# vlongle/pixie

Hardware: AMD Instinct MI355X
Metric: voxels/s (128^3 U-Net fwd) + MPM particle-steps/s (higher is better)
Workload: dtype f32 (operands split fp16 hi+lo, 3 f16 MFMAs/product, fp32 accumulate); 1 GPU; 128^3x64 feature grid -> SegmentationUNet+RegressionUNet forward (+argmax/one-hot combine), 1 scene per GPU per step; grid=128, feature_channels=64, parallelism=scene-parallel x1, executor=c+hip_graph

## Files before the change

include/pixie_hip.h:

```cpp
#ifndef PIXIE_HIP_H
#define PIXIE_HIP_H

#include <stdint.h>

#ifdef __cplusplus
extern "C" {
#endif

const char* pixie_last_error(void);
const char* pixie_build_arch(void);

typedef struct pixie_mpm pixie_mpm;

int pixie_mpm_create(pixie_mpm** out, int n_particles, int n_grid, double grid_lim);
int pixie_mpm_destroy(pixie_mpm* h);
int pixie_mpm_regrid(pixie_mpm* h, int n_grid, double grid_lim, void* stream);

int pixie_mpm_set_field(pixie_mpm* h, const char* name, const void* d_src, int64_t count, void* stream);
int pixie_mpm_get_field(pixie_mpm* h, const char* name, void* d_dst, int64_t count, void* stream);
int pixie_mpm_fill_field(pixie_mpm* h, const char* name, double value, void* stream);

int pixie_mpm_set_scalar(pixie_mpm* h, const char* key, double value);
int pixie_mpm_get_scalar(pixie_mpm* h, const char* key, double* value);

int pixie_mpm_update_mass(pixie_mpm* h, void* stream);
int pixie_mpm_finalize_mu_lam(pixie_mpm* h, int with_bulk, void* stream);
int pixie_mpm_apply_additional_params(pixie_mpm* h, const double point[3], const double size[3], double E,
                                      double nu, double density, int material, void* stream);
int pixie_mpm_apply_additional_params_batch(pixie_mpm* h, int64_t n_boxes, const float* d_boxes, const float* d_params,
                                            const int32_t* d_material, void* stream);

enum { PIXIE_BC_SURFACE = 0, PIXIE_BC_CUBOID = 1, PIXIE_BC_BBOX = 2 };
typedef struct pixie_bc_desc {
    int32_t type;
    int32_t surface_type;
    int32_t reset;
    int32_t pad_;
    double point[3], size[3], velocity[3], normal[3];
    double start_time, end_time, friction;
} pixie_bc_desc;
int pixie_mpm_add_bc(pixie_mpm* h, const pixie_bc_desc* bc);

enum { PIXIE_PM_IMPULSE = 0, PIXIE_PM_TRANSLATION = 1, PIXIE_PM_ROTATION = 2 };
typedef struct pixie_pmod_desc {
    int32_t type;
    int32_t pad_;
    double point[3], size[3];
    double force[3];
    double velocity[3];
    double normal[3], h1[3], h2[3];
    double half_height, radius, rotation_scale, translation_scale;
    double start_time, end_time;
} pixie_pmod_desc;
int pixie_mpm_add_particle_modifier(pixie_mpm* h, const pixie_pmod_desc* pm, void* stream);

int pixie_mpm_step(pixie_mpm* h, double dt, int n_substeps, void* stream);

typedef struct pixie_mpm_batch pixie_mpm_batch;
typedef struct pixie_batch_sched {
    double dt;
    int32_t steps_per_chunk;
    int32_t n_chunks;
    int32_t n_out;
    int32_t pad_;
    double shift[3], scale, mean[3];
    double inv_rotation[9];
    float* d_pos;
    float* d_cov;
} pixie_batch_sched;
int pixie_mpm_batch_create(pixie_mpm_batch** out, pixie_mpm* const* handles, int n_handles);
int pixie_mpm_batch_step(pixie_mpm_batch* b, double dt, int n_substeps, void* stream);
int pixie_mpm_batch_run(pixie_mpm_batch* b, const pixie_batch_sched* per_scene, int n_scenes, void* stream);
typedef struct pixie_batch_splat_out {
    float* d_log_scale;
    float* d_quat;
} pixie_batch_splat_out;
int pixie_mpm_batch_run_splats(pixie_mpm_batch* b, const pixie_batch_sched* per_scene, const pixie_batch_splat_out* splats ,
                               int n_scenes, void* stream);
int pixie_mpm_batch_destroy(pixie_mpm_batch* b);

int pixie_mpm_export_cov(pixie_mpm* h, float* d_cov , void* stream);
int pixie_mpm_export_R(pixie_mpm* h, float* d_R , void* stream);
int pixie_mpm_export_frame(pixie_mpm* h, int n_out, const double shift[3], double scale, const double mean[3],
                           const double inv_rotation[9], float* d_pos , float* d_cov ,
                           void* stream);
int pixie_splat_from_cov(const float* d_cov , int64_t n, float* d_log_scale , float* d_quat ,
                         void* stream);
int pixie_mpm_export_frame_splats(pixie_mpm* h, int n_out, const double shift[3], double scale, const double mean[3],
                                  const double inv_rotation[9], float* d_pos , float* d_cov ,
                                  float* d_log_scale , float* d_quat , void* stream);
int pixie_mpm_out_of_bounds(pixie_mpm* h, int64_t* count, void* stream);


typedef struct pixie_conv_desc {
    const float* d_in0; int32_t c0;
    const float* d_in1; int32_t c1;
    int32_t in_d, in_h, in_w;
    int32_t upsample;
    int32_t stride;
    int32_t ksize;
    const float* d_pro_a; const float* d_pro_b;
    const float* d_gamma; const float* d_beta;
    int32_t act;
    const float* d_w; const float* d_bias;
    int32_t c_out;
    const float* d_residual;
    float* d_out;
    const void* d_w16;
    const uint32_t* d_in_amax0; const uint32_t* d_in_amax1;
    float in_bound;
    float* d_out_stats;
    uint32_t* d_out_amax;
    void* d_workspace;
    int32_t out_d, out_h, out_w;
    const float* d_skip_in0; int32_t skip_c0;
    const float* d_skip_in1; int32_t skip_c1;
    const void* d_skip_w16; const float* d_skip_bias;
    const uint32_t* d_skip_amax0; const uint32_t* d_skip_amax1;
    int32_t w16_subpixel;
} pixie_conv_desc;

int pixie_conv_cout_padded(int c_out);
int pixie_conv_pack_weights(const float* d_w_oidhw, float* d_w_packed, int c_out, int c_in, int ksize, void* stream);
int64_t pixie_conv_packed16_bytes(int c_out, int c_in, int ksize);
int pixie_conv_pack_weights_f16x2(const float* d_w_oidhw, void* d_packed, int c_out, int c_in, int ksize, void* stream);
int64_t pixie_conv_subpixel_bytes(int c_out, int c_in);
int pixie_conv_pack_weights_subpixel(const float* d_w_oidhw, void* d_packed, int c_out, int c_in, void* stream);
int pixie_conv3d_forward(const pixie_conv_desc* desc, void* stream);
int64_t pixie_conv_stats_floats(const pixie_conv_desc* desc);
int64_t pixie_conv_workspace_bytes(const pixie_conv_desc* desc);
int pixie_stats_finalize(const float* d_stats, const pixie_conv_desc* desc, double* d_sums, void* stream);
int pixie_conv_skip_foldable(const pixie_conv_desc* desc);

int pixie_channel_sums(const float* d_x, int channels, int64_t spatial, double* d_sums, void* stream);
int pixie_channel_stats(const float* d_x, int channels, int64_t spatial, double* d_sums, uint32_t* d_amax, void* stream);
int pixie_tensor_amax(const float* d_x, int64_t count, uint32_t* d_slot, void* stream);
int pixie_norm_finalize(const double* d_sums, int channels, int64_t spatial, int mode, int groups, double eps,
                        const float* d_weight, const float* d_bias, float* d_a, float* d_b, void* stream);

int pixie_attention_forward(const float* d_qkv, float* d_out, int channels, int tokens, void* stream);

int pixie_channel_affine(const float* d_x, const float* d_a, const float* d_b, float* d_y, int channels,
                         int64_t spatial, void* stream);

int pixie_voxel_grid_to_ncdhw(const void* d_feat_dhwc_f16, int d, int h, int w, int channels, float* d_out_cdhw, void* stream);

int pixie_projector_conv0(const void* d_feat_dhwc_f16, int64_t voxels, int channels, int n_networks, const void* const* d_w16,
                          const float* const* d_bias, float* const* d_out, int c_out, void* stream);

int pixie_pack_fields(const float* d_cont, const int32_t* d_seg_pred, int64_t n_scenes, int64_t spatial, void* d_wire, int64_t wire_bytes,
                      void* stream);

int pixie_combine_predictions(const float* d_logits, int num_classes, const float* d_cont, int64_t spatial,
                              float* d_combined, int32_t* d_argmax , void* stream);

int pixie_combine_class_ids(const int32_t* d_seg_pred, int num_classes, const float* d_cont, int64_t spatial, float* d_combined,
                            void* stream);

typedef struct pixie_unet pixie_unet;
typedef struct pixie_unet_config {
    int32_t feature_channels, cond_dim, model_channels, num_res_blocks;
    int32_t n_channel_mult; int32_t channel_mult[8];
    int32_t n_attention_resolutions; int32_t attention_resolutions[8];
    int32_t grid_size;
    int32_t out_channels;
    int32_t precision;
} pixie_unet_config;

int pixie_unet_create(pixie_unet** out, const pixie_unet_config* cfg);
int pixie_unet_destroy(pixie_unet* h);
int pixie_unet_param_count(const pixie_unet* h);
int pixie_unet_param_info(const pixie_unet* h, int index, const char** key, int64_t* numel, int32_t* ndim, int64_t shape[5]);
int pixie_unet_set_param(pixie_unet* h, const char* key, const float* d_values, int64_t numel);
int64_t pixie_unet_workspace_bytes(pixie_unet* h, int d, int hh, int w);
int pixie_unet_forward(pixie_unet* h, const float* d_feat, const float* d_proj0, int d, int hh, int w, float* d_out,
                       void* d_workspace, int64_t workspace_bytes, void* stream);
int pixie_unet_set_option(pixie_unet* h, const char* key, int value);

typedef struct pixie_field_desc {
    const float* d_pred;
    const uint8_t* d_mask;
    const float* d_axis_x; const float* d_axis_y; const float* d_axis_z;
    int32_t n_classes, d, h, w;
    double min_spacing;
    double density_min, density_max, E_min, E_max, nu_min, nu_max;
} pixie_field_desc;
int pixie_field_to_particles(const pixie_field_desc* field, const float* d_pos, int n, int k, double nn_distance_threshold,
                             int weighted, int default_material, int default_part_label, float* d_density, float* d_E,
                             float* d_nu, int32_t* d_material, int32_t* d_part_label, float* d_conf, float* d_nearest,
                             void* d_scratch, void* stream);

int pixie_unscale_prediction(const float* d_pred, int channels, int64_t spatial, double density_min, double density_max,
                             double E_min, double E_max, double nu_min, double nu_max, float* d_out, void* stream);
int64_t pixie_field_points_scratch_bytes(const pixie_field_desc* field);
int pixie_field_points(const pixie_field_desc* field, int64_t capacity, float* d_xyz , float* d_density, float* d_E,
                       float* d_nu, int32_t* d_material, float* d_conf, int64_t* d_count, void* d_scratch, void* stream);

int pixie_dbscan_roots(const float* d_pos_sorted, const int32_t* d_orig_index, const int32_t* d_cell_start, int n, int nx, int ny, int nz,
                       const double lo[3], double cell_size, double eps, int min_samples, int32_t* d_core_scratch,
                       int32_t* d_parent_scratch, int32_t* d_root, void* stream);

int pixie_fill_densify(const float* d_pos, const float* d_opacity, const float* d_cov6, int n, int grid_n, double grid_dx,
                       int32_t* d_grid_count, float* d_grid_density, void* stream);
int pixie_fill_dense_cells(int32_t* d_grid_count, const float* d_grid_density, int grid_n, double grid_dx, double density_thres,
                           int max_particles_per_cell, float* d_new_particles , int64_t max_samples,
                           uint64_t* d_counter, uint32_t seed, void* stream);
int pixie_fill_internal_cells(int32_t* d_grid_count, const float* d_grid_density, int grid_n, double grid_dx, int max_particles_per_cell,
                              int exclude_dir, int ray_cast_dir, double threshold, float* d_new_particles, int64_t max_samples,
                              uint64_t* d_counter, uint32_t seed, void* stream);
int pixie_particle_volume(const float* d_pos, int n, int grid_n, double grid_dx, int32_t* d_grid_count_scratch, float* d_vol, void* stream);
int pixie_nearest_particle(const float* d_pos, int n, const float* d_new_pos, int n_new, int32_t* d_nearest, void* stream);

#ifdef PIXIE_DIAG
int pixie_mpm_phase(pixie_mpm* h, int phase, double dt, void* stream);

int pixie_mpm_kernel_times(pixie_mpm* h, double* particle_ms, double* grid_ms, int64_t* n_launches);

int pixie_conv_kernel_variant(const pixie_conv_desc* desc, int* slices);

int pixie_conv_tile_geometry(const pixie_conv_desc* desc, int32_t out[10]);
#endif

#ifdef __cplusplus
}
#endif
#endif
```

pixie_amd/_lib.py:

```python
from __future__ import annotations

import ctypes as C
import os

_HERE = os.path.dirname(os.path.abspath(__file__))
LIB_PATH = os.path.join(_HERE, "libpixie_hip.so")
DIAG_LIB_PATH = os.path.join(_HERE, "libpixie_hip_diag.so")


class PixieHipError(RuntimeError):
    pass


class BCDesc(C.Structure):
    _fields_ = [("type", C.c_int32), ("surface_type", C.c_int32), ("reset", C.c_int32), ("pad_", C.c_int32),
                ("point", C.c_double * 3), ("size", C.c_double * 3), ("velocity", C.c_double * 3),
                ("normal", C.c_double * 3), ("start_time", C.c_double), ("end_time", C.c_double),
                ("friction", C.c_double)]


class PModDesc(C.Structure):
    _fields_ = [("type", C.c_int32), ("pad_", C.c_int32),
                ("point", C.c_double * 3), ("size", C.c_double * 3), ("force", C.c_double * 3),
                ("velocity", C.c_double * 3), ("normal", C.c_double * 3), ("h1", C.c_double * 3),
                ("h2", C.c_double * 3), ("half_height", C.c_double), ("radius", C.c_double),
                ("rotation_scale", C.c_double), ("translation_scale", C.c_double),
                ("start_time", C.c_double), ("end_time", C.c_double)]


class ConvDesc(C.Structure):
    _fields_ = [("d_in0", C.c_void_p), ("c0", C.c_int32),
                ("d_in1", C.c_void_p), ("c1", C.c_int32),
                ("in_d", C.c_int32), ("in_h", C.c_int32), ("in_w", C.c_int32),
                ("upsample", C.c_int32), ("stride", C.c_int32), ("ksize", C.c_int32),
                ("d_pro_a", C.c_void_p), ("d_pro_b", C.c_void_p),
                ("d_gamma", C.c_void_p), ("d_beta", C.c_void_p),
                ("act", C.c_int32),
                ("d_w", C.c_void_p), ("d_bias", C.c_void_p),
                ("c_out", C.c_int32),
                ("d_residual", C.c_void_p), ("d_out", C.c_void_p),
                ("d_w16", C.c_void_p), ("d_in_amax0", C.c_void_p), ("d_in_amax1", C.c_void_p),
                ("in_bound", C.c_float),
                ("d_out_stats", C.c_void_p), ("d_out_amax", C.c_void_p),
                ("d_workspace", C.c_void_p),
                ("out_d", C.c_int32), ("out_h", C.c_int32), ("out_w", C.c_int32),
                ("d_skip_in0", C.c_void_p), ("skip_c0", C.c_int32),
                ("d_skip_in1", C.c_void_p), ("skip_c1", C.c_int32),
                ("d_skip_w16", C.c_void_p), ("d_skip_bias", C.c_void_p),
                ("d_skip_amax0", C.c_void_p), ("d_skip_amax1", C.c_void_p),
                ("w16_subpixel", C.c_int32)]


class UNetConfigC(C.Structure):
    _fields_ = [("feature_channels", C.c_int32), ("cond_dim", C.c_int32), ("model_channels", C.c_int32), ("num_res_blocks", C.c_int32),
                ("n_channel_mult", C.c_int32), ("channel_mult", C.c_int32 * 8),
                ("n_attention_resolutions", C.c_int32), ("attention_resolutions", C.c_int32 * 8),
                ("grid_size", C.c_int32), ("out_channels", C.c_int32), ("precision", C.c_int32)]


class BatchSched(C.Structure):
    _fields_ = [("dt", C.c_double), ("steps_per_chunk", C.c_int32), ("n_chunks", C.c_int32), ("n_out", C.c_int32), ("pad_", C.c_int32),
                ("shift", C.c_double * 3), ("scale", C.c_double), ("mean", C.c_double * 3), ("inv_rotation", C.c_double * 9),
                ("d_pos", C.c_void_p), ("d_cov", C.c_void_p)]


class BatchSplatOut(C.Structure):
    _fields_ = [("d_log_scale", C.c_void_p), ("d_quat", C.c_void_p)]


class FieldDesc(C.Structure):
    _fields_ = [("d_pred", C.c_void_p), ("d_mask", C.c_void_p),
                ("d_axis_x", C.c_void_p), ("d_axis_y", C.c_void_p), ("d_axis_z", C.c_void_p),
                ("n_classes", C.c_int32), ("d", C.c_int32), ("h", C.c_int32), ("w", C.c_int32),
                ("min_spacing", C.c_double),
                ("density_min", C.c_double), ("density_max", C.c_double), ("E_min", C.c_double), ("E_max", C.c_double),
                ("nu_min", C.c_double), ("nu_max", C.c_double)]


_VP, _I, _I64, _D, _S = C.c_void_p, C.c_int, C.c_int64, C.c_double, C.c_char_p
_D3 = C.POINTER(C.c_double)
SIGNATURES = {
    "pixie_last_error": (C.c_char_p, []),
    "pixie_build_arch": (C.c_char_p, []),
    "pixie_mpm_create": (_I, [C.POINTER(_VP), _I, _I, _D]),
    "pixie_mpm_destroy": (_I, [_VP]),
    "pixie_mpm_regrid": (_I, [_VP, _I, _D, _VP]),
    "pixie_mpm_set_field": (_I, [_VP, _S, _VP, _I64, _VP]),
    "pixie_mpm_get_field": (_I, [_VP, _S, _VP, _I64, _VP]),
    "pixie_mpm_fill_field": (_I, [_VP, _S, _D, _VP]),
    "pixie_mpm_set_scalar": (_I, [_VP, _S, _D]),
    "pixie_mpm_get_scalar": (_I, [_VP, _S, C.POINTER(_D)]),
    "pixie_mpm_update_mass": (_I, [_VP, _VP]),
    "pixie_mpm_finalize_mu_lam": (_I, [_VP, _I, _VP]),
    "pixie_mpm_apply_additional_params": (_I, [_VP, _D3, _D3, _D, _D, _D, _I, _VP]),
    "pixie_mpm_apply_additional_params_batch": (_I, [_VP, _I64, _VP, _VP, _VP, _VP]),
    "pixie_mpm_add_bc": (_I, [_VP, C.POINTER(BCDesc)]),
    "pixie_mpm_add_particle_modifier": (_I, [_VP, C.POINTER(PModDesc), _VP]),
    "pixie_mpm_step": (_I, [_VP, _D, _I, _VP]),
    "pixie_mpm_export_cov": (_I, [_VP, _VP, _VP]),
    "pixie_mpm_export_R": (_I, [_VP, _VP, _VP]),
    "pixie_mpm_export_frame": (_I, [_VP, _I, _D3, _D, _D3, C.POINTER(C.c_double), _VP, _VP, _VP]),
    "pixie_mpm_out_of_bounds": (_I, [_VP, C.POINTER(_I64), _VP]),
    "pixie_mpm_batch_create": (_I, [C.POINTER(_VP), C.POINTER(_VP), _I]),
    "pixie_mpm_batch_step": (_I, [_VP, _D, _I, _VP]),
    "pixie_mpm_batch_run": (_I, [_VP, C.POINTER(BatchSched), _I, _VP]),
    "pixie_mpm_batch_run_splats": (_I, [_VP, C.POINTER(BatchSched), C.POINTER(BatchSplatOut), _I, _VP]),
    "pixie_splat_from_cov": (_I, [_VP, _I64, _VP, _VP, _VP]),
    "pixie_mpm_export_frame_splats": (_I, [_VP, _I, _D3, _D, _D3, C.POINTER(C.c_double), _VP, _VP, _VP, _VP, _VP]),
    "pixie_mpm_batch_destroy": (_I, [_VP]),
    "pixie_pack_fields": (_I, [_VP, _VP, _I64, _I64, _VP, _I64, _VP]),
    "pixie_conv_cout_padded": (_I, [_I]),
    "pixie_conv_pack_weights": (_I, [_VP, _VP, _I, _I, _I, _VP]),
    "pixie_conv_packed16_bytes": (_I64, [_I, _I, _I]),
    "pixie_conv_pack_weights_f16x2": (_I, [_VP, _VP, _I, _I, _I, _VP]),
    "pixie_conv_subpixel_bytes": (_I64, [_I, _I]),
    "pixie_conv_pack_weights_subpixel": (_I, [_VP, _VP, _I, _I, _VP]),
    "pixie_conv3d_forward": (_I, [C.POINTER(ConvDesc), _VP]),
    "pixie_conv_stats_floats": (_I64, [C.POINTER(ConvDesc)]),
    "pixie_conv_workspace_bytes": (_I64, [C.POINTER(ConvDesc)]),
    "pixie_stats_finalize": (_I, [_VP, C.POINTER(ConvDesc), _VP, _VP]),
    "pixie_channel_stats": (_I, [_VP, _I, _I64, _VP, _VP, _VP]),
    "pixie_tensor_amax": (_I, [_VP, _I64, _VP, _VP]),
    "pixie_channel_sums": (_I, [_VP, _I, _I64, _VP, _VP]),
    "pixie_norm_finalize": (_I, [_VP, _I, _I64, _I, _I, _D, _VP, _VP, _VP, _VP, _VP]),
    "pixie_attention_forward": (_I, [_VP, _VP, _I, _I, _VP]),
    "pixie_channel_affine": (_I, [_VP, _VP, _VP, _VP, _I, _I64, _VP]),
    "pixie_projector_conv0": (_I, [_VP, _I64, _I, _I, C.POINTER(_VP), C.POINTER(_VP), C.POINTER(_VP), _I, _VP]),
    "pixie_conv_skip_foldable": (_I, [C.POINTER(ConvDesc)]),
    "pixie_unet_create": (_I, [C.POINTER(_VP), C.POINTER(UNetConfigC)]),
    "pixie_unet_destroy": (_I, [_VP]),
    "pixie_unet_param_count": (_I, [_VP]),
    "pixie_unet_param_info": (_I, [_VP, _I, C.POINTER(_S), C.POINTER(_I64), C.POINTER(C.c_int32), C.POINTER(_I64)]),
    "pixie_unet_set_param": (_I, [_VP, _S, _VP, _I64]),
    "pixie_unet_workspace_bytes": (_I64, [_VP, _I, _I, _I]),
    "pixie_unet_set_option": (_I, [_VP, _S, _I]),
    "pixie_unet_forward": (_I, [_VP, _VP, _VP, _I, _I, _I, _VP, _VP, _I64, _VP]),
    "pixie_combine_class_ids": (_I, [_VP, _I, _VP, _I64, _VP, _VP]),
    "pixie_combine_predictions": (_I, [_VP, _I, _VP, _I64, _VP, _VP, _VP]),
    "pixie_voxel_grid_to_ncdhw": (_I, [_VP, _I, _I, _I, _I, _VP, _VP]),
    "pixie_unscale_prediction": (_I, [_VP, _I, _I64, _D, _D, _D, _D, _D, _D, _VP, _VP]),
    "pixie_field_points_scratch_bytes": (_I64, [C.POINTER(FieldDesc)]),
    "pixie_field_points": (_I, [C.POINTER(FieldDesc), _I64, _VP, _VP, _VP, _VP, _VP, _VP, _VP, _VP, _VP]),
    "pixie_fill_densify": (_I, [_VP, _VP, _VP, _I, _I, _D, _VP, _VP, _VP]),
    "pixie_fill_dense_cells": (_I, [_VP, _VP, _I, _D, _D, _I, _VP, _I64, _VP, C.c_uint32, _VP]),
    "pixie_fill_internal_cells": (_I, [_VP, _VP, _I, _D, _I, _I, _I, _D, _VP, _I64, _VP, C.c_uint32, _VP]),
    "pixie_particle_volume": (_I, [_VP, _I, _I, _D, _VP, _VP, _VP]),
    "pixie_nearest_particle": (_I, [_VP, _I, _VP, _I, _VP, _VP]),
    "pixie_dbscan_roots": (_I, [_VP, _VP, _VP, _I, _I, _I, _I, C.POINTER(_D), _D, _D, _I, _VP, _VP, _VP, _VP]),
    "pixie_field_to_particles": (_I, [C.POINTER(FieldDesc), _VP, _I, _I, _D, _I, _I, _I, _VP, _VP, _VP, _VP, _VP, _VP, _VP, _VP, _VP]),
}

DIAG_SIGNATURES = {
    "pixie_mpm_phase": (_I, [_VP, _I, _D, _VP]),
    "pixie_mpm_kernel_times": (_I, [_VP, C.POINTER(_D), C.POINTER(_D), C.POINTER(_I64)]),
    "pixie_conv_kernel_variant": (C.c_int, [C.POINTER(ConvDesc), C.POINTER(C.c_int)]),
    "pixie_conv_tile_geometry": (C.c_int, [C.POINTER(ConvDesc), C.POINTER(C.c_int32)]),
}

_libs = {}


def load(diag: bool = False):
    if diag in _libs:
        return _libs[diag]
    path = DIAG_LIB_PATH if diag else LIB_PATH
    if not os.path.exists(path):
        raise PixieHipError(
            f"{path} not found: build it with `python -m pixie_amd.build` (hipcc, gfx950). "
            "pixie_amd has no CPU fallback.")
    import torch
    lib = C.CDLL(path)
    for name, (res, args) in list(SIGNATURES.items()) + (list(DIAG_SIGNATURES.items()) if diag else []):
        fn = getattr(lib, name)
        fn.restype = res
        fn.argtypes = args
    _libs[diag] = lib
    return lib


def check(rc: int, what: str = "", lib=None):
    if rc != 0:
        msg = (lib or load()).pixie_last_error()
        raise PixieHipError(f"{what}: {msg.decode() if msg else 'unknown error'}")


def current_stream_ptr():
    import torch
    try:
        return C.c_void_p(torch._C._cuda_getCurrentRawStream(torch.cuda.current_device()))
    except AttributeError:
        return C.c_void_p(torch.cuda.current_stream().cuda_stream)


def d3(v):
    return (C.c_double * 3)(*[float(x) for x in v])
```

pixie_amd/csrc/conv3d_f16x3.hip:

```cpp
#include <hip/hip_runtime.h>

#include <cstdlib>
#include <map>
#include <string>
#include <type_traits>

#include "../../include/pixie_hip.h"
#include "common.h"

namespace pixie {

typedef float f32x16 __attribute__((ext_vector_type(16)));
typedef _Float16 f16x8 __attribute__((ext_vector_type(8)));

constexpr int kW16HeaderU4 = 4;

struct Conv16Args {
    const float* in0; const float* in1;
    int c0, cin;
    int ID, IH, IW;
    int LD, LH, LW;
    int ups;
    int stride;
    int OD, OH, OW;
    const float* pro_a; const float* pro_b; const float* gamma; const float* beta;
    int act;
    const uint4* w16;
    const float* wf;
    const float* bias;
    int cout, coutp;
    const float* residual; float* out;
    const unsigned* amax0; const unsigned* amax1;
    float in_bound;
    int TX, TY, TZ, lTX, lTY;
    int tiles_x, tiles_y, tiles_z, n_tiles;
    int HX, HY, HZ, HYX, CS;
    unsigned mHX, mHYX;
    float* stats; unsigned* out_amax;
    float* partial; int chunks_per_slice;
    int epi_lds;
    const float* sk_in0; const float* sk_in1;
    int sk_c0, sk_cin;
    const uint4* sk_w16; const float* sk_bias;
    const unsigned* sk_amax0; const unsigned* sk_amax1;
};

__device__ __forceinline__ int fast_div16(int n, int d, unsigned magic) {
    return (d == 1) ? n : (int)__umulhi((unsigned)n, magic);
}
__device__ __forceinline__ float act16(float t, int act) {
    if (act == 1) return t > 0.0f ? t : 0.02f * t;
    if (act == 2) return t / (1.0f + __expf(-t));
    return t;
}
__device__ __forceinline__ int scale_exponent(float bound) {
    const unsigned bits = __float_as_uint(bound);
    const int eb = (int)((bits >> 23) & 0xffu) - 127;
    if (!(bound > 0.0f) || eb > 100) return 0;
    int e = 14 - eb;
    return e > 100 ? 100 : (e < -100 ? -100 : e);
}
__device__ __forceinline__ float pow2i(int e) { return __uint_as_float((unsigned)(e + 127) << 23); }

template <int KS, int MB, int NB, bool EX = false, bool SP = false>
__device__ __forceinline__ void conv3d_f16x3_body(const Conv16Args& A) {
    static_assert(!SP || (KS == 3 && NB == 4 && !EX), "sub-pixel path: 3^3, two x parities x two voxel blocks per wave");
    extern __shared__ uint4 smem16[];
    constexpr int PAD = (KS == 3) ? 1 : 0;
    constexpr int NW = 4, NT = 64 * NW;
    const int bufsz = 4 * A.CS;

    const int tid = threadIdx.x;
    const int lane = tid & 63;
    const int wave = tid >> 6;
    const int kh = lane >> 5;
    const int l31 = lane & 31;

    int t = blockIdx.x;
    {
        const int per = (A.n_tiles + 7) >> 3;
        const int cand = (t & 7) * per + (t >> 3);
        if ((A.n_tiles & 7) == 0) t = cand;
    }
    int par = 0;
    if constexpr (SP) { par = t & 3; t >>= 2; }
    const int py = par & 1, pz = par >> 1;
    const int tx = t % A.tiles_x; t /= A.tiles_x;
    const int ty = t % A.tiles_y;
    const int tz = t / A.tiles_y;
    const int ox0 = tx * A.TX, oy0 = ty * A.TY, oz0 = tz * A.TZ;
    const int cout0 = blockIdx.y * (MB * 32);
    const int lx0 = SP ? ox0 - 1 : ox0 * A.stride - PAD;
    const int ly0 = SP ? oy0 - 1 + py : oy0 * A.stride - PAD;
    const int lz0 = SP ? oz0 - 1 + pz : oz0 * A.stride - PAD;
    const size_t ISP = (size_t)A.ID * A.IH * A.IW;
    const size_t OSP = (size_t)A.OD * A.OH * A.OW;

    int voff[NB];
    int ovox[NB];
    bool valid[NB];
#pragma unroll
    for (int nb = 0; nb < NB; ++nb) {
        if constexpr (SP) {
            const int px = nb >> 1;
            const int j = (wave * 2 + (nb & 1)) * 32 + l31;
            int x = j & (A.TX - 1);
            int y = (j >> A.lTX) & (A.TY - 1);
            int z = j >> (A.lTX + A.lTY);
            const int gx = 2 * (ox0 + x) + px, gy = 2 * (oy0 + y) + py, gz = 2 * (oz0 + z) + pz;
            const bool v = (z < A.TZ) && (gx < A.OW) && (gy < A.OH) && (gz < A.OD);
            if (!v) { x = 0; y = 0; z = 0; }
            voff[nb] = (z * A.HY + y) * A.HX + x + px + kh * A.CS;
            ovox[nb] = v ? (gz * A.OH + gy) * A.OW + gx : 0;
            valid[nb] = v;
            continue;
        }
        const int j = (wave * NB + nb) * 32 + l31;
        int x = j & (A.TX - 1);
        int y = (j >> A.lTX) & (A.TY - 1);
        int z = j >> (A.lTX + A.lTY);
        const bool v = (z < A.TZ) && (ox0 + x < A.OW) && (oy0 + y < A.OH) && (oz0 + z < A.OD);
        if (!v) { x = 0; y = 0; z = 0; }
        voff[nb] = ((z * A.HY + y) * A.HX + x) * A.stride + kh * A.CS;
        ovox[nb] = ((oz0 + z) * A.OH + (oy0 + y)) * A.OW + ox0 + x;
        valid[nb] = v;
    }

    float bound = A.in_bound;
    if (A.amax0) {
        bound = __uint_as_float(*A.amax0);
        if (A.amax1) bound = fmaxf(bound, __uint_as_float(*A.amax1));
    }
    const int ex = EX ? 0 : scale_exponent(bound);
    const float sx = pow2i(ex);

    f32x16 acc[MB][NB];
#pragma unroll
    for (int mb = 0; mb < MB; ++mb)
#pragma unroll
        for (int nb = 0; nb < NB; ++nb)
#pragma unroll
            for (int r = 0; r < 16; ++r) acc[mb][nb][r] = 0.0f;

    const int KG = A.cin >> 3;
    const size_t tap_stride = (size_t)KG * A.coutp;
    const size_t plane = (size_t)(SP ? 64 : KS * KS * KS) * tap_stride;
    const uint4* wHi = A.w16 + kW16HeaderU4 + (size_t)kh * A.coutp + cout0 + l31 + (size_t)(par * 16) * tap_stride;
    const uint4* wLo = wHi + plane;
    const float* wF = A.wf + (size_t)kh * A.coutp + cout0 + l31;

    constexpr int TAPS = KS * KS * KS;
    auto stage_chunk = [&](int c_base, uint4* buf, int stid, int nthr) {
        uint4* bHi = buf;
        uint4* bLo = buf + 2 * A.CS;
        float pa[16], pb[16];
        {
            float pv = 0.0f;
            if (A.pro_a) pv = (lane & 16) ? A.pro_b[c_base + (lane & 15)] : A.pro_a[c_base + (lane & 15)];
#pragma unroll
            for (int j = 0; j < 16; ++j) {
                pa[j] = __int_as_float(__builtin_amdgcn_readlane(__float_as_int(pv), j));
                pb[j] = __int_as_float(__builtin_amdgcn_readlane(__float_as_int(pv), 16 + j));
            }
        }
        const bool has_aff = A.gamma != nullptr;
        for (int v0 = stid; v0 < A.CS; v0 += 2 * nthr) {
            float val[2][16];
            float gm[2], bt[2];
            int sidx[2];
            bool ok[2];
#pragma unroll
            for (int u = 0; u < 2; ++u) {
                const int vox = v0 + u * nthr;
                int rem = vox;
                const int hz = fast_div16(rem, A.HYX, A.mHYX);
                rem -= hz * A.HYX;
                const int hy = fast_div16(rem, A.HX, A.mHX);
                const int hx = rem - hy * A.HX;
                const int lz = lz0 + hz, ly = ly0 + hy, lx = lx0 + hx;
                ok[u] = vox < A.CS && (unsigned)lz < (unsigned)A.LD && (unsigned)ly < (unsigned)A.LH && (unsigned)lx < (unsigned)A.LW;
                sidx[u] = ok[u] ? ((lz >> A.ups) * A.IH + (ly >> A.ups)) * A.IW + (lx >> A.ups) : 0;
            }
#pragma unroll
            for (int u = 0; u < 2; ++u) {
#pragma unroll
                for (int j = 0; j < 16; ++j) {
                    const int cg = c_base + j;
                    const float* src = (cg < A.c0) ? (A.in0 + (size_t)cg * ISP) : (A.in1 + (size_t)(cg - A.c0) * ISP);
                    val[u][j] = src[sidx[u]];
                }
                gm[u] = 1.0f; bt[u] = 0.0f;
                if (has_aff) { gm[u] = A.gamma[sidx[u]]; bt[u] = A.beta[sidx[u]]; }
            }
            auto convert = [&](auto has_pro, auto act_c) {
#pragma unroll
                for (int u = 0; u < 2; ++u) {
                    const int vox = v0 + u * nthr;
                    if (EX) {
                        float* bF = reinterpret_cast<float*>(buf);
#pragma unroll
                        for (int j = 0; j < 16; ++j) {
                            float t = val[u][j];
                            if (decltype(has_pro)::value) t = t * pa[j] + pb[j];
                            t = t * gm[u] + bt[u];
                            const float sc = ok[u] ? act16(t, decltype(act_c)::value) : 0.0f;
                            if (vox < A.CS) bF[j * A.CS + vox] = sc;
                        }
                        continue;
                    }
                    f16x8 vh[2], vl[2];
#pragma unroll
                    for (int j = 0; j < 16; ++j) {
                        float t = val[u][j];
                        if (decltype(has_pro)::value) t = t * pa[j] + pb[j];
                        t = t * gm[u] + bt[u];
                        const float sc = ok[u] ? act16(t, decltype(act_c)::value) * sx : 0.0f;
                        const _Float16 h = (_Float16)sc;
                        vh[j >> 3][j & 7] = h;
                        vl[j >> 3][j & 7] = (_Float16)(sc - (float)h);
                    }
                    if (vox < A.CS) {
                        bHi[vox] = __builtin_bit_cast(uint4, vh[0]);
                        bHi[A.CS + vox] = __builtin_bit_cast(uint4, vh[1]);
                        bLo[vox] = __builtin_bit_cast(uint4, vl[0]);
                        bLo[A.CS + vox] = __builtin_bit_cast(uint4, vl[1]);
                    }
                }
            };
            using T = std::true_type; using F = std::false_type;
            if (A.pro_a) {
                if (A.act == 1) convert(T{}, std::integral_constant<int, 1>{});
                else if (A.act == 2) convert(T{}, std::integral_constant<int, 2>{});
                else convert(T{}, std::integral_constant<int, 0>{});
            } else {
                if (A.act == 1) convert(F{}, std::integral_constant<int, 1>{});
                else if (A.act == 2) convert(F{}, std::integral_constant<int, 2>{});
                else convert(F{}, std::integral_constant<int, 0>{});
            }
        }
    };
    auto mfma_chunk = [&](int c_base, const uint4* buf) {
        __builtin_amdgcn_s_setprio(3);
        if constexpr (EX) {
            const float* ldsF = reinterpret_cast<const float*>(buf);
            const size_t tapw = (size_t)A.cin * A.coutp;
            const float* wc = wF + (size_t)c_base * A.coutp;
            float a[8][MB], an[8][MB];
#pragma unroll
            for (int kp = 0; kp < 8; ++kp)
#pragma unroll
                for (int mb = 0; mb < MB; ++mb) a[kp][mb] = wc[(size_t)(2 * kp) * A.coutp + mb * 32];
#pragma unroll 1
            for (int zy = 0; zy < KS * KS; ++zy) {
                const int dz = zy / KS, dy = zy - dz * KS;
                const int rowoff = (dz * A.HY + dy) * A.HX;
#pragma unroll
                for (int dx = 0; dx < KS; ++dx) {
                    const int tap = zy * KS + dx;
                    const int nxt = (tap + 1 < TAPS) ? tap + 1 : tap;
#pragma unroll
                    for (int kp = 0; kp < 8; ++kp)
#pragma unroll
                        for (int mb = 0; mb < MB; ++mb) an[kp][mb] = wc[(size_t)nxt * tapw + (size_t)(2 * kp) * A.coutp + mb * 32];
                    __builtin_amdgcn_sched_barrier(0);
#pragma unroll
                    for (int kp = 0; kp < 8; ++kp) {
                        float b[NB];
#pragma unroll
                        for (int nb = 0; nb < NB; ++nb) b[nb] = ldsF[voff[nb] + rowoff + dx + 2 * kp * A.CS];
#pragma unroll
                        for (int mb = 0; mb < MB; ++mb)
#pragma unroll
                            for (int nb = 0; nb < NB; ++nb)
                                acc[mb][nb] = __builtin_amdgcn_mfma_f32_32x32x2f32(a[kp][mb], b[nb], acc[mb][nb], 0, 0, 0);
                    }
#pragma unroll
                    for (int kp = 0; kp < 8; ++kp)
#pragma unroll
                        for (int mb = 0; mb < MB; ++mb) a[kp][mb] = an[kp][mb];
                }
            }
            __builtin_amdgcn_s_setprio(0);
            return;
        }
        const uint4* ldsHi = buf;
        const uint4* ldsLo = buf + 2 * A.CS;
        const uint4* wh = wHi + (size_t)(c_base >> 3) * A.coutp;
        const uint4* wl = wLo + (size_t)(c_base >> 3) * A.coutp;
        if constexpr (SP) {
            f16x8 ah[MB], al[MB];
#pragma unroll
            for (int mb = 0; mb < MB; ++mb) {
                ah[mb] = __builtin_bit_cast(f16x8, wh[mb * 32]);
                al[mb] = __builtin_bit_cast(f16x8, wl[mb * 32]);
            }
#pragma unroll 1
            for (int zy = 0; zy < 4; ++zy) {
                const int rowoff = ((zy >> 1) * A.HY + (zy & 1)) * A.HX;
                const int zyn = zy < 3 ? zy + 1 : 3;
#pragma unroll
                for (int q = 0; q < 4; ++q) {
                    const int ex = q >> 1, px = q & 1;
                    const size_t nxt = (q < 3) ? (size_t)(((q + 1) & 1) * 8 + zy * 2 + ((q + 1) >> 1)) * tap_stride : (size_t)(zyn * 2) * tap_stride;
                    f16x8 ahn[MB], aln[MB];
#pragma unroll
                    for (int mb = 0; mb < MB; ++mb) {
                        ahn[mb] = __builtin_bit_cast(f16x8, wh[nxt + mb * 32]);
                        aln[mb] = __builtin_bit_cast(f16x8, wl[nxt + mb * 32]);
                    }
                    __builtin_amdgcn_sched_barrier(0);
                    f16x8 bh[2], bl[2];
#pragma unroll
                    for (int s = 0; s < 2; ++s) {
                        bh[s] = __builtin_bit_cast(f16x8, ldsHi[voff[px * 2 + s] + rowoff + ex]);
                        bl[s] = __builtin_bit_cast(f16x8, ldsLo[voff[px * 2 + s] + rowoff + ex]);
                    }
#pragma unroll
                    for (int mb = 0; mb < MB; ++mb)
#pragma unroll
                        for (int s = 0; s < 2; ++s)
                            acc[mb][px * 2 + s] = __builtin_amdgcn_mfma_f32_32x32x16_f16(al[mb], bh[s], acc[mb][px * 2 + s], 0, 0, 0);
#pragma unroll
                    for (int mb = 0; mb < MB; ++mb)
#pragma unroll
                        for (int s = 0; s < 2; ++s)
                            acc[mb][px * 2 + s] = __builtin_amdgcn_mfma_f32_32x32x16_f16(ah[mb], bl[s], acc[mb][px * 2 + s], 0, 0, 0);
#pragma unroll
                    for (int mb = 0; mb < MB; ++mb)
#pragma unroll
                        for (int s = 0; s < 2; ++s)
                            acc[mb][px * 2 + s] = __builtin_amdgcn_mfma_f32_32x32x16_f16(ah[mb], bh[s], acc[mb][px * 2 + s], 0, 0, 0);
#pragma unroll
                    for (int mb = 0; mb < MB; ++mb) { ah[mb] = ahn[mb]; al[mb] = aln[mb]; }
                }
            }
            __builtin_amdgcn_s_setprio(0);
            return;
        }
        f16x8 ah[MB], al[MB];
#pragma unroll
        for (int mb = 0; mb < MB; ++mb) {
            ah[mb] = __builtin_bit_cast(f16x8, wh[mb * 32]);
            al[mb] = __builtin_bit_cast(f16x8, wl[mb * 32]);
        }
#pragma unroll 1
        for (int zy = 0; zy < KS * KS; ++zy) {
            const int dz = zy / KS, dy = zy - dz * KS;
            const int rowoff = (dz * A.HY + dy) * A.HX;
#pragma unroll
            for (int dx = 0; dx < KS; ++dx) {
                const int tap = zy * KS + dx;
                const int nxt = (tap + 1 < TAPS) ? tap + 1 : tap;
                f16x8 ahn[MB], aln[MB];
#pragma unroll
                for (int mb = 0; mb < MB; ++mb) {
                    ahn[mb] = __builtin_bit_cast(f16x8, wh[(size_t)nxt * tap_stride + mb * 32]);
                    aln[mb] = __builtin_bit_cast(f16x8, wl[(size_t)nxt * tap_stride + mb * 32]);
                }
                __builtin_amdgcn_sched_barrier(0);
                f16x8 bh[NB], bl[NB];
#pragma unroll
                for (int nb = 0; nb < NB; ++nb) {
                    bh[nb] = __builtin_bit_cast(f16x8, ldsHi[voff[nb] + rowoff + dx]);
                    bl[nb] = __builtin_bit_cast(f16x8, ldsLo[voff[nb] + rowoff + dx]);
                }
#pragma unroll
                for (int mb = 0; mb < MB; ++mb)
#pragma unroll
                    for (int nb = 0; nb < NB; ++nb)
                        acc[mb][nb] = __builtin_amdgcn_mfma_f32_32x32x16_f16(al[mb], bh[nb], acc[mb][nb], 0, 0, 0);
#pragma unroll
                for (int mb = 0; mb < MB; ++mb)
#pragma unroll
                    for (int nb = 0; nb < NB; ++nb)
                        acc[mb][nb] = __builtin_amdgcn_mfma_f32_32x32x16_f16(ah[mb], bl[nb], acc[mb][nb], 0, 0, 0);
#pragma unroll
                for (int mb = 0; mb < MB; ++mb)
#pragma unroll
                    for (int nb = 0; nb < NB; ++nb)
                        acc[mb][nb] = __builtin_amdgcn_mfma_f32_32x32x16_f16(ah[mb], bh[nb], acc[mb][nb], 0, 0, 0);
#pragma unroll
                for (int mb = 0; mb < MB; ++mb) { ah[mb] = ahn[mb]; al[mb] = aln[mb]; }
            }
        }
        __builtin_amdgcn_s_setprio(0);
    };

    float inv2 = 0.0f;
    {
        const int c_begin = A.partial ? (int)blockIdx.z * A.chunks_per_slice * 16 : 0;
        const int c_end = A.partial ? min(A.cin, c_begin + A.chunks_per_slice * 16) : A.cin;
        for (int c_base = c_begin; c_base < c_end; c_base += 16) {
            __syncthreads();
            stage_chunk(c_base, smem16, tid, NT);
            __syncthreads();
            mfma_chunk(c_base, smem16);
        }
        if (!EX && !SP && A.sk_w16) {
            float sb = __uint_as_float(*A.sk_amax0);
            if (A.sk_amax1) sb = fmaxf(sb, __uint_as_float(*A.sk_amax1));
            const int ex2 = scale_exponent(sb);
            const float sx2 = pow2i(ex2);
            const float inv_main = __uint_as_float(A.w16[0].x) * pow2i(-ex);
            inv2 = __uint_as_float(A.sk_w16[0].x) * pow2i(-ex2);
            const float ratio = inv_main / inv2;
#pragma unroll
            for (int mb = 0; mb < MB; ++mb)
#pragma unroll
                for (int nb = 0; nb < NB; ++nb)
#pragma unroll
                    for (int r = 0; r < 16; ++r) acc[mb][nb][r] *= ratio;
            const int KG2 = A.sk_cin >> 3;
            const uint4* w2Hi = A.sk_w16 + kW16HeaderU4 + (size_t)kh * A.coutp + cout0 + l31;
            const uint4* w2Lo = w2Hi + (size_t)KG2 * A.coutp;
            const int centre = (KS == 3) ? (A.HY + 1) * A.HX + 1 : 0;
            const int tvox = A.TX * A.TY * A.TZ;
            for (int c2 = 0; c2 < A.sk_cin; c2 += 16) {
                f16x8 ah[MB], al[MB];
#pragma unroll
                for (int mb = 0; mb < MB; ++mb) {
                    ah[mb] = __builtin_bit_cast(f16x8, w2Hi[(size_t)(c2 >> 3) * A.coutp + mb * 32]);
                    al[mb] = __builtin_bit_cast(f16x8, w2Lo[(size_t)(c2 >> 3) * A.coutp + mb * 32]);
                }
                __syncthreads();
                uint4* bHi = smem16;
                uint4* bLo = smem16 + 2 * A.CS;
                for (int j = tid; j < tvox; j += NT) {
                    const int x = j & (A.TX - 1), y = (j >> A.lTX) & (A.TY - 1), z = j >> (A.lTX + A.lTY);
                    const bool okv = (ox0 + x < A.OW) && (oy0 + y < A.OH) && (oz0 + z < A.OD);
                    const size_t sidx = okv ? ((size_t)(oz0 + z) * A.IH + (oy0 + y)) * A.IW + ox0 + x : 0;
                    float val[16];
#pragma unroll
                    for (int q = 0; q < 16; ++q) {
                        const int cg = c2 + q;
                        const float* src = (cg < A.sk_c0) ? (A.sk_in0 + (size_t)cg * ISP) : (A.sk_in1 + (size_t)(cg - A.sk_c0) * ISP);
                        val[q] = src[sidx];
                    }
                    f16x8 vh[2], vl[2];
#pragma unroll
                    for (int q = 0; q < 16; ++q) {
                        const float sc = okv ? val[q] * sx2 : 0.0f;
                        const _Float16 hq = (_Float16)sc;
                        vh[q >> 3][q & 7] = hq;
                        vl[q >> 3][q & 7] = (_Float16)(sc - (float)hq);
                    }
                    const int slot = (z * A.HY + y) * A.HX + x + centre;
                    bHi[slot] = __builtin_bit_cast(uint4, vh[0]);
                    bHi[A.CS + slot] = __builtin_bit_cast(uint4, vh[1]);
                    bLo[slot] = __builtin_bit_cast(uint4, vl[0]);
                    bLo[A.CS + slot] = __builtin_bit_cast(uint4, vl[1]);
                }
                __syncthreads();
                f16x8 bh[NB], bl[NB];
#pragma unroll
                for (int nb = 0; nb < NB; ++nb) {
                    bh[nb] = __builtin_bit_cast(f16x8, bHi[voff[nb] + centre]);
                    bl[nb] = __builtin_bit_cast(f16x8, bLo[voff[nb] + centre]);
                }
#pragma unroll
                for (int mb = 0; mb < MB; ++mb)
#pragma unroll
                    for (int nb = 0; nb < NB; ++nb)
                        acc[mb][nb] = __builtin_amdgcn_mfma_f32_32x32x16_f16(al[mb], bh[nb], acc[mb][nb], 0, 0, 0);
#pragma unroll
                for (int mb = 0; mb < MB; ++mb)
#pragma unroll
                    for (int nb = 0; nb < NB; ++nb)
                        acc[mb][nb] = __builtin_amdgcn_mfma_f32_32x32x16_f16(ah[mb], bl[nb], acc[mb][nb], 0, 0, 0);
#pragma unroll
                for (int mb = 0; mb < MB; ++mb)
#pragma unroll
                    for (int nb = 0; nb < NB; ++nb)
                        acc[mb][nb] = __builtin_amdgcn_mfma_f32_32x32x16_f16(ah[mb], bh[nb], acc[mb][nb], 0, 0, 0);
            }
        }
    }

    const float inv = EX ? 1.0f : (A.sk_w16 ? inv2 : __uint_as_float(A.w16[0].x) * pow2i(-ex));
    if (A.partial) {
        float* dst = A.partial + (size_t)blockIdx.z * A.cout * OSP;
#pragma unroll
        for (int mb = 0; mb < MB; ++mb)
#pragma unroll
            for (int r = 0; r < 16; ++r) {
                const int co = cout0 + mb * 32 + (r & 3) + 8 * (r >> 2) + 4 * kh;
                if (co < A.cout) {
#pragma unroll
                    for (int nb = 0; nb < NB; ++nb)
                        if (valid[nb]) dst[(size_t)co * OSP + ovox[nb]] = acc[mb][nb][r] * inv;
                }
            }
        return;
    }
    float* red = reinterpret_cast<float*>(smem16);
    float wmax = 0.0f;
    const bool full = SP ? (A.epi_lds && cout0 + MB * 32 <= A.cout && (A.TX & 1) == 0 && (A.OW & 3) == 0 && NW * 64 <= A.TX * A.TY * A.TZ &&
                            2 * (ox0 + A.TX) <= A.OW && 2 * (oy0 + A.TY) <= A.OH && 2 * (oz0 + A.TZ) <= A.OD)
                         : (A.epi_lds && cout0 + MB * 32 <= A.cout && (A.TX & 3) == 0 && (A.OW & 3) == 0 && NW * NB * 32 <= A.TX * A.TY * A.TZ &&
                            ox0 + A.TX <= A.OW && oy0 + A.TY <= A.OH && oz0 + A.TZ <= A.OD);
    if (full) {
        __syncthreads();
        constexpr int LDO = NB * 32 + 4;
        float* ldsO = reinterpret_cast<float*>(smem16) + wave * (32 * LDO);
        red = reinterpret_cast<float*>(smem16) + NW * 32 * LDO;
        constexpr int LPR = NB * 8;
        constexpr int RPI = 32 / LPR;
        const int rsub = l31 / LPR, colq = 4 * (l31 % LPR), nbq = colq >> 5;
        const int jq = SP ? wave * 64 + (colq >> 1) : (wave * NB + nbq) * 32 + (colq & 31);
        const int xq = jq & (A.TX - 1), yq = (jq >> A.lTX) & (A.TY - 1), zq = jq >> (A.lTX + A.lTY);
        const size_t ovq = SP ? ((size_t)(2 * (oz0 + zq) + pz) * A.OH + (2 * (oy0 + yq) + py)) * A.OW + 2 * (ox0 + xq)
                              : ((size_t)(oz0 + zq) * A.OH + (oy0 + yq)) * A.OW + ox0 + xq;
        const bool has_res = A.residual != nullptr, has_stats = A.stats != nullptr;
#pragma unroll
        for (int mb = 0; mb < MB; ++mb) {
#pragma unroll
            for (int r = 0; r < 16; ++r)
#pragma unroll
                for (int nb = 0; nb < NB; ++nb)
                    ldsO[((r & 3) + 8 * (r >> 2) + 4 * kh) * LDO + (SP ? 2 * ((nb & 1) * 32 + l31) + (nb >> 1) : nb * 32 + l31)] = acc[mb][nb][r];
#pragma unroll 4
            for (int it = 0; it < 16 / RPI; ++it) {
                const int rowl = (2 * it + kh) * RPI + rsub;
                const int co = cout0 + mb * 32 + rowl;
                const float4 a4 = *reinterpret_cast<const float4*>(ldsO + rowl * LDO + colq);
                const float bv = (A.bias ? A.bias[co] : 0.0f) + (A.sk_bias ? A.sk_bias[co] : 0.0f);
                const size_t o = (size_t)co * OSP + ovq;
                float4 v4;
                v4.x = a4.x * inv + bv; v4.y = a4.y * inv + bv; v4.z = a4.z * inv + bv; v4.w = a4.w * inv + bv;
                if (has_res) {
                    const float4 r4 = *reinterpret_cast<const float4*>(A.residual + o);
                    v4.x += r4.x; v4.y += r4.y; v4.z += r4.z; v4.w += r4.w;
                }
                *reinterpret_cast<float4*>(A.out + o) = v4;
                if (has_stats) {
                    float s1 = (v4.x + v4.y) + (v4.z + v4.w);
                    float s2 = (v4.x * v4.x + v4.y * v4.y) + (v4.z * v4.z + v4.w * v4.w);
                    wmax = fmaxf(fmaxf(wmax, fmaxf(fabsf(v4.x), fabsf(v4.y))), fmaxf(fabsf(v4.z), fabsf(v4.w)));
#pragma unroll
                    for (int off = LPR / 2; off > 0; off >>= 1) { s1 += __shfl_xor(s1, off, 64); s2 += __shfl_xor(s2, off, 64); }
                    if ((l31 % LPR) == 0) { red[(wave * MB * 32 + mb * 32 + rowl) * 2] = s1; red[(wave * MB * 32 + mb * 32 + rowl) * 2 + 1] = s2; }
                }
            }
        }
    } else {
    if (A.stats) __syncthreads();
#pragma unroll
    for (int mb = 0; mb < MB; ++mb) {
#pragma unroll
        for (int r = 0; r < 16; ++r) {
            const int row = mb * 32 + (r & 3) + 8 * (r >> 2) + 4 * kh;
            const int co = cout0 + row;
            float s1 = 0.0f, s2 = 0.0f;
            if (co < A.cout) {
                const float bv = (A.bias ? A.bias[co] : 0.0f) + (A.sk_bias ? A.sk_bias[co] : 0.0f);
#pragma unroll
                for (int nb = 0; nb < NB; ++nb) {
                    if (valid[nb]) {
                        const size_t o = (size_t)co * OSP + ovox[nb];
                        float val = acc[mb][nb][r] * inv + bv;
                        if (A.residual) val += A.residual[o];
                        A.out[o] = val;
                        s1 += val; s2 += val * val; wmax = fmaxf(wmax, fabsf(val));
                    }
                }
            }
            if (A.stats) {
#pragma unroll
                for (int off = 16; off > 0; off >>= 1) { s1 += __shfl_xor(s1, off, 64); s2 += __shfl_xor(s2, off, 64); }
                if (l31 == 0) { red[(wave * MB * 32 + row) * 2] = s1; red[(wave * MB * 32 + row) * 2 + 1] = s2; }
            }
        }
    }
    }
    if (A.stats) {
        __syncthreads();
        if (tid < MB * 32 * 2) {
            float t = red[tid];
#pragma unroll
            for (int w = 1; w < NW; ++w) t += red[w * MB * 64 + tid];
            A.stats[((size_t)blockIdx.x * A.coutp + cout0) * 2 + tid] = t;
        }
        if (A.out_amax) {
#pragma unroll
            for (int off = 32; off > 0; off >>= 1) wmax = fmaxf(wmax, __shfl_xor(wmax, off, 64));
            if (lane == 0 && wmax > 0.0f) atomicMax(A.out_amax, __float_as_uint(wmax));
        }
    }
}

template <int KS, int MB, int NB>
__global__ __launch_bounds__(256, 2) void conv3d_f16x3_kernel(Conv16Args A) {
    conv3d_f16x3_body<KS, MB, NB>(A);
}
template <int KS, int MB, int NB>
__global__ __launch_bounds__(256, 2) void conv3d_exact_kernel(Conv16Args A) {
    conv3d_f16x3_body<KS, MB, NB, true>(A);
}
template <int MB>
__global__ __launch_bounds__(256, 2) void conv3d_f16x3_subpixel_kernel(Conv16Args A) {
    conv3d_f16x3_body<3, MB, 4, false, true>(A);
}
__global__ __launch_bounds__(256, 2) void conv3d_f16x3_c64_fullres_kernel(Conv16Args A) {
    conv3d_f16x3_body<3, 2, 4>(A);
}

__global__ __launch_bounds__(256) void stats_finalize_kernel(const float* __restrict__ stats, int n_tiles, int coutp, double* __restrict__ sums) {
    const int c = blockIdx.x;
    double s1 = 0.0, s2 = 0.0;
    for (int t = threadIdx.x; t < n_tiles; t += 256) {
        const float2 v = *reinterpret_cast<const float2*>(stats + ((size_t)t * coutp + c) * 2);
        s1 += v.x; s2 += v.y;
    }
    for (int off = 32; off > 0; off >>= 1) { s1 += __shfl_down(s1, off, 64); s2 += __shfl_down(s2, off, 64); }
    __shared__ double r[8];
    if ((threadIdx.x & 63) == 0) { r[2 * (threadIdx.x >> 6)] = s1; r[2 * (threadIdx.x >> 6) + 1] = s2; }
    __syncthreads();
    if (threadIdx.x == 0) { sums[2 * c] = r[0] + r[2] + r[4] + r[6]; sums[2 * c + 1] = r[1] + r[3] + r[5] + r[7]; }
}

__global__ __launch_bounds__(256) void splitk_reduce_kernel(const float* __restrict__ partial, int slices, long n_elems, long osp,
                                                            const float* __restrict__ bias, const float* residual, float* out) {
    const long i = (long)blockIdx.x * 256 + threadIdx.x;
    if (i >= n_elems) return;
    float v = partial[i];
    for (int s = 1; s < slices; ++s) v += partial[(size_t)s * n_elems + i];
    if (bias) v += bias[i / osp];
    if (residual) v += residual[i];
    out[i] = v;
}

__global__ __launch_bounds__(256) void amax_kernel(const float* __restrict__ x, long n, unsigned* __restrict__ slot) {
    float m = 0.0f;
    const long stride = (long)gridDim.x * 256 * 4;
    long i = ((long)blockIdx.x * 256 + threadIdx.x) * 4;
    if ((reinterpret_cast<size_t>(x) & 15) == 0) {
        for (; i + 3 < n; i += stride) {
            const float4 v = *reinterpret_cast<const float4*>(x + i);
            m = fmaxf(fmaxf(m, fabsf(v.x)), fmaxf(fabsf(v.y), fmaxf(fabsf(v.z), fabsf(v.w))));
        }
        for (long k = i; k < n && k < i + 4; ++k) m = fmaxf(m, fabsf(x[k]));
    } else {
        for (long k = (long)blockIdx.x * 256 + threadIdx.x; k < n; k += (long)gridDim.x * 256) m = fmaxf(m, fabsf(x[k]));
    }
    for (int off = 32; off > 0; off >>= 1) m = fmaxf(m, __shfl_down(m, off, 64));
    if ((threadIdx.x & 63) == 0 && m > 0.0f) atomicMax(slot, __float_as_uint(m));
}

__global__ void pack_weights_f16x2_kernel(const float* __restrict__ src, uint4* __restrict__ dst, int cout, int cin, int taps,
                                          int coutp, const unsigned* __restrict__ amax_bits) {
    const int KG = cin >> 3;
    const long total = (long)taps * KG * coutp;
    const long i = (long)blockIdx.x * blockDim.x + threadIdx.x;
    const int e = scale_exponent(__uint_as_float(*amax_bits));
    if (i == 0) dst[0] = make_uint4(__float_as_uint(pow2i(-e)), (unsigned)cout, (unsigned)cin, (unsigned)taps);
    if (i >= total) return;
    const float s = pow2i(e);
    const int co = (int)(i % coutp);
    const long row = i / coutp;
    const int kg = (int)(row % KG);
    const int tap = (int)(row / KG);
    f16x8 vh, vl;
#pragma unroll
    for (int j = 0; j < 8; ++j) {
        float w = 0.0f;
        if (co < cout) w = src[((long)co * cin + kg * 8 + j) * taps + tap] * s;
        const _Float16 h = (_Float16)w;
        vh[j] = h;
        vl[j] = (_Float16)(w - (float)h);
    }
    dst[kW16HeaderU4 + i] = __builtin_bit_cast(uint4, vh);
    dst[kW16HeaderU4 + total + i] = __builtin_bit_cast(uint4, vl);
}

__device__ __forceinline__ float subpixel_weight(const float* __restrict__ w27, int par, int tap) {
    int lo[3], hi[3];
#pragma unroll
    for (int ax = 0; ax < 3; ++ax) {
        const int p = (par >> (2 - ax)) & 1, e = (tap >> (2 - ax)) & 1;
        lo[ax] = e ? (p ? 2 : 1) : 0;
        hi[ax] = e ? 2 : (p ? 1 : 0);
    }
    float sum = 0.0f;
    for (int dz = lo[0]; dz <= hi[0]; ++dz)
        for (int dy = lo[1]; dy <= hi[1]; ++dy)
            for (int dx = lo[2]; dx <= hi[2]; ++dx) sum += w27[(dz * 3 + dy) * 3 + dx];
    return sum;
}
__global__ __launch_bounds__(256) void subpixel_amax_kernel(const float* __restrict__ src, long pairs, unsigned* __restrict__ slot) {
    const long i = (long)blockIdx.x * 256 + threadIdx.x;
    float m = 0.0f;
    if (i < pairs)
        for (int pt = 0; pt < 64; ++pt) m = fmaxf(m, fabsf(subpixel_weight(src + i * 27, pt >> 3, pt & 7)));
    for (int off = 32; off > 0; off >>= 1) m = fmaxf(m, __shfl_down(m, off, 64));
    if ((threadIdx.x & 63) == 0 && m > 0.0f) atomicMax(slot, __float_as_uint(m));
}
__global__ void pack_weights_subpixel_kernel(const float* __restrict__ src, uint4* __restrict__ dst, int cout, int cin, int coutp,
                                             const unsigned* __restrict__ amax_bits) {
    const int KG = cin >> 3;
    const long total = 64L * KG * coutp;
    const long i = (long)blockIdx.x * blockDim.x + threadIdx.x;
    const int e = scale_exponent(__uint_as_float(*amax_bits));
    if (i == 0) dst[0] = make_uint4(__float_as_uint(pow2i(-e)), (unsigned)cout, (unsigned)cin, 64u);
    if (i >= total) return;
    const float s = pow2i(e);
    const int co = (int)(i % coutp);
    const long row = i / coutp;
    const int kg = (int)(row % KG);
    const int pt = (int)(row / KG);
    f16x8 vh, vl;
#pragma unroll
    for (int j = 0; j < 8; ++j) {
        float w = 0.0f;
        if (co < cout) w = subpixel_weight(src + ((long)co * cin + kg * 8 + j) * 27, pt >> 3, pt & 7) * s;
        const _Float16 h = (_Float16)w;
        vh[j] = h;
        vl[j] = (_Float16)(w - (float)h);
    }
    dst[kW16HeaderU4 + i] = __builtin_bit_cast(uint4, vh);
    dst[kW16HeaderU4 + total + i] = __builtin_bit_cast(uint4, vl);
}

static unsigned magic_of16(int d) { return d <= 1 ? 0u : (unsigned)((0x100000000ull + (unsigned long long)d - 1) / (unsigned long long)d); }
static int ilog2_16(int v) { int l = 0; while ((1 << l) < v) ++l; return l; }
static int pow2_le16(int v, int cap) { int p = 1; while (p * 2 <= v && p * 2 <= cap) p *= 2; return p; }

template <int MB>
static int launch_subpixel(const Conv16Args& a, size_t lds_bytes, dim3 grid, hipStream_t st) {
    auto kern = conv3d_f16x3_subpixel_kernel<MB>;
    PX_CHECK_HIP(allow_max_dynamic_lds(reinterpret_cast<const void*>(kern)));
    hipLaunchKernelGGL(kern, grid, dim3(256), lds_bytes, st, a);
    PX_CHECK_HIP(hipGetLastError());
    return 0;
}

static bool conv16_subpixel(const pixie_conv_desc* d) {
    return d->d_w16 && d->w16_subpixel && d->upsample == 1 && d->ksize == 3 && d->stride == 1;
}

template <int KS, int MB, int NB>
static int launch_f16x3(const Conv16Args& a, size_t lds_bytes, dim3 grid, hipStream_t st) {
    auto kern = conv3d_f16x3_kernel<KS, MB, NB>;
    PX_CHECK_HIP(allow_max_dynamic_lds(reinterpret_cast<const void*>(kern)));
    hipLaunchKernelGGL(kern, grid, dim3(256), lds_bytes, st, a);
    PX_CHECK_HIP(hipGetLastError());
    return 0;
}

static void conv16_tiling(const pixie_conv_desc* d, Conv16Args& a, int& MB_out, int& NB_out, int* slices_out = nullptr) {
    a.ID = d->in_d; a.IH = d->in_h; a.IW = d->in_w;
    a.ups = d->upsample;
    a.LD = a.ID << a.ups; a.LH = a.IH << a.ups; a.LW = a.IW << a.ups;
    const int pad = d->ksize == 3 ? 1 : 0;
    a.stride = d->stride;
    a.OD = (a.LD + 2 * pad - d->ksize) / a.stride + 1; a.OH = (a.LH + 2 * pad - d->ksize) / a.stride + 1; a.OW = (a.LW + 2 * pad - d->ksize) / a.stride + 1;
    if (d->out_d > 0) a.OD = std::min(a.OD, (int)d->out_d);
    if (d->out_h > 0) a.OH = std::min(a.OH, (int)d->out_h);
    if (d->out_w > 0) a.OW = std::min(a.OW, (int)d->out_w);
    a.cout = d->c_out; a.coutp = pixie_conv_cout_padded(d->c_out);
    const int chunks = (d->c0 + d->c1) / 16;
    const int smax = d->d_workspace ? std::min(8, chunks / 2) : 1;
    if (conv16_subpixel(d)) {
        a.ups = 0; a.LD = a.ID; a.LH = a.IH; a.LW = a.IW;
        const int SD = (a.OD + 1) / 2, SH = (a.OH + 1) / 2, SW = (a.OW + 1) / 2;
        a.TX = pow2_le16(SW, 32);
        a.TY = pow2_le16(SH, std::max(1, std::min(4, 256 / a.TX)));
        a.TZ = std::max(1, std::min(SD, 256 / (a.TX * a.TY)));
        a.lTX = ilog2_16(a.TX); a.lTY = ilog2_16(a.TY);
        a.tiles_x = (SW + a.TX - 1) / a.TX; a.tiles_y = (SH + a.TY - 1) / a.TY; a.tiles_z = (SD + a.TZ - 1) / a.TZ;
        a.n_tiles = 4 * a.tiles_x * a.tiles_y * a.tiles_z;
        a.HX = a.TX + 2; a.HY = a.TY + 1; a.HZ = a.TZ + 1;
        a.HYX = a.HY * a.HX; a.CS = a.HZ * a.HYX;
        a.mHX = magic_of16(a.HX); a.mHYX = magic_of16(a.HYX);
        MB_out = (a.coutp >= 64) ? 2 : 1; NB_out = 4;
        int sl = 1;
        const long wgs = (long)a.n_tiles * ((a.coutp + MB_out * 32 - 1) / (MB_out * 32));
        while (sl * 2 <= smax && wgs * sl < 512) sl *= 2;
        if (slices_out) *slices_out = sl;
        return;
    }
    const long ovol = (long)a.OD * a.OH * a.OW;
    int MB = (a.coutp >= 64) ? 2 : 1;
    int NB = (a.stride == 2) ? 1 : 4;
    auto n_wg = [&](int mb, int nb) {
        const long tiles = (ovol + 128L * nb - 1) / (128L * nb);
        return tiles * ((a.coutp + mb * 32 - 1) / (mb * 32));
    };
    int slices = 1;
    if (smax >= 2 && n_wg(MB, NB) < 512) {
        bool found = false;
        for (int nb = NB; nb >= 1 && !found; nb /= 2) {
            for (int sl = 1; sl <= smax; sl *= 2)
                if (n_wg(MB, nb) * sl >= 512) { NB = nb; slices = sl; found = true; break; }
        }
        if (!found) { NB = 1; slices = 1; while (slices * 2 <= smax) slices *= 2; }
    } else {
        while (n_wg(MB, NB) < 512 && NB > 1) NB /= 2;
        if (n_wg(MB, NB) < 512 && MB > 1) MB = 1;
    }
    if (slices_out) *slices_out = slices;
    const int tile_vox = 128 * NB;
    a.TX = pow2_le16(a.OW, 32);
    a.TY = pow2_le16(a.OH, std::max(1, std::min(4, tile_vox / a.TX)));
    a.TZ = std::max(1, std::min(a.OD, tile_vox / (a.TX * a.TY)));
    a.lTX = ilog2_16(a.TX); a.lTY = ilog2_16(a.TY);
    a.tiles_x = (a.OW + a.TX - 1) / a.TX; a.tiles_y = (a.OH + a.TY - 1) / a.TY; a.tiles_z = (a.OD + a.TZ - 1) / a.TZ;
    a.n_tiles = a.tiles_x * a.tiles_y * a.tiles_z;
    a.HX = (a.TX - 1) * a.stride + d->ksize; a.HY = (a.TY - 1) * a.stride + d->ksize; a.HZ = (a.TZ - 1) * a.stride + d->ksize;
    a.HYX = a.HY * a.HX; a.CS = a.HZ * a.HYX;
    a.mHX = magic_of16(a.HX); a.mHYX = magic_of16(a.HYX);

    MB_out = MB; NB_out = NB;
}

static size_t conv16_epi_bytes(int MB, int NB) { return ((size_t)4 * 32 * (NB * 32 + 4) + (size_t)4 * MB * 32 * 2) * sizeof(float); }
static bool conv16_epi_lds(int MB, int NB, int slices) { return slices == 1 && conv16_epi_bytes(MB, NB) <= 80 * 1024; }

static void conv16_exact_tiling(const pixie_conv_desc* d, Conv16Args& a, int& MB_out, int& NB_out) {
    pixie_conv_desc probe = *d;
    probe.d_workspace = nullptr;
    probe.w16_subpixel = 0;
    int slices = 1;
    conv16_tiling(&probe, a, MB_out, NB_out, &slices);
}

int conv3d_f16x3_forward(const pixie_conv_desc* d, hipStream_t st) {
    PX_REQUIRE(d->stride == 1 || (d->stride == 2 && d->ksize == 3 && !d->upsample), "f16x3 conv: stride must be 1, or 2 for a 3^3 kernel");
    const int cin = d->c0 + d->c1;
    PX_REQUIRE(cin % 16 == 0 && d->c0 % 8 == 0, "f16x3 conv: c_in must be a multiple of 16 (got %d+%d)", d->c0, d->c1);
    PX_REQUIRE(d->d_in_amax0 != nullptr || d->in_bound > 0.0f, "f16x3 conv: needs d_in_amax0 or a positive in_bound");
    PX_REQUIRE(d->c1 == 0 || d->d_in_amax0 == nullptr || d->d_in_amax1 != nullptr, "f16x3 conv: second input needs its own amax slot");
    Conv16Args a{};
    a.in0 = d->d_in0; a.in1 = d->d_in1; a.c0 = d->c0; a.cin = cin;
    a.ID = d->in_d; a.IH = d->in_h; a.IW = d->in_w;
    a.ups = d->upsample;
    a.LD = a.ID << a.ups; a.LH = a.IH << a.ups; a.LW = a.IW << a.ups;
    const int pad = d->ksize == 3 ? 1 : 0;
    a.stride = d->stride;
    a.OD = (a.LD + 2 * pad - d->ksize) / a.stride + 1; a.OH = (a.LH + 2 * pad - d->ksize) / a.stride + 1; a.OW = (a.LW + 2 * pad - d->ksize) / a.stride + 1;
    if (d->out_d > 0) a.OD = std::min(a.OD, (int)d->out_d);
    if (d->out_h > 0) a.OH = std::min(a.OH, (int)d->out_h);
    if (d->out_w > 0) a.OW = std::min(a.OW, (int)d->out_w);
    a.pro_a = d->d_pro_a; a.pro_b = d->d_pro_b; a.gamma = d->d_gamma; a.beta = d->d_beta; a.act = d->act;
    a.w16 = reinterpret_cast<const uint4*>(d->d_w16); a.bias = d->d_bias; a.cout = d->c_out; a.coutp = pixie_conv_cout_padded(d->c_out);
    a.residual = d->d_residual; a.out = d->d_out;
    a.amax0 = d->d_in_amax0; a.amax1 = (d->c1 > 0) ? d->d_in_amax1 : nullptr; a.in_bound = d->in_bound;
    a.stats = d->d_out_stats; a.out_amax = d->d_out_amax;

    int MB = 0, NB = 0, slices = 1;
    const bool sp = d->w16_subpixel != 0;
    PX_REQUIRE(!sp || (conv16_subpixel(d) && !d->d_skip_w16), "f16x3 conv: sub-pixel weights need upsample = 1, ksize = 3, stride = 1 and no folded skip");
    conv16_tiling(d, a, MB, NB, &slices);
    if (d->d_skip_w16) {
        const int scin = d->skip_c0 + d->skip_c1;
        PX_REQUIRE(pixie_conv_skip_foldable(d), "f16x3 conv: this launch cannot fold a skip convolution (pixie_conv_skip_foldable)");
        PX_REQUIRE(d->d_skip_in0 && d->d_skip_amax0 && (d->skip_c1 == 0 || (d->d_skip_in1 && d->d_skip_amax1)), "f16x3 conv: folded skip needs its inputs and their amax slots");
        a.sk_in0 = d->d_skip_in0; a.sk_in1 = d->d_skip_in1; a.sk_c0 = d->skip_c0; a.sk_cin = scin;
        a.sk_w16 = reinterpret_cast<const uint4*>(d->d_skip_w16); a.sk_bias = d->d_skip_bias;
        a.sk_amax0 = d->d_skip_amax0; a.sk_amax1 = d->skip_c1 > 0 ? d->d_skip_amax1 : nullptr;
    }
    if (slices > 1) {
        a.partial = static_cast<float*>(d->d_workspace);
        a.chunks_per_slice = (cin / 16 + slices - 1) / slices;
        a.stats = nullptr; a.out_amax = nullptr;
    }

    size_t lds = (size_t)4 * a.CS * sizeof(uint4);
    PX_REQUIRE(lds <= 160 * 1024, "f16x3 conv: tile needs %zu B of LDS", lds);
    if (conv16_epi_lds(MB, NB, slices)) { a.epi_lds = 1; lds = std::max(lds, conv16_epi_bytes(MB, NB)); }
    const dim3 grid((unsigned)a.n_tiles, (unsigned)((a.coutp + MB * 32 - 1) / (MB * 32)), (unsigned)slices);
    if (slices > 1) {
        int rc = 1;
        if (sp) {
            rc = (MB == 2) ? launch_subpixel<2>(a, lds, grid, st) : launch_subpixel<1>(a, lds, grid, st);
        } else {
#define PX_CONV16_SK(KS_, MB_, NB_) \
            if (d->ksize == KS_ && MB == MB_ && NB == NB_) rc = launch_f16x3<KS_, MB_, NB_>(a, lds, grid, st);
            PX_CONV16_SK(3, 2, 4) PX_CONV16_SK(3, 2, 2) PX_CONV16_SK(3, 2, 1) PX_CONV16_SK(3, 1, 4) PX_CONV16_SK(3, 1, 2) PX_CONV16_SK(3, 1, 1)
            PX_CONV16_SK(1, 2, 4) PX_CONV16_SK(1, 2, 2) PX_CONV16_SK(1, 2, 1) PX_CONV16_SK(1, 1, 4) PX_CONV16_SK(1, 1, 2) PX_CONV16_SK(1, 1, 1)
#undef PX_CONV16_SK
        }
        if (rc) return rc;
        const long osp = (long)a.OD * a.OH * a.OW, n_elems = (long)a.cout * osp;
        hipLaunchKernelGGL(splitk_reduce_kernel, dim3((unsigned)((n_elems + 255) / 256)), dim3(256), 0, st, a.partial, slices, n_elems, osp,
                           a.bias, a.residual, a.out);
        PX_CHECK_HIP(hipGetLastError());
        return 0;
    }
    if (sp) return (MB == 2) ? launch_subpixel<2>(a, lds, grid, st) : launch_subpixel<1>(a, lds, grid, st);
    if (d->ksize == 3 && MB == 2 && NB == 4 && cin == 64 && d->c_out == 64 && d->stride == 1 && !d->upsample && d->c1 == 0 && !a.sk_w16 &&
        (long)a.OD * a.OH * a.OW >= 128L * 128 * 128) {
        auto kern = conv3d_f16x3_c64_fullres_kernel;
        PX_CHECK_HIP(allow_max_dynamic_lds(reinterpret_cast<const void*>(kern)));
        hipLaunchKernelGGL(kern, grid, dim3(256), lds, st, a);
        PX_CHECK_HIP(hipGetLastError());
        return 0;
    }
#define PX_CONV16_CASE(KS_, MB_, NB_) \
    if (d->ksize == KS_ && MB == MB_ && NB == NB_) return launch_f16x3<KS_, MB_, NB_>(a, lds, grid, st);
    PX_CONV16_CASE(3, 2, 4) PX_CONV16_CASE(3, 2, 2) PX_CONV16_CASE(3, 2, 1)
    PX_CONV16_CASE(3, 1, 4) PX_CONV16_CASE(3, 1, 2) PX_CONV16_CASE(3, 1, 1)
    PX_CONV16_CASE(1, 2, 4) PX_CONV16_CASE(1, 2, 2) PX_CONV16_CASE(1, 2, 1)
    PX_CONV16_CASE(1, 1, 4) PX_CONV16_CASE(1, 1, 2) PX_CONV16_CASE(1, 1, 1)
#undef PX_CONV16_CASE
    return set_error("f16x3 conv: no kernel variant for ksize=%d MB=%d NB=%d", d->ksize, MB, NB);
}

template <int KS, int MB, int NB>
static int launch_exact(const Conv16Args& a, size_t lds_bytes, dim3 grid, hipStream_t st) {
    auto kern = conv3d_exact_kernel<KS, MB, NB>;
    PX_CHECK_HIP(allow_max_dynamic_lds(reinterpret_cast<const void*>(kern)));
    hipLaunchKernelGGL(kern, grid, dim3(256), lds_bytes, st, a);
    PX_CHECK_HIP(hipGetLastError());
    return 0;
}

bool conv3d_exact_tiled_ok(const pixie_conv_desc* d) {
    const int cin = d->c0 + d->c1;
    return cin % 16 == 0 && (d->stride == 1 || (d->stride == 2 && d->ksize == 3 && !d->upsample)) && getenv("PIXIE_CONV_EXACT_V1") == nullptr;
}

int conv3d_exact_forward(const pixie_conv_desc* d, hipStream_t st) {
    Conv16Args a{};
    a.in0 = d->d_in0; a.in1 = d->d_in1; a.c0 = d->c0; a.cin = d->c0 + d->c1;
    a.pro_a = d->d_pro_a; a.pro_b = d->d_pro_b; a.gamma = d->d_gamma; a.beta = d->d_beta; a.act = d->act;
    a.wf = d->d_w; a.bias = d->d_bias;
    a.residual = d->d_residual; a.out = d->d_out;
    a.in_bound = 1.0f;
    int MB = 0, NB = 0;
    conv16_exact_tiling(d, a, MB, NB);
    size_t lds = (size_t)4 * a.CS * sizeof(uint4);
    PX_REQUIRE(lds <= 160 * 1024, "exact conv: tile needs %zu B of LDS", lds);
    if (conv16_epi_lds(MB, NB, 1)) { a.epi_lds = 1; lds = std::max(lds, conv16_epi_bytes(MB, NB)); }
    const dim3 grid((unsigned)a.n_tiles, (unsigned)((a.coutp + MB * 32 - 1) / (MB * 32)), 1u);
#define PX_CONVEX_CASE(KS_, MB_, NB_) \
    if (d->ksize == KS_ && MB == MB_ && NB == NB_) return launch_exact<KS_, MB_, NB_>(a, lds, grid, st);
    PX_CONVEX_CASE(3, 2, 4) PX_CONVEX_CASE(3, 2, 2) PX_CONVEX_CASE(3, 2, 1)
    PX_CONVEX_CASE(3, 1, 4) PX_CONVEX_CASE(3, 1, 2) PX_CONVEX_CASE(3, 1, 1)
    PX_CONVEX_CASE(1, 2, 4) PX_CONVEX_CASE(1, 2, 2) PX_CONVEX_CASE(1, 2, 1)
    PX_CONVEX_CASE(1, 1, 4) PX_CONVEX_CASE(1, 1, 2) PX_CONVEX_CASE(1, 1, 1)
#undef PX_CONVEX_CASE
    return set_error("exact conv: no kernel variant for ksize=%d MB=%d NB=%d", d->ksize, MB, NB);
}

}

using namespace pixie;

extern "C" int64_t pixie_conv_stats_floats(const pixie_conv_desc* d) {
    if (!d || !d->d_w16 || !(d->stride == 1 || (d->stride == 2 && d->ksize == 3)) || (d->ksize != 1 && d->ksize != 3)) return 0;
    Conv16Args a{};
    int MB = 0, NB = 0, slices = 1;
    conv16_tiling(d, a, MB, NB, &slices);
    return slices > 1 ? 0 : (int64_t)a.n_tiles * a.coutp * 2;
}

extern "C" int64_t pixie_conv_workspace_bytes(const pixie_conv_desc* d) {
    if (!d || !d->d_w16 || !(d->stride == 1 || (d->stride == 2 && d->ksize == 3)) || (d->ksize != 1 && d->ksize != 3)) return 0;
    pixie_conv_desc probe = *d;
    probe.d_workspace = reinterpret_cast<void*>(1);
    Conv16Args a{};
    int MB = 0, NB = 0, slices = 1;
    conv16_tiling(&probe, a, MB, NB, &slices);
    return slices > 1 ? (int64_t)slices * a.cout * a.OD * a.OH * a.OW * (int64_t)sizeof(float) : 0;
}

#ifdef PIXIE_DIAG
extern "C" int pixie_conv_kernel_variant(const pixie_conv_desc* d, int* slices_out) {
    if (slices_out) *slices_out = 1;
    if (!d || !d->d_w16 || !(d->stride == 1 || (d->stride == 2 && d->ksize == 3)) || (d->ksize != 1 && d->ksize != 3)) return 0;
    Conv16Args a{};
    int MB = 0, NB = 0, slices = 1;
    conv16_tiling(d, a, MB, NB, &slices);
    if (slices_out) *slices_out = slices;
    if (conv16_subpixel(d)) return 8300 + MB * 10 + NB;
    if (d->ksize == 3 && MB == 2 && NB == 4 && d->c0 + d->c1 == 64 && d->c_out == 64 && d->stride == 1 && !d->upsample && d->c1 == 0 && !d->d_skip_w16 &&
        (long)a.OD * a.OH * a.OW >= 128L * 128 * 128)
        return 9324;
    return d->ksize * 100 + MB * 10 + NB;
}

extern "C" int pixie_conv_tile_geometry(const pixie_conv_desc* d, int32_t out[10]) {
    if (!d || !out || (d->ksize != 1 && d->ksize != 3) || !(d->stride == 1 || (d->stride == 2 && d->ksize == 3 && !d->upsample))) return 1;
    if ((d->c0 + d->c1) % 16 != 0 || (d->d_w16 && d->c0 % 8 != 0)) return 1;
    if (!d->d_w16 && !conv3d_exact_tiled_ok(d)) return 1;
    Conv16Args a{};
    int MB = 0, NB = 0, slices = 1;
    if (d->d_w16) conv16_tiling(d, a, MB, NB, &slices);
    else conv16_exact_tiling(d, a, MB, NB);
    const int32_t v[10] = {a.TX, a.TY, a.TZ, a.tiles_x, a.tiles_y, a.tiles_z, conv16_epi_lds(MB, NB, slices) ? 1 : 0, slices, MB, NB};
    for (int i = 0; i < 10; ++i) out[i] = v[i];
    return 0;
}
#endif

extern "C" int pixie_conv_skip_foldable(const pixie_conv_desc* d) {
    if (!d || !d->d_w16 || d->stride != 1 || d->upsample || (d->ksize != 1 && d->ksize != 3)) return 0;
    const int scin = d->skip_c0 + d->skip_c1;
    if (scin <= 0 || scin % 16 != 0 || d->skip_c0 % 8 != 0 || (d->c0 + d->c1) % 16 != 0 || d->c0 % 8 != 0) return 0;
    Conv16Args a{};
    int MB = 0, NB = 0, slices = 1;
    conv16_tiling(d, a, MB, NB, &slices);
    return slices == 1 ? 1 : 0;
}

extern "C" int pixie_stats_finalize(const float* d_stats, const pixie_conv_desc* d, double* d_sums, void* stream) {
    PX_REQUIRE(d_stats && d && d_sums, "pixie_stats_finalize: null argument");
    Conv16Args a{};
    int MB = 0, NB = 0;
    conv16_tiling(d, a, MB, NB);
    hipLaunchKernelGGL(stats_finalize_kernel, dim3((unsigned)d->c_out), dim3(256), 0, as_stream(stream), d_stats, a.n_tiles, a.coutp, d_sums);
    PX_CHECK_HIP(hipGetLastError());
    return 0;
}

extern "C" int64_t pixie_conv_packed16_bytes(int c_out, int c_in, int ksize) {
    if (c_out <= 0 || c_in <= 0 || c_in % 8 != 0 || (ksize != 1 && ksize != 3)) return 0;
    const int64_t taps = (int64_t)ksize * ksize * ksize;
    return ((int64_t)kW16HeaderU4 + 2 * taps * (c_in / 8) * pixie_conv_cout_padded(c_out)) * (int64_t)sizeof(uint4);
}

extern "C" int pixie_tensor_amax(const float* d_x, int64_t count, uint32_t* d_slot, void* stream) {
    PX_REQUIRE(d_x && d_slot && count > 0, "pixie_tensor_amax: bad arguments");
    const int blocks = (int)std::min<int64_t>(2048, (count + 1023) / 1024);
    hipLaunchKernelGGL(amax_kernel, dim3(blocks), dim3(256), 0, as_stream(stream), d_x, (long)count, d_slot);
    PX_CHECK_HIP(hipGetLastError());
    return 0;
}

extern "C" int pixie_conv_pack_weights_f16x2(const float* d_w, void* d_packed, int c_out, int c_in, int ksize, void* stream) {
    PX_REQUIRE(d_w && d_packed && c_out > 0 && c_in > 0 && c_in % 8 == 0 && (ksize == 1 || ksize == 3),
               "pixie_conv_pack_weights_f16x2: bad arguments (c_in must be a multiple of 8)");
    hipStream_t st = as_stream(stream);
    const int taps = ksize * ksize * ksize;
    const int coutp = pixie_conv_cout_padded(c_out);
    unsigned* slot = reinterpret_cast<unsigned*>(d_packed) + 15;
    PX_CHECK_HIP(hipMemsetAsync(d_packed, 0, kW16HeaderU4 * sizeof(uint4), st));
    if (pixie_tensor_amax(d_w, (int64_t)c_out * c_in * taps, slot, stream)) return 1;
    const long total = (long)taps * (c_in / 8) * coutp;
    hipLaunchKernelGGL(pack_weights_f16x2_kernel, dim3(cdiv(total, 256)), dim3(256), 0, st, d_w, reinterpret_cast<uint4*>(d_packed), c_out,
                       c_in, taps, coutp, slot);
    PX_CHECK_HIP(hipGetLastError());
    return 0;
}

extern "C" int64_t pixie_conv_subpixel_bytes(int c_out, int c_in) {
    if (c_out <= 0 || c_in <= 0 || c_in % 16 != 0) return 0;
    return ((int64_t)kW16HeaderU4 + 2 * 64 * (int64_t)(c_in / 8) * pixie_conv_cout_padded(c_out)) * (int64_t)sizeof(uint4);
}

extern "C" int pixie_conv_pack_weights_subpixel(const float* d_w, void* d_packed, int c_out, int c_in, void* stream) {
    PX_REQUIRE(d_w && d_packed && c_out > 0 && c_in > 0 && c_in % 16 == 0,
               "pixie_conv_pack_weights_subpixel: bad arguments (c_in must be a multiple of 16)");
    hipStream_t st = as_stream(stream);
    const int coutp = pixie_conv_cout_padded(c_out);
    unsigned* slot = reinterpret_cast<unsigned*>(d_packed) + 15;
    PX_CHECK_HIP(hipMemsetAsync(d_packed, 0, kW16HeaderU4 * sizeof(uint4), st));
    const long pairs = (long)c_out * c_in;
    hipLaunchKernelGGL(subpixel_amax_kernel, dim3(cdiv(pairs, 256)), dim3(256), 0, st, d_w, pairs, slot);
    PX_CHECK_HIP(hipGetLastError());
    const long total = 64L * (c_in / 8) * coutp;
    hipLaunchKernelGGL(pack_weights_subpixel_kernel, dim3(cdiv(total, 256)), dim3(256), 0, st, d_w, reinterpret_cast<uint4*>(d_packed), c_out,
                       c_in, coutp, slot);
    PX_CHECK_HIP(hipGetLastError());
    return 0;
}
```

pixie_amd/csrc/unet_exec.hip:

```cpp
#include <hip/hip_runtime.h>

#include <algorithm>
#include <cmath>
#include <cstdlib>
#include <cstring>
#include <map>
#include <memory>
#include <stdexcept>
#include <string>
#include <tuple>
#include <unordered_map>
#include <vector>

#include "../../include/pixie_hip.h"
#include "common.h"

namespace pixie {
int channel_stats_prezeroed(const float* d_x, int channels, int64_t spatial, double* d_sums, uint32_t* d_amax, hipStream_t st);
int norm_finalize_cat(const double* d_sums0, int c0, const double* d_sums1, int c1, int64_t spatial, int mode, int groups, double eps,
                      const float* d_weight, const float* d_bias, float* d_a, float* d_b, hipStream_t st);
namespace {

enum { ACT_NONE = 0, ACT_LEAKY = 1, ACT_SILU = 2 };
enum Kind { CONV_IN, RES, DOWN, ATTN, UP };

struct Blk { Kind kind; std::string prefix; int cin, cout, sp; };
struct Plan {
    std::vector<std::vector<Blk>> in_blocks, out_blocks;
    std::vector<Blk> middle;
    int out_sp = 0;
};

struct Err : std::runtime_error { using std::runtime_error::runtime_error; };
[[noreturn]] void fail(const char* fmt, ...) {
    char buf[512];
    va_list ap; va_start(ap, fmt); vsnprintf(buf, sizeof buf, fmt, ap); va_end(ap);
    throw Err(buf);
}
void ok(int rc, const char* what) { if (rc != 0) fail("%s: %s", what, pixie_last_error()); }

bool has(const std::vector<int>& v, int x) { for (int e : v) if (e == x) return true; return false; }

struct Cfg {
    int feature_channels, cond_dim, model_channels, num_res_blocks;
    std::vector<int> mult, attn;
    int grid_size, out_channels, precision;
    bool has_projector() const { return feature_channels != cond_dim; }
    int projector_hidden() const { return feature_channels > cond_dim ? 128 : 0; }
};

Plan build_plan(const Cfg& c) {
    Plan p;
    const int mc = c.model_channels, nrb = c.num_res_blocks;
    auto name = [](const char* part, int idx, int sub) { return std::string("unet.") + part + "." + std::to_string(idx) + "." + std::to_string(sub); };
    p.in_blocks.push_back({Blk{CONV_IN, "unet.input_blocks.0.0", c.cond_dim, mc, c.grid_size}});
    std::vector<int> chans{mc}, sizes{c.grid_size};
    int ch = mc, ds = 1, sp = c.grid_size;
    for (size_t level = 0; level < c.mult.size(); ++level) {
        const int m = c.mult[level];
        for (int r = 0; r < nrb; ++r) {
            const int idx = (int)p.in_blocks.size();
            std::vector<Blk> seq{Blk{RES, name("input_blocks", idx, 0), ch, m * mc, sp}};
            ch = m * mc;
            if (has(c.attn, ds)) seq.push_back(Blk{ATTN, name("input_blocks", idx, 1), ch, ch, sp});
            p.in_blocks.push_back(seq);
            chans.push_back(ch);
        }
        if (level + 1 != c.mult.size()) {
            const int idx = (int)p.in_blocks.size();
            p.in_blocks.push_back({Blk{DOWN, name("input_blocks", idx, 0), ch, ch, sp}});
            chans.push_back(ch);
            sizes.push_back(sp);
            ds *= 2;
            sp = (sp + 1) / 2;
        }
    }
    p.middle = {Blk{RES, "unet.middle_block.0", ch, ch, sp}, Blk{ATTN, "unet.middle_block.1", ch, ch, sp}, Blk{RES, "unet.middle_block.2", ch, ch, sp}};
    for (int level = (int)c.mult.size() - 1; level >= 0; --level) {
        const int m = c.mult[level];
        for (int i = 0; i <= nrb; ++i) {
            const int idx = (int)p.out_blocks.size();
            const int ich = chans.back(); chans.pop_back();
            std::vector<Blk> seq{Blk{RES, name("output_blocks", idx, 0), ch + ich, mc * m, sp}};
            ch = mc * m;
            if (has(c.attn, ds)) seq.push_back(Blk{ATTN, name("output_blocks", idx, (int)seq.size()), ch, ch, sp});
            if (level && i == nrb) {
                seq.push_back(Blk{UP, name("output_blocks", idx, (int)seq.size()), ch, ch, sp});
                ds /= 2;
                sp = sizes.back(); sizes.pop_back();
            }
            p.out_blocks.push_back(seq);
        }
    }
    p.out_sp = sp;
    return p;
}

struct Param {
    std::string key;
    std::vector<int64_t> shape;
    int64_t numel = 1;
    bool norm = false;
    const float* d = nullptr;
    uint64_t version = 0;
};

std::vector<Param> param_table(const Cfg& c, const Plan& plan) {
    std::vector<Param> out;
    auto add = [&](const std::string& key, std::vector<int64_t> shape, bool norm) {
        Param p; p.key = key; p.shape = shape; p.norm = norm;
        for (int64_t s : shape) p.numel *= s;
        out.push_back(p);
    };
    auto conv = [&](const std::string& prefix, int cout, int cin, int k, int dims = 3) {
        std::vector<int64_t> s{cout, cin};
        for (int i = 0; i < dims; ++i) s.push_back(k);
        add(prefix + ".weight", s, false);
        add(prefix + ".bias", {cout}, false);
    };
    auto norm = [&](const std::string& prefix, std::vector<int64_t> shape) {
        add(prefix + ".weight", shape, true);
        add(prefix + ".bias", shape, true);
    };
    if (c.has_projector()) {
        const int hid = c.projector_hidden();
        if (!hid) {
            conv("projector.net.0", c.cond_dim, c.feature_channels, 1);
            norm("projector.net.1", {c.cond_dim});
        } else {
            conv("projector.net.0", hid, c.feature_channels, 1);
            norm("projector.net.1", {hid});
            conv("projector.net.3", hid, hid, 3);
            norm("projector.net.4", {hid});
            conv("projector.net.6", c.cond_dim, hid, 1);
            norm("projector.net.7", {c.cond_dim});
        }
    }
    auto emit = [&](const Blk& b) {
        const std::vector<int64_t> vol{b.sp, b.sp, b.sp};
        switch (b.kind) {
            case CONV_IN: conv(b.prefix, b.cout, b.cin, 3); break;
            case RES:
                norm(b.prefix + ".in_layers.0", vol);
                conv(b.prefix + ".in_layers.2", b.cout, b.cin, 3);
                norm(b.prefix + ".out_layers.0", vol);
                conv(b.prefix + ".out_layers.3", b.cout, b.cout, 3);
                if (b.cin != b.cout) conv(b.prefix + ".skip_connection", b.cout, b.cin, 1);
                break;
            case DOWN: conv(b.prefix + ".op", b.cout, b.cin, 3); break;
            case UP:   conv(b.prefix + ".conv", b.cout, b.cin, 3); break;
            case ATTN:
                norm(b.prefix + ".norm", {b.cin});
                conv(b.prefix + ".qkv", 3 * b.cin, b.cin, 1, 1);
                conv(b.prefix + ".proj_out", b.cin, b.cin, 1, 1);
                break;
        }
    };
    for (auto& seq : plan.in_blocks) for (auto& b : seq) emit(b);
    for (auto& b : plan.middle) emit(b);
    for (auto& seq : plan.out_blocks) for (auto& b : seq) emit(b);
    norm("unet.out.0", {plan.out_sp, plan.out_sp, plan.out_sp});
    conv("unet.out.2", c.out_channels, c.model_channels, 3);
    return out;
}

struct Arena {
    static constexpr int64_t kAlign = 256;
    char* base = nullptr;
    int64_t capacity = 0, peak = 0;
    std::map<int64_t, int64_t> free_;
    std::map<int64_t, int64_t> used_;

    void reset(char* b, int64_t cap) {
        base = b; capacity = cap; peak = 0;
        free_.clear(); used_.clear();
        free_[0] = cap;
    }
    int64_t alloc(int64_t bytes) {
        bytes = (bytes + kAlign - 1) / kAlign * kAlign;
        if (bytes == 0) bytes = kAlign;
        for (auto it = free_.begin(); it != free_.end(); ++it) {
            if (it->second < bytes) continue;
            const int64_t off = it->first, rest = it->second - bytes;
            free_.erase(it);
            if (rest > 0) free_[off + bytes] = rest;
            used_[off] = bytes;
            if (off + bytes > peak) peak = off + bytes;
            return off;
        }
        fail("pixie_unet_forward: the workspace is too small (%lld bytes; ask pixie_unet_workspace_bytes for this grid size)", (long long)capacity);
    }
    void release(int64_t off) {
        auto u = used_.find(off);
        if (u == used_.end()) return;
        int64_t size = u->second;
        used_.erase(u);
        auto next = free_.lower_bound(off);
        if (next != free_.end() && off + size == next->first) { size += next->second; next = free_.erase(next); }
        if (next != free_.begin()) {
            auto prev = std::prev(next);
            if (prev->first + prev->second == off) { prev->second += size; return; }
        }
        free_[off] = size;
    }
    template <class T> T* ptr(int64_t off) const { return reinterpret_cast<T*>(base + off); }
};

struct Exec;
struct Tens {
    Exec* ex = nullptr;
    float* p = nullptr;
    int64_t off = -1;
    int c = 0, d = 0, h = 0, w = 0;
    int64_t sums_off = -1;
    bool has_sums = false;
    double* sums = nullptr;
    uint32_t* slot = nullptr;
    int64_t spatial() const { return (int64_t)d * h * w; }
    ~Tens();
};
using TP = std::shared_ptr<Tens>;

struct Packed { void* d = nullptr; uint64_t version = ~0ull; };
struct Sized { int64_t bytes; int slots; int64_t zsum_doubles; };
struct Bound { float wmax = 0, bmax = 0; uint64_t wver = ~0ull, bver = ~0ull; };

}
}

using namespace pixie;

struct pixie_unet {
    Cfg cfg;
    Plan plan;
    std::vector<Param> params;
    std::unordered_map<std::string, int> index;
    std::unordered_map<std::string, Packed> packed32, packed16;
    std::unordered_map<std::string, Bound> bounds;
    uint32_t* d_bound_slots = nullptr;
    std::vector<uint32_t> h_bound_slots;
    std::map<std::tuple<int, int, int, bool>, Sized> sized;
    bool fuse_stats = true, split_k = true, fold_skip = true, subpixel = true;
    struct Replay { const float* feat; const float* proj0; float* out; void* ws; int d; uint64_t epoch; hipGraph_t graph; hipGraphExec_t exec; };
    bool use_graph = false;
    uint64_t epoch = 0;
    std::vector<Replay> replays;
    static constexpr size_t kMaxReplays = 4;
    void drop_replay(size_t i) {
        (void)hipGraphExecDestroy(replays[i].exec);
        (void)hipGraphDestroy(replays[i].graph);
        replays.erase(replays.begin() + (long)i);
    }

    const Param& param(const std::string& key) const {
        auto it = index.find(key);
        if (it == index.end()) fail("pixie_unet: no parameter named '%s'", key.c_str());
        return params[it->second];
    }
};

namespace pixie {
namespace {

struct Exec {
    pixie_unet* net = nullptr;
    Arena arena;
    bool dry = false;
    void* stream = nullptr;
    uint32_t* slots = nullptr;
    int slot_next = 0, slot_cap = 0;
    double* zsums = nullptr;
    int64_t zsum_next = 0, zsum_cap = 0;

    TP make(int c, int d, int h, int w) {
        auto t = std::make_shared<Tens>();
        t->ex = this; t->c = c; t->d = d; t->h = h; t->w = w;
        t->off = arena.alloc((int64_t)c * d * h * w * sizeof(float));
        t->p = arena.ptr<float>(t->off);
        return t;
    }
    TP external(const float* p, int c, int d, int h, int w) {
        auto t = std::make_shared<Tens>();
        t->ex = this; t->p = const_cast<float*>(p); t->c = c; t->d = d; t->h = h; t->w = w;
        return t;
    }
    uint32_t* new_slot() {
        if (!dry && slot_next >= slot_cap) fail("pixie_unet_forward: out of |x|max slots (internal sizing error)");
        return dry ? (slot_next++, nullptr) : slots + slot_next++;
    }
    struct Scratch {
        Exec* ex; int64_t off;
        Scratch(Exec* e, int64_t bytes) : ex(e), off(e->arena.alloc(bytes)) {}
        ~Scratch() { ex->arena.release(off); }
        template <class T> T* as() const { return ex->arena.ptr<T>(off); }
    };

    const float* P(const std::string& key) {
        const Param& p = net->param(key);
        if (!dry && !p.d) fail("pixie_unet_forward: parameter '%s' was never set", key.c_str());
        return p.d;
    }
    const void* w16(const std::string& key, bool subpixel = false) {
        const Param& p = net->param(key + ".weight");
        if (dry) return nullptr;
        Packed& e = net->packed16[subpixel ? key + "#subpixel" : key];
        if (e.version != p.version) {
            const int cout = (int)p.shape[0], cin = (int)p.shape[1], k = (int)p.shape[2];
            const int64_t nb = subpixel ? (k == 3 ? pixie_conv_subpixel_bytes(cout, cin) : 0) : pixie_conv_packed16_bytes(cout, cin, k);
            if (nb <= 0) fail("pixie_unet: '%s' cannot take the f16x3 packing (c_in %d)", key.c_str(), cin);
            if (!e.d && hipMalloc(&e.d, (size_t)nb) != hipSuccess) fail("pixie_unet: hipMalloc of %lld bytes failed", (long long)nb);
            if (!p.d) fail("pixie_unet_forward: parameter '%s.weight' was never set", key.c_str());
            if (subpixel) ok(pixie_conv_pack_weights_subpixel(p.d, e.d, cout, cin, stream), "pixie_conv_pack_weights_subpixel");
            else ok(pixie_conv_pack_weights_f16x2(p.d, e.d, cout, cin, k, stream), "pixie_conv_pack_weights_f16x2");
            e.version = p.version;
        }
        return e.d;
    }
    const float* w32(const std::string& key) {
        const Param& p = net->param(key + ".weight");
        if (dry) return nullptr;
        Packed& e = net->packed32[key];
        if (e.version != p.version) {
            const int cout = (int)p.shape[0], cin = (int)p.shape[1], k = (int)p.shape[2];
            int64_t taps = 1;
            for (size_t i = 2; i < p.shape.size(); ++i) taps *= p.shape[i];
            const int64_t nb = taps * cin * pixie_conv_cout_padded(cout) * (int64_t)sizeof(float);
            if (!e.d && hipMalloc(&e.d, (size_t)nb) != hipSuccess) fail("pixie_unet: hipMalloc of %lld bytes failed", (long long)nb);
            if (!p.d) fail("pixie_unet_forward: parameter '%s.weight' was never set", key.c_str());
            ok(pixie_conv_pack_weights(p.d, static_cast<float*>(e.d), cout, cin, k, stream), "pixie_conv_pack_weights");
            e.version = p.version;
        }
        return static_cast<const float*>(e.d);
    }
    float norm_bound(const std::string& key, int64_t count) {
        if (dry) return 1.0f;
        const Bound& b = net->bounds[key];
        return (float)(std::sqrt((double)count) * (double)b.wmax + (double)b.bmax + 1e-30);
    }

    void stats(const TP& t) {
        if (t->has_sums) return;
        t->has_sums = true;
        if (!dry && zsum_next + 2 * t->c > zsum_cap) fail("pixie_unet_forward: out of statistics space (internal sizing error)");
        t->sums = dry ? nullptr : zsums + zsum_next;
        zsum_next += 2 * t->c;
        t->slot = new_slot();
        if (!dry) ok(channel_stats_prezeroed(t->p, t->c, t->spatial(), t->sums, t->slot, as_stream(stream)), "pixie_channel_stats");
    }
    struct AB { std::shared_ptr<Scratch> mem; float* a; float* b; };
    AB norm_finalize(const double* sums, int c, int64_t spatial, int mode, int groups, const float* w, const float* b) {
        AB r;
        const int cpad = (c + 63) / 64 * 64;
        r.mem = std::make_shared<Scratch>(this, (int64_t)(cpad + c) * sizeof(float));
        r.a = r.mem->as<float>();
        r.b = r.a + cpad;
        if (!dry) ok(pixie_norm_finalize(sums, c, spatial, mode, groups, 1e-5, w, b, r.a, r.b, stream), "pixie_norm_finalize");
        return r;
    }

    bool f16_ok(const std::vector<TP>& parts, int stride) const {
        int cin = 0;
        for (auto& t : parts) cin += t->c;
        return net->cfg.precision == 0 && (stride == 1 || stride == 2) && cin % 16 == 0 && parts[0]->c % 8 == 0;
    }
    bool skip_foldable(const TP& x, int cout, int ksize, const std::vector<TP>& sp) const {
        pixie_conv_desc d;
        std::memset(&d, 0, sizeof d);
        d.c0 = x->c; d.in_d = x->d; d.in_h = x->h; d.in_w = x->w;
        d.stride = 1; d.ksize = ksize; d.c_out = cout;
        d.d_w16 = reinterpret_cast<const void*>(0x100);
        d.d_workspace = net->split_k ? reinterpret_cast<void*>(0x100) : nullptr;
        d.skip_c0 = sp[0]->c; d.skip_c1 = sp.size() > 1 ? sp[1]->c : 0;
        return pixie_conv_skip_foldable(&d) != 0;
    }

    struct ConvOpt {
        int stride = 1; bool upsample = false;
        const AB* pro = nullptr; std::string affine_store;
        int act = ACT_NONE; TP residual; float bound = 0.0f;
        int out_d = 0, out_h = 0, out_w = 0;
        float* out_ptr = nullptr;
        const std::vector<TP>* skip_parts = nullptr; std::string skip_key;
    };
    TP conv(const std::vector<TP>& parts, const std::string& wkey, int cout, int ksize, const ConvOpt& o) {
        const TP& x0 = parts[0];
        const Tens* x1 = parts.size() > 1 ? parts[1].get() : nullptr;
        const int up = o.upsample ? 2 : 1, pad = ksize == 3 ? 1 : 0;
        int od = (x0->d * up + 2 * pad - ksize) / o.stride + 1;
        int oh = (x0->h * up + 2 * pad - ksize) / o.stride + 1;
        int ow = (x0->w * up + 2 * pad - ksize) / o.stride + 1;
        pixie_conv_desc desc;
        std::memset(&desc, 0, sizeof desc);
        if (o.out_d) {
            od = std::min(od, o.out_d); oh = std::min(oh, o.out_h); ow = std::min(ow, o.out_w);
            desc.out_d = od; desc.out_h = oh; desc.out_w = ow;
        }
        const bool f16 = f16_ok(parts, o.stride);
        const bool raw = !o.pro && o.affine_store.empty();
        if (f16 && raw) for (auto& t : parts) stats(t);

        TP out = o.out_ptr ? external(o.out_ptr, cout, od, oh, ow) : make(cout, od, oh, ow);
        desc.d_in0 = x0->p; desc.c0 = x0->c;
        desc.d_in1 = x1 ? x1->p : nullptr; desc.c1 = x1 ? x1->c : 0;
        desc.in_d = x0->d; desc.in_h = x0->h; desc.in_w = x0->w;
        desc.upsample = o.upsample ? 1 : 0;
        desc.stride = o.stride;
        desc.ksize = ksize;
        if (o.pro) { desc.d_pro_a = o.pro->a; desc.d_pro_b = o.pro->b; }
        if (!o.affine_store.empty()) { desc.d_gamma = P(o.affine_store + ".weight"); desc.d_beta = P(o.affine_store + ".bias"); }
        desc.act = o.act;
        desc.d_bias = P(wkey + ".bias");
        desc.c_out = cout;
        desc.d_residual = o.residual ? o.residual->p : nullptr;
        desc.d_out = out->p;
        if (!f16) {
            desc.d_w = w32(wkey);
            if (!dry) ok(pixie_conv3d_forward(&desc, stream), "pixie_conv3d_forward");
            return out;
        }
        const bool sub = net->subpixel && o.upsample && ksize == 3 && o.stride == 1;
        desc.d_w16 = w16(wkey, sub);
        desc.w16_subpixel = sub ? 1 : 0;
        if (o.skip_parts) {
            const std::vector<TP>& sp = *o.skip_parts;
            desc.d_skip_in0 = sp[0]->p; desc.skip_c0 = sp[0]->c;
            desc.d_skip_in1 = sp.size() > 1 ? sp[1]->p : nullptr; desc.skip_c1 = sp.size() > 1 ? sp[1]->c : 0;
            desc.d_skip_w16 = w16(o.skip_key);
            desc.d_skip_bias = P(o.skip_key + ".bias");
            desc.d_skip_amax0 = sp[0]->slot; desc.d_skip_amax1 = sp.size() > 1 ? sp[1]->slot : nullptr;
            if (dry) desc.d_skip_w16 = reinterpret_cast<const void*>(0x100);
        }
        if (raw) {
            desc.d_in_amax0 = parts[0]->slot;
            desc.d_in_amax1 = x1 ? parts[1]->slot : nullptr;
        } else {
            desc.in_bound = o.bound;
        }
        std::unique_ptr<Scratch> workspace, tile_stats;
        if (dry) { desc.d_w16 = reinterpret_cast<const void*>(0x100); }
        if (net->split_k) {
            const int64_t wsb = pixie_conv_workspace_bytes(&desc);
            if (wsb > 0) { workspace.reset(new Scratch(this, wsb)); desc.d_workspace = workspace->as<void>(); if (dry) desc.d_workspace = reinterpret_cast<void*>(0x100); }
        }
        bool have_stats = false;
        if (net->fuse_stats) {
            uint32_t* slot = new_slot();
            const int64_t nfl = pixie_conv_stats_floats(&desc);
            if (nfl > 0) {
                tile_stats.reset(new Scratch(this, nfl * (int64_t)sizeof(float)));
                desc.d_out_stats = tile_stats->as<float>();
                desc.d_out_amax = slot;
                have_stats = true;
                out->slot = slot;
            }
        }
        if (!dry) ok(pixie_conv3d_forward(&desc, stream), "pixie_conv3d_forward");
        if (have_stats) {
            out->sums_off = arena.alloc((int64_t)cout * 2 * sizeof(double));
            out->sums = arena.ptr<double>(out->sums_off);
            out->has_sums = true;
            if (!dry) ok(pixie_stats_finalize(desc.d_out_stats, &desc, out->sums, stream), "pixie_stats_finalize");
        }
        return out;
    }

    AB norm_finalize_parts(const std::vector<TP>& parts, int64_t spatial) {
        for (auto& t : parts) stats(t);
        if (parts.size() == 1) return norm_finalize(parts[0]->sums, parts[0]->c, spatial, 0, 1, nullptr, nullptr);
        const int c0 = parts[0]->c, c1 = parts[1]->c, c = c0 + c1;
        AB r;
        const int cpad = (c + 63) / 64 * 64;
        r.mem = std::make_shared<Scratch>(this, (int64_t)(cpad + c) * sizeof(float));
        r.a = r.mem->as<float>();
        r.b = r.a + cpad;
        if (!dry) ok(norm_finalize_cat(parts[0]->sums, c0, parts[1]->sums, c1, spatial, 0, 1, 1e-5, nullptr, nullptr, r.a, r.b, as_stream(stream)),
                     "pixie_norm_finalize");
        return r;
    }
    TP res(const Blk& b, const std::vector<TP>& parts) {
        const std::string& p = b.prefix;
        const int64_t spatial = parts[0]->spatial();
        AB pro = norm_finalize_parts(parts, spatial);
        ConvOpt o1; o1.pro = &pro; o1.affine_store = p + ".in_layers.0"; o1.act = ACT_LEAKY; o1.bound = norm_bound(p + ".in_layers.0", spatial);
        TP h = conv(parts, p + ".in_layers.2", b.cout, 3, o1);
        stats(h);
        AB pro2 = norm_finalize(h->sums, b.cout, spatial, 0, 1, nullptr, nullptr);
        TP skip = parts[0];
        ConvOpt o2; o2.pro = &pro2; o2.affine_store = p + ".out_layers.0"; o2.act = ACT_LEAKY; o2.bound = norm_bound(p + ".out_layers.0", spatial);
        if (b.cin != b.cout) {
            if (net->fold_skip && f16_ok({h}, 1) && f16_ok(parts, 1) && skip_foldable(h, b.cout, 3, parts)) {
                skip.reset();
                for (auto& t : parts) stats(t);
                o2.skip_parts = &parts; o2.skip_key = p + ".skip_connection";
            } else {
                skip = conv(parts, p + ".skip_connection", b.cout, 1, ConvOpt{});
            }
        }
        o2.residual = skip;
        return conv({h}, p + ".out_layers.3", b.cout, 3, o2);
    }
    TP attn(const Blk& b, const TP& x) {
        const std::string& p = b.prefix;
        const int c = x->c;
        const int64_t spatial = x->spatial();
        stats(x);
        AB pro = norm_finalize(x->sums, c, spatial, 1, 32, P(p + ".norm.weight"), P(p + ".norm.bias"));
        ConvOpt o; o.pro = &pro; o.bound = norm_bound(p + ".norm", spatial * (c / 32));
        TP qkv = conv({x}, p + ".qkv", 3 * c, 1, o);
        TP att = make(c, x->d, x->h, x->w);
        if (!dry) ok(pixie_attention_forward(qkv->p, att->p, c, (int)spatial, stream), "pixie_attention_forward");
        qkv.reset();
        ConvOpt o2; o2.residual = x;
        return conv({att}, p + ".proj_out", c, 1, o2);
    }
    TP block(const Blk& b, const std::vector<TP>& parts, const Tens* up_to) {
        if (b.kind == RES) return res(b, parts);
        const TP& x = parts[0];
        if (b.kind == ATTN) return attn(b, x);
        if (b.kind == DOWN) { ConvOpt o; o.stride = 2; return conv({x}, b.prefix + ".op", b.cout, 3, o); }
        if (b.kind == UP) {
            ConvOpt o; o.upsample = true;
            if (up_to) { o.out_d = up_to->d; o.out_h = up_to->h; o.out_w = up_to->w; }
            return conv({x}, b.prefix + ".conv", b.cout, 3, o);
        }
        fail("pixie_unet: unexpected block kind");
    }

    TP forward(const float* d_feat, const float* d_proj0, int D, int H, int W, float* d_out) {
        const Cfg& c = net->cfg;
        const int64_t spatial = (int64_t)D * H * W;
        TP x;
        AB pro_in; const AB* pro_in_p = nullptr;
        int act_in = ACT_NONE; float bound_in = 0.0f;
        if (c.has_projector()) {
            const std::string q = "projector.net.";
            const int hid = c.projector_hidden();
            if (!hid) {
                const int g = std::max(c.cond_dim / 2, 1);
                x = conv({external(d_feat, c.feature_channels, D, H, W)}, q + "0", c.cond_dim, 1, ConvOpt{});
                stats(x);
                pro_in = norm_finalize(x->sums, c.cond_dim, spatial, 1, g, P(q + "1.weight"), P(q + "1.bias"));
                act_in = ACT_SILU;
                bound_in = norm_bound(q + "1", spatial * (c.cond_dim / g));
            } else {
                if (d_proj0) x = external(d_proj0, hid, D, H, W);
                else x = conv({external(d_feat, c.feature_channels, D, H, W)}, q + "0", hid, 1, ConvOpt{});
                stats(x);
                AB pro = norm_finalize(x->sums, hid, spatial, 1, 32, P(q + "1.weight"), P(q + "1.bias"));
                ConvOpt o; o.pro = &pro; o.act = ACT_SILU; o.bound = norm_bound(q + "1", spatial * (hid / 32));
                x = conv({x}, q + "3", hid, 3, o);
                stats(x);
                AB pro2 = norm_finalize(x->sums, hid, spatial, 1, 32, P(q + "4.weight"), P(q + "4.bias"));
                ConvOpt o2; o2.pro = &pro2; o2.act = ACT_SILU; o2.bound = norm_bound(q + "4", spatial * (hid / 32));
                x = conv({x}, q + "6", c.cond_dim, 1, o2);
                stats(x);
                pro_in = norm_finalize(x->sums, c.cond_dim, spatial, 1, 32, P(q + "7.weight"), P(q + "7.bias"));
                bound_in = norm_bound(q + "7", spatial * std::max(c.cond_dim / 32, 1));
            }
            pro_in_p = &pro_in;
        } else {
            x = external(d_feat, c.feature_channels, D, H, W);
        }
        const Plan& plan = net->plan;
        std::vector<TP> hs;
        const Blk& first = plan.in_blocks[0][0];
        ConvOpt of; of.pro = pro_in_p; of.act = act_in; of.bound = bound_in;
        TP h = conv({x}, first.prefix, first.cout, 3, of);
        x.reset();
        pro_in = AB{};
        hs.push_back(h);
        for (size_t i = 1; i < plan.in_blocks.size(); ++i) {
            for (const Blk& b : plan.in_blocks[i]) h = block(b, {h}, nullptr);
            hs.push_back(h);
        }
        for (const Blk& b : plan.middle) h = block(b, {h}, nullptr);
        for (auto& seq : plan.out_blocks) {
            TP skip = hs.back(); hs.pop_back();
            if (skip->d != h->d || skip->h != h->h || skip->w != h->w) fail("pixie_unet_forward: skip tensor and decoder tensor differ in size");
            std::vector<TP> parts{h, skip};
            h.reset(); skip.reset();
            for (const Blk& b : seq) {
                TP nh = block(b, parts, (b.kind == UP && !hs.empty()) ? hs.back().get() : nullptr);
                parts.clear();
                parts.push_back(nh);
            }
            h = parts[0];
        }
        stats(h);
        AB pro = norm_finalize(h->sums, h->c, h->spatial(), 0, 1, nullptr, nullptr);
        ConvOpt oo; oo.pro = &pro; oo.affine_store = "unet.out.0"; oo.act = ACT_LEAKY; oo.bound = norm_bound("unet.out.0", h->spatial());
        oo.out_ptr = d_out;
        return conv({h}, "unet.out.2", c.out_channels, 3, oo);
    }
};

Tens::~Tens() {
    if (!ex) return;
    if (off >= 0) ex->arena.release(off);
    if (sums_off >= 0) ex->arena.release(sums_off);
}

void refresh_bounds(pixie_unet* net, void* stream) {
    std::vector<std::pair<std::string, int>> todo;
    int n_norm = 0;
    for (const Param& p : net->params) {
        if (!p.norm || p.key.size() < 7 || p.key.compare(p.key.size() - 7, 7, ".weight") != 0) continue;
        const std::string key = p.key.substr(0, p.key.size() - 7);
        const Param& pb = net->param(key + ".bias");
        Bound& b = net->bounds[key];
        if (b.wver != p.version || b.bver != pb.version) todo.push_back({key, 2 * n_norm});
        ++n_norm;
    }
    if (todo.empty()) return;
    const size_t bytes = (size_t)2 * n_norm * sizeof(uint32_t);
    if (!net->d_bound_slots && hipMalloc(&net->d_bound_slots, bytes) != hipSuccess) fail("pixie_unet: hipMalloc failed");
    net->h_bound_slots.assign((size_t)2 * n_norm, 0u);
    hipStream_t s = as_stream(stream);
    if (hipMemsetAsync(net->d_bound_slots, 0, bytes, s) != hipSuccess) fail("pixie_unet: hipMemsetAsync failed");
    for (auto& t : todo) {
        const Param& pw = net->param(t.first + ".weight");
        const Param& pb = net->param(t.first + ".bias");
        if (!pw.d || !pb.d) fail("pixie_unet_forward: parameter '%s' was never set", t.first.c_str());
        ok(pixie_tensor_amax(pw.d, pw.numel, net->d_bound_slots + t.second, stream), "pixie_tensor_amax");
        ok(pixie_tensor_amax(pb.d, pb.numel, net->d_bound_slots + t.second + 1, stream), "pixie_tensor_amax");
    }
    if (hipMemcpyAsync(net->h_bound_slots.data(), net->d_bound_slots, bytes, hipMemcpyDeviceToHost, s) != hipSuccess ||
        hipStreamSynchronize(s) != hipSuccess)
        fail("pixie_unet: reading the normalisation bounds back failed: %s", hipGetErrorString(hipGetLastError()));
    for (auto& t : todo) {
        Bound& b = net->bounds[t.first];
        std::memcpy(&b.wmax, &net->h_bound_slots[t.second], 4);
        std::memcpy(&b.bmax, &net->h_bound_slots[t.second + 1], 4);
        b.wver = net->param(t.first + ".weight").version;
        b.bver = net->param(t.first + ".bias").version;
    }
}

__global__ void zero_head_kernel(uint4* p, int64_t n16) {
    const int64_t i = (int64_t)blockIdx.x * 256 + threadIdx.x;
    if (i < n16) p[i] = make_uint4(0u, 0u, 0u, 0u);
}

constexpr int64_t kSlotAlign = 256;
int64_t slot_region_bytes(int n_slots) { return ((int64_t)n_slots * 4 + kSlotAlign - 1) / kSlotAlign * kSlotAlign; }
int64_t zsum_region_bytes(int64_t n_doubles) { return (n_doubles * 8 + kSlotAlign - 1) / kSlotAlign * kSlotAlign; }

Sized size_pass(pixie_unet* net, int D, int H, int W, bool from_proj0) {
    auto key = std::make_tuple(D, H, W, from_proj0);
    auto it = net->sized.find(key);
    if (it != net->sized.end()) return it->second;
    Exec ex;
    ex.net = net; ex.dry = true; ex.stream = nullptr;
    ex.arena.reset(reinterpret_cast<char*>(0x10000000), (int64_t)1 << 50);
    {
        const float* fake = reinterpret_cast<const float*>(0x100);
        TP out = ex.forward(from_proj0 ? nullptr : fake, from_proj0 ? fake : nullptr, D, H, W, reinterpret_cast<float*>(0x100));
    }
    Sized r{ex.arena.peak + slot_region_bytes(ex.slot_next) + zsum_region_bytes(ex.zsum_next), ex.slot_next, ex.zsum_next};
    net->sized[key] = r;
    return r;
}

template <class F> int guarded(F f) {
    try { return f(); }
    catch (const std::exception& e) { return set_error("%s", e.what()); }
}

}
}

extern "C" int pixie_unet_create(pixie_unet** out, const pixie_unet_config* c) {
    PX_REQUIRE(out && c, "pixie_unet_create: null argument");
    PX_REQUIRE(c->n_channel_mult >= 1 && c->n_channel_mult <= 8 && c->n_attention_resolutions >= 0 && c->n_attention_resolutions <= 8,
               "pixie_unet_create: channel_mult needs 1..8 entries, attention_resolutions 0..8");
    PX_REQUIRE(c->feature_channels > 0 && c->cond_dim > 0 && c->model_channels > 0 && c->num_res_blocks > 0 && c->grid_size > 0 && c->out_channels > 0,
               "pixie_unet_create: non-positive size");
    PX_REQUIRE(c->precision == 0 || c->precision == 1, "pixie_unet_create: precision is 0 (f16x3) or 1 (exact fp32)");
    return guarded([&] {
        std::unique_ptr<pixie_unet> n(new pixie_unet);
        n->cfg.feature_channels = c->feature_channels; n->cfg.cond_dim = c->cond_dim; n->cfg.model_channels = c->model_channels;
        n->cfg.num_res_blocks = c->num_res_blocks; n->cfg.grid_size = c->grid_size; n->cfg.out_channels = c->out_channels;
        n->cfg.precision = c->precision;
        n->cfg.mult.assign(c->channel_mult, c->channel_mult + c->n_channel_mult);
        n->cfg.attn.assign(c->attention_resolutions, c->attention_resolutions + c->n_attention_resolutions);
        n->plan = build_plan(n->cfg);
        n->params = param_table(n->cfg, n->plan);
        for (size_t i = 0; i < n->params.size(); ++i) n->index[n->params[i].key] = (int)i;
        const char* fs = getenv("PIXIE_FUSE_STATS"); n->fuse_stats = !(fs && fs[0] == '0');
        const char* sk = getenv("PIXIE_CONV_SPLIT_K"); n->split_k = !(sk && sk[0] == '0');
        const char* fk = getenv("PIXIE_FOLD_SKIP"); n->fold_skip = !(fk && fk[0] == '0');
        const char* sx = getenv("PIXIE_CONV_SUBPIXEL"); n->subpixel = !(sx && sx[0] == '0');
        *out = n.release();
        return 0;
    });
}

extern "C" int pixie_unet_destroy(pixie_unet* h) {
    if (!h) return 0;
    for (auto& kv : h->packed16) if (kv.second.d) (void)hipFree(kv.second.d);
    for (auto& kv : h->packed32) if (kv.second.d) (void)hipFree(kv.second.d);
    if (h->d_bound_slots) (void)hipFree(h->d_bound_slots);
    while (!h->replays.empty()) h->drop_replay(0);
    delete h;
    return 0;
}

extern "C" int pixie_unet_param_count(const pixie_unet* h) { return h ? (int)h->params.size() : 0; }

extern "C" int pixie_unet_param_info(const pixie_unet* h, int i, const char** key, int64_t* numel, int32_t* ndim, int64_t shape[5]) {
    PX_REQUIRE(h && i >= 0 && i < (int)h->params.size(), "pixie_unet_param_info: index out of range");
    const Param& p = h->params[i];
    if (key) *key = p.key.c_str();
    if (numel) *numel = p.numel;
    if (ndim) *ndim = (int32_t)p.shape.size();
    if (shape) for (size_t k = 0; k < p.shape.size() && k < 5; ++k) shape[k] = p.shape[k];
    return 0;
}

extern "C" int pixie_unet_set_param(pixie_unet* h, const char* key, const float* d_values, int64_t numel) {
    PX_REQUIRE(h && key && d_values, "pixie_unet_set_param: null argument");
    auto it = h->index.find(key);
    PX_REQUIRE(it != h->index.end(), "pixie_unet_set_param: unexpected key '%s' (the reference's load_state_dict(strict=True) raises here too)", key);
    Param& p = h->params[it->second];
    PX_REQUIRE(numel == p.numel, "pixie_unet_set_param: '%s' has %lld elements, got %lld", key, (long long)p.numel, (long long)numel);
    p.d = d_values;
    ++p.version;
    ++h->epoch;
    return 0;
}

extern "C" int64_t pixie_unet_workspace_bytes(pixie_unet* h, int d, int hh, int w) {
    if (!h || d <= 0 || hh <= 0 || w <= 0) { set_error("pixie_unet_workspace_bytes: bad argument"); return -1; }
    int64_t bytes = -1;
    const int rc = guarded([&] {
        bytes = size_pass(h, d, hh, w, false).bytes;
        if (h->cfg.projector_hidden() > 0) bytes = std::max(bytes, size_pass(h, d, hh, w, true).bytes);
        return 0;
    });
    return rc == 0 ? bytes : -1;
}

extern "C" int pixie_unet_forward(pixie_unet* h, const float* d_feat, const float* d_proj0, int d, int hh, int w, float* d_out,
                                  void* d_workspace, int64_t workspace_bytes, void* stream) {
    PX_REQUIRE(h && d_out && d_workspace && (d_feat || d_proj0), "pixie_unet_forward: null argument");
    PX_REQUIRE(d == h->cfg.grid_size && hh == d && w == d,
               "pixie_unet_forward: the network was built for a %d^3 grid (its LayerNorm parameters have that shape), got %d x %d x %d", h->cfg.grid_size, d, hh, w);
    PX_REQUIRE(!d_proj0 || h->cfg.projector_hidden() > 0, "pixie_unet_forward: d_proj0 needs the hidden-128 projector (feature_channels > cond_dim)");
    PX_REQUIRE(d_feat || (d_proj0 && h->cfg.has_projector()), "pixie_unet_forward: d_feat is null");
    return guarded([&] {
        const auto sized = size_pass(h, d, hh, w, d_proj0 != nullptr);
        if (workspace_bytes < sized.bytes)
            fail("pixie_unet_forward: workspace of %lld bytes, this grid needs %lld (pixie_unet_workspace_bytes)", (long long)workspace_bytes, (long long)sized.bytes);
        auto launch_all = [&] {
            Exec ex;
            ex.net = h; ex.dry = false; ex.stream = stream;
            const int64_t slot_bytes = slot_region_bytes(sized.slots), head_bytes = slot_bytes + zsum_region_bytes(sized.zsum_doubles);
            ex.slots = static_cast<uint32_t*>(d_workspace);
            ex.slot_cap = sized.slots;
            ex.zsums = reinterpret_cast<double*>(static_cast<char*>(d_workspace) + slot_bytes);
            ex.zsum_cap = sized.zsum_doubles;
            hipLaunchKernelGGL(zero_head_kernel, dim3((unsigned)((head_bytes / 16 + 255) / 256)), dim3(256), 0, as_stream(stream),
                               static_cast<uint4*>(d_workspace), head_bytes / 16);
            if (hipGetLastError() != hipSuccess) fail("pixie_unet_forward: clearing the workspace head failed");
            ex.arena.reset(static_cast<char*>(d_workspace) + head_bytes, workspace_bytes - head_bytes);
            TP out = ex.forward(d_feat, d_proj0, d, hh, w, d_out);
        };
        if (h->use_graph) {
            for (size_t i = 0; i < h->replays.size(); ++i) {
                const pixie_unet::Replay& r = h->replays[i];
                if (r.feat != d_feat || r.proj0 != d_proj0 || r.out != d_out || r.ws != d_workspace || r.d != d) continue;
                if (r.epoch != h->epoch) { h->drop_replay(i); break; }
                if (hipGraphLaunch(r.exec, as_stream(stream)) != hipSuccess) fail("pixie_unet_forward: hipGraphLaunch failed: %s", hipGetErrorString(hipGetLastError()));
                if (i + 1 != h->replays.size()) std::rotate(h->replays.begin() + (long)i, h->replays.begin() + (long)i + 1, h->replays.end());
                return 0;
            }
        }
        if (h->use_graph && as_stream(stream) == nullptr)
            fail("pixie_unet_forward: option \"graph\" needs a non-default stream (the legacy stream cannot be captured); pass a created stream or set graph = 0");
        refresh_bounds(h, stream);
        launch_all();
        if (h->use_graph) {
            hipStream_t st = as_stream(stream);
            if (hipStreamBeginCapture(st, hipStreamCaptureModeThreadLocal) != hipSuccess)
                fail("pixie_unet_forward: cannot capture on this stream (graph replay needs a non-default stream): %s", hipGetErrorString(hipGetLastError()));
            hipGraph_t graph = nullptr;
            try { launch_all(); }
            catch (...) { (void)hipStreamEndCapture(st, &graph); if (graph) (void)hipGraphDestroy(graph); throw; }
            if (hipStreamEndCapture(st, &graph) != hipSuccess || !graph) fail("pixie_unet_forward: hipStreamEndCapture failed: %s", hipGetErrorString(hipGetLastError()));
            hipGraphExec_t exec = nullptr;
            if (hipGraphInstantiate(&exec, graph, nullptr, nullptr, 0) != hipSuccess) { (void)hipGraphDestroy(graph); fail("pixie_unet_forward: hipGraphInstantiate failed"); }
            if (h->replays.size() >= pixie_unet::kMaxReplays) h->drop_replay(0);
            h->replays.push_back(pixie_unet::Replay{d_feat, d_proj0, d_out, d_workspace, d, h->epoch, graph, exec});
        }
        return 0;
    });
}

extern "C" int pixie_unet_set_option(pixie_unet* h, const char* key, int value) {
    PX_REQUIRE(h && key, "pixie_unet_set_option: null argument");
    const std::string k(key);
    if (k == "graph") {
        h->use_graph = value != 0;
        if (!h->use_graph) while (!h->replays.empty()) h->drop_replay(0);
        return 0;
    }
    return set_error("pixie_unet_set_option: unknown key '%s' (known: graph)", key);
}
```

pixie_amd/unet.py:

```python
from __future__ import annotations

import ctypes as C
import math
import os
import warnings
import weakref
from typing import Dict, List, Optional, Sequence, Tuple

import torch
import torch.nn as nn

from . import _lib
from ._lib import ConvDesc, check
from .unet_plan import Block, UNetConfig, UNetPlan, build_plan, param_shapes, is_norm_key

ACT_NONE, ACT_LEAKY, ACT_SILU = 0, 1, 2
DEFAULT_PRECISION = os.environ.get("PIXIE_CONV_PRECISION", "f16x3")
_ZERO_INIT_SUFFIXES = (".out_layers.3.weight", ".out_layers.3.bias", ".proj_out.weight", ".proj_out.bias",
                       "unet.out.2.weight", "unet.out.2.bias")


def _ptr(t: Optional[torch.Tensor]):
    return C.c_void_p(t.data_ptr()) if t is not None else C.c_void_p(0)


def _addr(t: Optional[torch.Tensor]):
    return t.data_ptr() if t is not None else None


def fill_conv_desc(lib, alloc, parts: Sequence[torch.Tensor], packed_w, bias, cout: int, ksize: int, *, stride: int = 1,
                   upsample: bool = False, pro=None, affine=None, act: int = 0, residual=None, w16=None, in_amax=None,
                   in_bound: float = 0.0, out_amax=None, out_size=None, skip=None, subpixel: bool = False, split_k: bool = True,
                   addr=_addr):
    x0 = parts[0]
    x1 = parts[1] if len(parts) > 1 else None
    cin0, d, h, w = x0.shape
    up = 2 if upsample else 1
    pad = 1 if ksize == 3 else 0
    od = (d * up + 2 * pad - ksize) // stride + 1
    oh = (h * up + 2 * pad - ksize) // stride + 1
    ow = (w * up + 2 * pad - ksize) // stride + 1
    desc = ConvDesc()
    if out_size is not None:
        od, oh, ow = min(od, int(out_size[0])), min(oh, int(out_size[1])), min(ow, int(out_size[2]))
        desc.out_d, desc.out_h, desc.out_w = od, oh, ow
    out = alloc((cout, od, oh, ow), torch.float32)
    desc.d_in0 = addr(x0); desc.c0 = cin0
    desc.d_in1 = addr(x1)
    desc.c1 = x1.shape[0] if x1 is not None else 0
    desc.in_d, desc.in_h, desc.in_w = d, h, w
    desc.upsample = 1 if upsample else 0
    desc.stride = stride
    desc.ksize = ksize
    desc.d_pro_a = addr(pro[0]) if pro is not None else None
    desc.d_pro_b = addr(pro[1]) if pro is not None else None
    desc.d_gamma = addr(affine[0]) if affine is not None else None
    desc.d_beta = addr(affine[1]) if affine is not None else None
    desc.act = act
    desc.d_w = addr(packed_w)
    desc.d_w16 = addr(w16)
    desc.w16_subpixel = 1 if subpixel else 0
    desc.d_in_amax0 = addr(in_amax[0]) if in_amax else None
    desc.d_in_amax1 = addr(in_amax[1]) if in_amax and len(in_amax) > 1 else None
    desc.in_bound = float(in_bound)
    desc.d_bias = addr(bias)
    desc.c_out = cout
    desc.d_residual = addr(residual)
    desc.d_out = addr(out)
    if skip is not None:
        sp = skip["parts"]
        desc.d_skip_in0 = addr(sp[0]); desc.skip_c0 = sp[0].shape[0]
        desc.d_skip_in1 = addr(sp[1]) if len(sp) > 1 else None
        desc.skip_c1 = sp[1].shape[0] if len(sp) > 1 else 0
        desc.d_skip_w16 = addr(skip["w16"])
        desc.d_skip_bias = addr(skip["bias"])
        desc.d_skip_amax0 = addr(skip["amax"][0])
        desc.d_skip_amax1 = addr(skip["amax"][1]) if len(sp) > 1 else None
    stats = workspace = None
    if w16 is not None and split_k:
        wsb = lib.pixie_conv_workspace_bytes(C.byref(desc))
        if wsb > 0:
            workspace = alloc((wsb,), torch.uint8)
            desc.d_workspace = addr(workspace)
    if out_amax is not None and w16 is not None:
        nfl = lib.pixie_conv_stats_floats(C.byref(desc))
        if nfl > 0:
            stats = alloc((nfl,), torch.float32)
            desc.d_out_stats = addr(stats)
            desc.d_out_amax = addr(out_amax)
    return desc, out, stats, workspace


class HipOps:

    def __init__(self, device: torch.device):
        if device.type != "cuda":
            raise _lib.PixieHipError("pixie_amd U-Net operators run on a HIP device only (no CPU fallback)")
        self.device = device
        self.lib = _lib.load()
        self.split_k = os.environ.get("PIXIE_CONV_SPLIT_K", "1") != "0"
        self.record_variant = False
        self.last_variant = (0, 1)

    @property
    def stream(self):
        return _lib.current_stream_ptr()

    def pack_conv(self, weight: torch.Tensor) -> torch.Tensor:
        cout, cin = weight.shape[0], weight.shape[1]
        k = weight.shape[2]
        coutp = self.lib.pixie_conv_cout_padded(cout)
        w = weight.detach().to(self.device, torch.float32).contiguous()
        taps = 1
        for s in weight.shape[2:]:
            taps *= int(s)
        packed = torch.empty((taps, cin, coutp), device=self.device, dtype=torch.float32)
        check(self.lib.pixie_conv_pack_weights(_ptr(w), _ptr(packed), cout, cin, k, self.stream), "pixie_conv_pack_weights")
        return packed

    def pack_conv16(self, weight: torch.Tensor) -> torch.Tensor:
        cout, cin, k = weight.shape[0], weight.shape[1], weight.shape[2]
        nbytes = self.lib.pixie_conv_packed16_bytes(cout, cin, k)
        if nbytes <= 0:
            raise _lib.PixieHipError(f"f16x3 packing needs c_in % 8 == 0 (got {cin})")
        w = weight.detach().to(self.device, torch.float32).contiguous()
        packed = torch.empty(nbytes, device=self.device, dtype=torch.uint8)
        check(self.lib.pixie_conv_pack_weights_f16x2(_ptr(w), _ptr(packed), cout, cin, k, self.stream), "pixie_conv_pack_weights_f16x2")
        return packed

    def pack_conv_subpixel(self, weight: torch.Tensor) -> torch.Tensor:
        cout, cin = weight.shape[0], weight.shape[1]
        nbytes = self.lib.pixie_conv_subpixel_bytes(cout, cin) if tuple(weight.shape[2:]) == (3, 3, 3) else 0
        if nbytes <= 0:
            raise _lib.PixieHipError(f"sub-pixel packing needs a 3x3x3 weight with c_in % 16 == 0 (got {tuple(weight.shape)})")
        w = weight.detach().to(self.device, torch.float32).contiguous()
        packed = torch.empty(nbytes, device=self.device, dtype=torch.uint8)
        check(self.lib.pixie_conv_pack_weights_subpixel(_ptr(w), _ptr(packed), cout, cin, self.stream), "pixie_conv_pack_weights_subpixel")
        return packed

    @staticmethod
    def f16x3_ok(parts: Sequence[torch.Tensor], stride: int) -> bool:
        cin = sum(int(p.shape[0]) for p in parts)
        return stride in (1, 2) and cin % 16 == 0 and int(parts[0].shape[0]) % 8 == 0

    def conv(self, parts: Sequence[torch.Tensor], packed_w: Optional[torch.Tensor], bias: Optional[torch.Tensor], cout: int, ksize: int,
             stride: int = 1, upsample: bool = False, pro: Optional[Tuple[torch.Tensor, torch.Tensor]] = None,
             affine: Optional[Tuple[torch.Tensor, torch.Tensor]] = None, act: int = ACT_NONE,
             residual: Optional[torch.Tensor] = None, w16: Optional[torch.Tensor] = None,
             in_amax: Optional[Sequence[torch.Tensor]] = None, in_bound: float = 0.0,
             out_amax: Optional[torch.Tensor] = None, out_size: Optional[Tuple[int, int, int]] = None,
             skip: Optional[dict] = None, subpixel: bool = False):
        desc, out, stats, _ = fill_conv_desc(
            self.lib, lambda shape, dtype: torch.empty(shape, device=self.device, dtype=dtype), parts, packed_w, bias, cout, ksize,
            stride=stride, upsample=upsample, pro=pro, affine=affine, act=act, residual=residual, w16=w16, in_amax=in_amax,
            in_bound=in_bound, out_amax=out_amax, out_size=out_size, skip=skip, subpixel=subpixel, split_k=self.split_k)
        sums = None
        if self.record_variant:
            sl = C.c_int(1)
            self.last_variant = (int(_lib.load(diag=True).pixie_conv_kernel_variant(C.byref(desc), C.byref(sl))), int(sl.value))
        check(self.lib.pixie_conv3d_forward(C.byref(desc), self.stream), "pixie_conv3d_forward")
        if desc.d_out_stats:
            sums = torch.empty((cout, 2), device=self.device, dtype=torch.float64)
            check(self.lib.pixie_stats_finalize(_ptr(stats), C.byref(desc), _ptr(sums), self.stream), "pixie_stats_finalize")
        if out_amax is not None:
            return out, sums
        return out

    def skip_foldable(self, x: torch.Tensor, cout: int, ksize: int, skip_parts: Sequence[torch.Tensor]) -> bool:
        desc = ConvDesc()
        desc.c0 = x.shape[0]
        desc.in_d, desc.in_h, desc.in_w = (int(v) for v in x.shape[1:])
        desc.stride, desc.ksize, desc.c_out = 1, ksize, cout
        desc.d_w16 = 1
        desc.d_workspace = 1 if self.split_k else None
        desc.skip_c0 = skip_parts[0].shape[0]
        desc.skip_c1 = skip_parts[1].shape[0] if len(skip_parts) > 1 else 0
        return bool(self.lib.pixie_conv_skip_foldable(C.byref(desc)))

    def channel_sums(self, x: torch.Tensor) -> torch.Tensor:
        c = x.shape[0]
        spatial = x.numel() // c
        sums = torch.empty((c, 2), device=self.device, dtype=torch.float64)
        check(self.lib.pixie_channel_sums(_ptr(x), c, spatial, _ptr(sums), self.stream), "pixie_channel_sums")
        return sums

    def channel_stats(self, x: torch.Tensor, amax_slot: torch.Tensor) -> torch.Tensor:
        c = x.shape[0]
        spatial = x.numel() // c
        sums = torch.empty((c, 2), device=self.device, dtype=torch.float64)
        check(self.lib.pixie_channel_stats(_ptr(x), c, spatial, _ptr(sums), _ptr(amax_slot), self.stream), "pixie_channel_stats")
        return sums

    def norm_finalize(self, sums: torch.Tensor, spatial: int, mode: int, groups: int = 1, eps: float = 1e-5,
                      weight: Optional[torch.Tensor] = None, bias: Optional[torch.Tensor] = None):
        c = sums.shape[0]
        a = torch.empty(c, device=self.device, dtype=torch.float32)
        b = torch.empty(c, device=self.device, dtype=torch.float32)
        check(self.lib.pixie_norm_finalize(_ptr(sums), c, spatial, mode, groups, eps, _ptr(weight), _ptr(bias), _ptr(a), _ptr(b),
                                           self.stream), "pixie_norm_finalize")
        return a, b

    def attention(self, qkv: torch.Tensor, channels: int, tokens: int) -> torch.Tensor:
        out = torch.empty((channels, tokens), device=self.device, dtype=torch.float32)
        check(self.lib.pixie_attention_forward(_ptr(qkv), _ptr(out), channels, tokens, self.stream), "pixie_attention_forward")
        return out

    def projector_conv0(self, grid_dhwc_f16: torch.Tensor, nets: Sequence[Tuple[torch.Tensor, Optional[torch.Tensor]]], cout: int):
        d, h, w, c = (int(v) for v in grid_dhwc_f16.shape)
        g = grid_dhwc_f16.contiguous()
        outs = [torch.empty((cout, d, h, w), device=self.device, dtype=torch.float32) for _ in nets]
        n = len(nets)
        w_arr = (C.c_void_p * n)(*[t[0].data_ptr() for t in nets])
        b_arr = (C.c_void_p * n)(*[(t[1].data_ptr() if t[1] is not None else None) for t in nets])
        o_arr = (C.c_void_p * n)(*[o.data_ptr() for o in outs])
        check(self.lib.pixie_projector_conv0(_ptr(g), d * h * w, c, n, w_arr, b_arr, o_arr, cout, self.stream), "pixie_projector_conv0")
        return outs

    def combine(self, logits: torch.Tensor, cont: torch.Tensor):
        ncls = logits.shape[0]
        spatial = logits.numel() // ncls
        combined = torch.empty((3 + ncls,) + tuple(logits.shape[1:]), device=self.device, dtype=torch.float32)
        amax = torch.empty(tuple(logits.shape[1:]), device=self.device, dtype=torch.int32)
        check(self.lib.pixie_combine_predictions(_ptr(logits), ncls, _ptr(cont), spatial, _ptr(combined), _ptr(amax), self.stream),
              "pixie_combine_predictions")
        return combined, amax


class UNetRunner:

    def __init__(self, cfg: UNetConfig, params: Dict[str, torch.Tensor], ops, precision: Optional[str] = None):
        self.cfg = cfg
        self.plan: UNetPlan = build_plan(cfg)
        self.p = params
        self.ops = ops
        self.precision = precision or DEFAULT_PRECISION
        if self.precision not in ("f16x3", "f32"):
            raise ValueError(f"unknown conv precision {self.precision!r}")
        self._packed: Dict[str, Tuple[int, int, torch.Tensor]] = {}
        self._packed16: Dict[str, Tuple[int, int, torch.Tensor]] = {}
        self._bounds: Dict[str, Tuple[int, int, float, float]] = {}
        self.fuse_stats = os.environ.get("PIXIE_FUSE_STATS", "1") != "0"
        self.fold_skip = os.environ.get("PIXIE_FOLD_SKIP", "1") != "0"
        self.subpixel = os.environ.get("PIXIE_CONV_SUBPIXEL", "1") != "0"

    @property
    def _f16x3(self) -> bool:
        return self.precision == "f16x3" and hasattr(self.ops, "pack_conv16")

    def _w(self, key: str) -> torch.Tensor:
        t = self.p[key + ".weight"]
        ent = self._packed.get(key)
        if ent is None or ent[0] != t.data_ptr() or ent[1] != t._version:
            self._packed[key] = (t.data_ptr(), t._version, self.ops.pack_conv(t))
        return self._packed[key][2]

    def _w16(self, key: str, subpixel: bool = False) -> torch.Tensor:
        t = self.p[key + ".weight"]
        ck = key + "#subpixel" if subpixel else key
        ent = self._packed16.get(ck)
        if ent is None or ent[0] != t.data_ptr() or ent[1] != t._version:
            self._packed16[ck] = (t.data_ptr(), t._version, self.ops.pack_conv_subpixel(t) if subpixel else self.ops.pack_conv16(t))
        return self._packed16[ck][2]

    def _b(self, key: str) -> torch.Tensor:
        return self.p[key + ".bias"]

    def _absmax(self, key: str) -> Tuple[float, float]:
        w, bb = self.p[key + ".weight"], self.p[key + ".bias"]
        ent = self._bounds.get(key)
        if ent is None or ent[0] != w._version or ent[1] != bb._version:
            self._bounds[key] = (w._version, bb._version, float(w.abs().max()), float(bb.abs().max()))
            ent = self._bounds[key]
        return ent[2], ent[3]

    def _norm_bound(self, key: str, count: int) -> float:
        wmax, bmax = self._absmax(key)
        return math.sqrt(float(count)) * wmax + bmax + 1e-30

    _SLOT_POOL = 1024

    @classmethod
    def _new_slot(cls, cache: dict, device) -> torch.Tensor:
        pool = cache.get("_slots")
        if pool is None or cache["_next"] >= pool.numel():
            pool = cache["_slots"] = torch.zeros(cls._SLOT_POOL, dtype=torch.int32, device=device)
            cache["_next"] = 0
        i = cache["_next"]
        cache["_next"] = i + 1
        return pool[i:i + 1]

    @staticmethod
    def _remember(cache: dict, t: torch.Tensor, sums, slot) -> None:
        k = id(t)
        cache[k] = (sums, slot)
        weakref.finalize(t, cache.pop, k, None)

    def _stats(self, cache: dict, t: torch.Tensor):
        k = id(t)
        if k not in cache:
            if hasattr(self.ops, "channel_stats"):
                slot = self._new_slot(cache, t.device)
                self._remember(cache, t, self.ops.channel_stats(t, slot), slot)
            else:
                self._remember(cache, t, self.ops.channel_sums(t), None)
        return cache[k]

    def _sums(self, cache: dict, t: torch.Tensor) -> torch.Tensor:
        return self._stats(cache, t)[0]

    def _amax(self, cache: dict, t: torch.Tensor) -> torch.Tensor:
        return self._stats(cache, t)[1]

    def _conv(self, cache: dict, parts: List[torch.Tensor], wkey: str, cout: int, ksize: int, *, stride: int = 1,
              upsample: bool = False, pro=None, affine_key: Optional[str] = None, act: int = ACT_NONE,
              residual: Optional[torch.Tensor] = None, bound: float = 0.0, out_size=None, skip=None) -> torch.Tensor:
        ops = self.ops
        affine = (self.p[affine_key + ".weight"], self.p[affine_key + ".bias"]) if affine_key else None
        if not (self._f16x3 and ops.f16x3_ok(parts, stride)):
            return ops.conv(parts, self._w(wkey), self._b(wkey), cout, ksize, stride=stride, upsample=upsample, pro=pro,
                            affine=affine, act=act, residual=residual, **({"out_size": out_size} if out_size is not None else {}))
        if pro is None and affine is None:
            kw = dict(in_amax=[self._amax(cache, t) for t in parts])
        else:
            kw = dict(in_bound=bound)
        if out_size is not None:
            kw["out_size"] = out_size
        if skip is not None:
            kw["skip"] = skip
        sub = self.subpixel and upsample and ksize == 3 and stride == 1 and hasattr(ops, "pack_conv_subpixel")
        if sub:
            kw["subpixel"] = True
        if self.fuse_stats:
            slot = self._new_slot(cache, parts[0].device)
            out, sums = ops.conv(parts, None, self._b(wkey), cout, ksize, stride=stride, upsample=upsample, pro=pro, affine=affine,
                                 act=act, residual=residual, w16=self._w16(wkey, sub), out_amax=slot, **kw)
            if sums is not None:
                self._remember(cache, out, sums, slot)
            return out
        return ops.conv(parts, None, self._b(wkey), cout, ksize, stride=stride, upsample=upsample, pro=pro, affine=affine,
                        act=act, residual=residual, w16=self._w16(wkey, sub), **kw)

    def _res(self, b: Block, parts: List[torch.Tensor], cache: dict) -> torch.Tensor:
        ops, p = self.ops, b.prefix
        spatial = parts[0][0].numel()
        sums = torch.cat([self._sums(cache, t) for t in parts], dim=0) if len(parts) > 1 else self._sums(cache, parts[0])
        pro = ops.norm_finalize(sums, spatial, 0)
        h = self._conv(cache, parts, p + ".in_layers.2", b.cout, 3, pro=pro, affine_key=p + ".in_layers.0", act=ACT_LEAKY,
                       bound=self._norm_bound(p + ".in_layers.0", spatial))
        pro2 = ops.norm_finalize(self._sums(cache, h), spatial, 0)
        fold = None
        if b.cin != b.cout:
            if (self.fold_skip and self._f16x3 and ops.f16x3_ok([h], 1) and ops.f16x3_ok(parts, 1)
                    and ops.skip_foldable(h, b.cout, 3, parts)):
                skip = None
                fold = dict(parts=parts, w16=self._w16(p + ".skip_connection"), bias=self._b(p + ".skip_connection"),
                            amax=[self._amax(cache, t) for t in parts])
            else:
                skip = self._conv(cache, parts, p + ".skip_connection", b.cout, 1)
        else:
            skip = parts[0]
        return self._conv(cache, [h], p + ".out_layers.3", b.cout, 3, pro=pro2, affine_key=p + ".out_layers.0", act=ACT_LEAKY,
                          residual=skip, bound=self._norm_bound(p + ".out_layers.0", spatial), skip=fold)

    def _attn(self, b: Block, x: torch.Tensor, cache: dict) -> torch.Tensor:
        ops, p = self.ops, b.prefix
        c = x.shape[0]
        spatial = x[0].numel()
        pro = ops.norm_finalize(self._sums(cache, x), spatial, 1, groups=32, weight=self.p[p + ".norm.weight"],
                                bias=self.p[p + ".norm.bias"])
        qkv = self._conv(cache, [x], p + ".qkv", 3 * c, 1, pro=pro, bound=self._norm_bound(p + ".norm", spatial * (c // 32)))
        att = ops.attention(qkv.reshape(3 * c, spatial), c, spatial).reshape(x.shape)
        return self._conv(cache, [att], p + ".proj_out", c, 1, residual=x)

    def _block(self, b: Block, parts: List[torch.Tensor], cache: dict, up_size=None) -> torch.Tensor:
        if b.kind == "res":
            return self._res(b, parts, cache)
        assert len(parts) == 1
        x = parts[0]
        if b.kind == "attn":
            return self._attn(b, x, cache)
        if b.kind == "down":
            return self._conv(cache, [x], b.prefix + ".op", b.cout, 3, stride=2)
        if b.kind == "up":
            return self._conv(cache, [x], b.prefix + ".conv", b.cout, 3, upsample=True, out_size=up_size)
        raise ValueError(b.kind)

    def _stem(self, feat: Optional[torch.Tensor], cache: dict, proj0: Optional[torch.Tensor] = None) -> torch.Tensor:
        cfg, ops = self.cfg, self.ops
        spatial = (proj0 if proj0 is not None else feat)[0].numel()
        x = feat
        pro_in, act_in, bound_in = None, ACT_NONE, 0.0
        if cfg.has_projector:
            q = "projector.net."
            if cfg.projector_hidden is None:
                g = max(cfg.cond_dim // 2, 1)
                x = self._conv(cache, [x], q + "0", cfg.cond_dim, 1)
                pro_in = ops.norm_finalize(self._sums(cache, x), spatial, 1, groups=g,
                                           weight=self.p[q + "1.weight"], bias=self.p[q + "1.bias"])
                act_in = ACT_SILU
                bound_in = self._norm_bound(q + "1", spatial * (cfg.cond_dim // g))
            else:
                hid = cfg.projector_hidden
                x = proj0 if proj0 is not None else self._conv(cache, [x], q + "0", hid, 1)
                pro = ops.norm_finalize(self._sums(cache, x), spatial, 1, groups=32, weight=self.p[q + "1.weight"], bias=self.p[q + "1.bias"])
                x = self._conv(cache, [x], q + "3", hid, 3, pro=pro, act=ACT_SILU, bound=self._norm_bound(q + "1", spatial * (hid // 32)))
                pro = ops.norm_finalize(self._sums(cache, x), spatial, 1, groups=32, weight=self.p[q + "4.weight"], bias=self.p[q + "4.bias"])
                x = self._conv(cache, [x], q + "6", cfg.cond_dim, 1, pro=pro, act=ACT_SILU, bound=self._norm_bound(q + "4", spatial * (hid // 32)))
                pro_in = ops.norm_finalize(self._sums(cache, x), spatial, 1, groups=32, weight=self.p[q + "7.weight"], bias=self.p[q + "7.bias"])
                bound_in = self._norm_bound(q + "7", spatial * max(cfg.cond_dim // 32, 1))
        first = self.plan.input_blocks[0][0]
        return self._conv(cache, [x], first.prefix, first.cout, 3, pro=pro_in, act=act_in, bound=bound_in)

    def _head(self, h: torch.Tensor, cache: dict) -> torch.Tensor:
        pro = self.ops.norm_finalize(self._sums(cache, h), h[0].numel(), 0)
        return self._conv(cache, [h], "unet.out.2", self.cfg.out_channels, 3, pro=pro, affine_key="unet.out.0", act=ACT_LEAKY,
                          bound=self._norm_bound("unet.out.0", h[0].numel()))

    def forward(self, feat: Optional[torch.Tensor], taps: Optional[dict] = None, proj0: Optional[torch.Tensor] = None) -> torch.Tensor:
        cache: dict = {}
        only = set(taps) if taps else None

        def tap(key, t):
            if taps is not None and (only is None or key in only):
                taps[key] = t

        plan = self.plan
        hs: List[torch.Tensor] = []
        h = self._stem(feat, cache, proj0)
        hs.append(h)
        tap("unet.input_blocks.0", h)
        for seq in plan.input_blocks[1:]:
            for b in seq:
                h = self._block(b, [h], cache)
            hs.append(h)
            tap(seq[0].prefix.rsplit(".", 1)[0], h)
        for b in plan.middle:
            h = self._block(b, [h], cache)
            tap(b.prefix, h)
        for seq in plan.output_blocks:
            skip = hs.pop()
            assert tuple(skip.shape[1:]) == tuple(h.shape[1:]), (skip.shape, h.shape)
            parts = [h, skip]
            for b in seq:
                h = self._block(b, parts, cache, up_size=tuple(hs[-1].shape[1:]) if (b.kind == "up" and hs) else None)
                parts = [h]
            tap(seq[0].prefix.rsplit(".", 1)[0], h)
        return self._head(h, cache)


class UNetHandle:

    def __init__(self, cfg: UNetConfig, precision: str, device: torch.device):
        if device.type != "cuda":
            raise _lib.PixieHipError("pixie_amd U-Net runs on a HIP device only (no CPU fallback)")
        if precision not in ("f16x3", "f32"):
            raise ValueError(f"unknown conv precision {precision!r}")
        self.lib = _lib.load()
        self.cfg, self.precision, self.device = cfg, precision, device
        c = _lib.UNetConfigC()
        c.feature_channels, c.cond_dim, c.model_channels, c.num_res_blocks = cfg.feature_channels, cfg.cond_dim, cfg.model_channels, cfg.num_res_blocks
        c.n_channel_mult = len(cfg.channel_mult)
        for i, m in enumerate(cfg.channel_mult):
            c.channel_mult[i] = int(m)
        c.n_attention_resolutions = len(cfg.attention_resolutions)
        for i, m in enumerate(cfg.attention_resolutions):
            c.attention_resolutions[i] = int(m)
        c.grid_size, c.out_channels, c.precision = cfg.grid_size, cfg.out_channels, 0 if precision == "f16x3" else 1
        self._h = C.c_void_p()
        check(self.lib.pixie_unet_create(C.byref(self._h), C.byref(c)), "pixie_unet_create")
        weakref.finalize(self, self.lib.pixie_unet_destroy, self._h)
        self._seen: Dict[str, Tuple[int, int]] = {}
        self._keep: Dict[str, torch.Tensor] = {}

    def keys(self) -> List[str]:
        out = []
        for i in range(self.lib.pixie_unet_param_count(self._h)):
            key = C.c_char_p()
            check(self.lib.pixie_unet_param_info(self._h, i, C.byref(key), None, None, None), "pixie_unet_param_info")
            out.append(key.value.decode())
        return out

    def load(self, params: Dict[str, torch.Tensor]) -> None:
        for key, t in params.items():
            tag = (t.data_ptr(), t._version)
            if self._seen.get(key) == tag:
                continue
            v = t.detach()
            if v.device != self.device or v.dtype != torch.float32 or not v.is_contiguous():
                v = v.to(self.device, torch.float32).contiguous()
            self._keep[key] = v
            check(self.lib.pixie_unet_set_param(self._h, key.encode(), _ptr(v), v.numel()), "pixie_unet_set_param")
            self._seen[key] = tag

    def workspace_bytes(self, d: int, h: int, w: int) -> int:
        n = int(self.lib.pixie_unet_workspace_bytes(self._h, d, h, w))
        if n < 0:
            raise _lib.PixieHipError(self.lib.pixie_last_error().decode())
        return n

    def forward(self, feat: Optional[torch.Tensor], proj0: Optional[torch.Tensor] = None, workspace: Optional[torch.Tensor] = None) -> torch.Tensor:
        src = proj0 if proj0 is not None else feat
        d, h, w = (int(v) for v in src.shape[1:])
        out = torch.empty((self.cfg.out_channels, d, h, w), device=self.device, dtype=torch.float32)
        nbytes = self.workspace_bytes(d, h, w)
        if workspace is None:
            workspace = torch.empty(nbytes, device=self.device, dtype=torch.uint8)
        elif workspace.dtype != torch.uint8 or workspace.device != self.device or workspace.numel() < nbytes or not workspace.is_contiguous():
            raise ValueError(f"workspace must be a contiguous uint8 tensor of >= {nbytes} bytes on {self.device}")
        check(self.lib.pixie_unet_forward(self._h, _ptr(feat), _ptr(proj0), d, h, w, _ptr(out), _ptr(workspace), nbytes,
                                          _lib.current_stream_ptr()), "pixie_unet_forward")
        return out


class _Node(nn.Module):
    """Empty container used to reproduce the reference's state_dict key hierarchy."""


class _PixieUNet(nn.Module):
    def __init__(self, cfg: UNetConfig):
        super().__init__()
        self.cfg = cfg
        shapes = param_shapes(cfg)
        gen = torch.Generator().manual_seed(0)
        for key, shape in shapes.items():
            parts = key.split(".")
            node = self
            for name in parts[:-1]:
                if name not in node._modules:
                    node.add_module(name, _Node())
                node = node._modules[name]
            node.register_parameter(parts[-1], nn.Parameter(self._init(key, shape, shapes, gen), requires_grad=False))
        self._runner: Optional[UNetRunner] = None
        self._handle: Optional[UNetHandle] = None
        self.executor = os.environ.get("PIXIE_UNET_EXECUTOR", "c")
        self.conv_precision = DEFAULT_PRECISION
        self.use_graph = os.environ.get("PIXIE_UNET_GRAPH", "1") == "1"
        self._graphs: dict = {}
        self._plist = None

    @staticmethod
    def _init(key, shape, shapes, gen) -> torch.Tensor:
        if is_norm_key(key):
            return torch.ones(shape) if key.endswith(".weight") else torch.zeros(shape)
        if key.endswith(_ZERO_INIT_SUFFIXES):
            return torch.zeros(shape)
        wshape = shapes[key[: key.rfind(".")] + ".weight"]
        bound = 1.0 / math.sqrt(float(torch.tensor(wshape[1:]).prod()))
        return (torch.rand(shape, generator=gen) * 2.0 - 1.0) * bound

    def _params(self) -> Dict[str, torch.Tensor]:
        return {k: v for k, v in self.named_parameters()}

    def load_numpy_state(self, sd) -> None:
        self.load_state_dict({k: torch.from_numpy(v) for k, v in sd.items()}, strict=True)

    @torch.no_grad()
    def forward(self, feat_grid: torch.Tensor, taps: Optional[dict] = None) -> torch.Tensor:
        if feat_grid.dim() != 5 or feat_grid.shape[1] != self.cfg.feature_channels:
            raise ValueError(f"expected (N,{self.cfg.feature_channels},D,H,W), got {tuple(feat_grid.shape)}")
        dev = next(self.parameters()).device
        if dev.type != "cuda" or feat_grid.device != dev:
            raise _lib.PixieHipError("model and input must live on the same HIP device (no CPU fallback)")
        with torch.cuda.device(dev):
            self._prepare(dev)
            x = feat_grid.detach().to(torch.float32).contiguous()
            if self.use_graph and taps is None:
                return torch.stack([self._forward_graphed(x[n]) for n in range(x.shape[0])], dim=0)
            outs = [self._forward_one(x[n], taps=taps if n == 0 else None) for n in range(x.shape[0])]
            return torch.stack(outs, dim=0)

    def _prepare(self, dev) -> None:
        params = self._params()
        if self._runner is None or self._runner.ops.device != dev or self._runner.precision != self.conv_precision:
            self._runner = UNetRunner(self.cfg, params, HipOps(dev), precision=self.conv_precision)
        else:
            self._runner.p = params
        if self.executor == "c":
            if self._handle is None or self._handle.device != dev or self._handle.precision != self.conv_precision:
                self._handle = UNetHandle(self.cfg, self.conv_precision, dev)
            self._handle.load(params)
        elif self.executor != "python":
            raise ValueError(f"unknown executor {self.executor!r} (PIXIE_UNET_EXECUTOR is 'c' or 'python')")

    def _forward_one(self, x: Optional[torch.Tensor], taps: Optional[dict] = None, proj0: Optional[torch.Tensor] = None) -> torch.Tensor:
        if self.executor == "c" and taps is None:
            return self._handle.forward(x, proj0)
        return self._runner.forward(x, taps, proj0)

    def _apply(self, fn, *args, **kwargs):
        self._plist = None
        return super()._apply(fn, *args, **kwargs)

    def _param_list(self) -> List[torch.Tensor]:
        refs = self.__dict__.get("_plist")
        if refs is None:
            refs = self._plist = [(m._parameters, name) for m in self.modules() for name, p in m._parameters.items() if p is not None]
        return [d[name] for d, name in refs]

    def load_state_dict(self, state_dict, strict: bool = True, assign: bool = False):
        self._plist = None
        return super().load_state_dict(state_dict, strict=strict, assign=assign)

    def _forward_graphed(self, x: Optional[torch.Tensor], proj0: Optional[torch.Tensor] = None) -> torch.Tensor:
        src = proj0 if proj0 is not None else x
        base = (tuple(src.shape), tuple(src.stride()), src.dtype, proj0 is not None, self.executor, self.conv_precision, src.device.index,
                tuple((id(p), p.data_ptr(), p._version) for p in self._param_list()))
        run = (lambda t: self._forward_one(None, proj0=t)) if proj0 is not None else (lambda t: self._forward_one(t))
        if self._graphs.get("base") != base:
            self._graphs = {"base": base, "first_ptr": None}
        ent = self._graphs.get(src.data_ptr()) or self._graphs.get("copy")
        if ent is None:
            out = run(src)
            if self._graphs["first_ptr"] is None:
                self._graphs["first_ptr"] = src.data_ptr()
                return out
            in_place = (proj0 is None and self._graphs["first_ptr"] == src.data_ptr() and "copy" not in self._graphs
                        and os.environ.get("PIXIE_UNET_GRAPH_INPLACE", "1") == "1")
            try:
                static_in = src if in_place else src.clone()
                side = torch.cuda.Stream(src.device)
                side.wait_stream(torch.cuda.current_stream())
                with torch.cuda.stream(side):
                    run(static_in)
                torch.cuda.current_stream().wait_stream(side)
                graph = torch.cuda.CUDAGraph()
                with torch.cuda.graph(graph, capture_error_mode="thread_local"):
                    static_out = run(static_in)
            except RuntimeError as exc:
                warnings.warn(f"pixie_amd: HIP-graph capture of the U-Net forward failed ({exc}); continuing with eager launches",
                              RuntimeWarning)
                self.use_graph = False
                return out
            if in_place:
                ent = self._graphs[src.data_ptr()] = (graph, None, static_out)
            else:
                ent = self._graphs["copy"] = (graph, static_in, static_out)
        graph, static_in, static_out = ent
        if static_in is not None:
            static_in.copy_(src)
        graph.replay()
        return static_out.clone()


class SegmentationUNet(_PixieUNet):

    def __init__(self, feature_channels: int, cond_dim: int, model_channels: int, num_res_blocks: int,
                 channel_mult: Tuple[int, ...], attention_resolutions: Tuple[int, ...], grid_size: int, num_classes: int):
        super().__init__(UNetConfig(feature_channels, cond_dim, model_channels, num_res_blocks, tuple(channel_mult),
                                    tuple(attention_resolutions), grid_size, num_classes))


class RegressionUNet(_PixieUNet):

    def __init__(self, feature_channels: int, cond_dim: int, model_channels: int, num_res_blocks: int,
                 channel_mult: Tuple[int, ...], attention_resolutions: Tuple[int, ...], grid_size: int, out_channels: int = 3):
        super().__init__(UNetConfig(feature_channels, cond_dim, model_channels, num_res_blocks, tuple(channel_mult),
                                    tuple(attention_resolutions), grid_size, out_channels))


@torch.no_grad()
def predict_material_field_from_voxel_grid(seg_network: "SegmentationUNet", cont_network: "RegressionUNet", grid_dhwc_f16: torch.Tensor,
                                           dual_stream: Optional[bool] = None):
    dev = next(seg_network.parameters()).device
    g = grid_dhwc_f16
    if g.dim() != 4 or g.dtype != torch.float16 or g.device != dev or dev.type != "cuda":
        raise ValueError("expected a (D, H, W, C) float16 tensor on the networks' HIP device")
    nets = (seg_network, cont_network)
    for net in nets:
        if net.cfg.projector_hidden is None or net.cfg.feature_channels != g.shape[3] or net.conv_precision != "f16x3":
            raise ValueError("the fused grid path needs the hidden-128 projector, matching feature_channels and conv_precision 'f16x3'")
        net._prepare(dev)
    ops = seg_network._runner.ops
    q = "projector.net.0"
    packed = [(net._runner._w16(q), net._runner._b(q)) for net in nets]
    x_seg, x_cont = ops.projector_conv0(g, packed, seg_network.cfg.projector_hidden)
    if dual_stream is None:
        dual_stream = _dual_stream_default(seg_network, cont_network, int(g.shape[0]) * int(g.shape[1]) * int(g.shape[2]))

    def fwd(net, p0):
        return net._forward_graphed(None, p0) if net.use_graph else net._forward_one(None, proj0=p0)

    if dual_stream:
        cur = torch.cuda.current_stream()
        s1, s2 = _side_streams(dev)
        s1.wait_stream(cur); s2.wait_stream(cur)
        with torch.cuda.stream(s1):
            seg_logits = fwd(seg_network, x_seg)[None]
        with torch.cuda.stream(s2):
            cont_pred = fwd(cont_network, x_cont)[None]
        x_seg.record_stream(s1); x_cont.record_stream(s2)
        cur.wait_stream(s1); cur.wait_stream(s2)
        seg_logits.record_stream(cur); cont_pred.record_stream(cur)
    else:
        seg_logits = fwd(seg_network, x_seg)[None]
        cont_pred = fwd(cont_network, x_cont)[None]
    combined, seg_pred = ops.combine(seg_logits[0].contiguous(), cont_pred[0].contiguous())
    return combined[None], seg_pred[None], seg_logits, cont_pred


_SIDE_STREAMS: Dict[str, Tuple[torch.cuda.Stream, torch.cuda.Stream]] = {}


def _dual_stream_default(seg_network, cont_network, voxels: int) -> bool:
    env = os.environ.get("PIXIE_DUAL_STREAM")
    if env is not None:
        return env == "1"
    return not (seg_network.use_graph and cont_network.use_graph and voxels >= 128 ** 3)


def _side_streams(device):
    key = str(device)
    if key not in _SIDE_STREAMS:
        _SIDE_STREAMS[key] = (torch.cuda.Stream(device), torch.cuda.Stream(device))
    return _SIDE_STREAMS[key]


@torch.no_grad()
def predict_material_field(seg_network: SegmentationUNet, cont_network: RegressionUNet, feat_grid: torch.Tensor,
                           dual_stream: Optional[bool] = None):
    if feat_grid.is_cuda and feat_grid.device.index != torch.cuda.current_device():
        with torch.cuda.device(feat_grid.device):
            return predict_material_field(seg_network, cont_network, feat_grid, dual_stream)
    if dual_stream is None:
        dual_stream = _dual_stream_default(seg_network, cont_network, int(feat_grid[0, 0].numel()))
    if dual_stream and feat_grid.is_cuda:
        cur = torch.cuda.current_stream()
        s1, s2 = _side_streams(feat_grid.device)
        s1.wait_stream(cur); s2.wait_stream(cur)
        with torch.cuda.stream(s1):
            seg_logits = seg_network(feat_grid)
        with torch.cuda.stream(s2):
            cont_pred = cont_network(feat_grid)
        feat_grid.record_stream(s1); feat_grid.record_stream(s2)
        cur.wait_stream(s1); cur.wait_stream(s2)
        seg_logits.record_stream(cur); cont_pred.record_stream(cur)
    else:
        seg_logits = seg_network(feat_grid)
        cont_pred = cont_network(feat_grid)
    ops = seg_network._runner.ops
    combined, seg_pred = [], []
    for n in range(feat_grid.shape[0]):
        cmb, am = ops.combine(seg_logits[n].contiguous(), cont_pred[n].contiguous())
        combined.append(cmb)
        seg_pred.append(am)
    return torch.stack(combined), torch.stack(seg_pred), seg_logits, cont_pred
```

Measured before the change: 24.11 million voxels/s.

## Fuse split-K reduction with channel stats and merge stats finalize into norm finalize

The split-K reduce kernel now also emits per-segment per-channel sum, sum-of-squares and amax, so split-K conv outputs no longer need a separate channel-stats pass over the output. Statistics finalization and norm finalization are merged into one kernel that reduces the per-tile partials and computes the affine coefficients, and concatenated inputs are handled as two parts. This removes an extra full read of activations and some kernel launches, at the cost of a 2D reduce grid with double-precision accumulation and more bookkeeping to keep partial buffers alive until the norm consumes them.

Measured after the change: 24.36 million voxels/s, median of 6. 1.1% higher.

```diff
diff --git a/include/pixie_hip.h b/include/pixie_hip.h
--- a/include/pixie_hip.h
+++ b/include/pixie_hip.h
@@ -130,6 +130,9 @@
 int64_t pixie_conv_stats_floats(const pixie_conv_desc* desc);
 int64_t pixie_conv_workspace_bytes(const pixie_conv_desc* desc);
 int pixie_stats_finalize(const float* d_stats, const pixie_conv_desc* desc, double* d_sums, void* stream);
+int pixie_stats_norm_finalize(const float* d_stats0, const pixie_conv_desc* desc0, double* d_sums0, const float* d_stats1,
+                              const pixie_conv_desc* desc1, double* d_sums1, int c1, int64_t spatial, int mode, int groups,
+                              double eps, const float* d_weight, const float* d_bias, float* d_a, float* d_b, void* stream);
 int pixie_conv_skip_foldable(const pixie_conv_desc* desc);
 
 int pixie_channel_sums(const float* d_x, int channels, int64_t spatial, double* d_sums, void* stream);
diff --git a/pixie_amd/_lib.py b/pixie_amd/_lib.py
--- a/pixie_amd/_lib.py
+++ b/pixie_amd/_lib.py
@@ -119,6 +119,7 @@
     "pixie_conv_stats_floats": (_I64, [C.POINTER(ConvDesc)]),
     "pixie_conv_workspace_bytes": (_I64, [C.POINTER(ConvDesc)]),
     "pixie_stats_finalize": (_I, [_VP, C.POINTER(ConvDesc), _VP, _VP]),
+    "pixie_stats_norm_finalize": (_I, [_VP, C.POINTER(ConvDesc), _VP, _VP, C.POINTER(ConvDesc), _VP, _I, _I64, _I, _I, _D, _VP, _VP, _VP, _VP, _VP]),
     "pixie_channel_stats": (_I, [_VP, _I, _I64, _VP, _VP, _VP]),
     "pixie_tensor_amax": (_I, [_VP, _I64, _VP, _VP]),
     "pixie_channel_sums": (_I, [_VP, _I, _I64, _VP, _VP]),
diff --git a/pixie_amd/csrc/conv3d_f16x3.hip b/pixie_amd/csrc/conv3d_f16x3.hip
--- a/pixie_amd/csrc/conv3d_f16x3.hip
+++ b/pixie_amd/csrc/conv3d_f16x3.hip
@@ -604,18 +604,68 @@
     conv3d_f16x3_body<3, 2, 4>(A);
 }
 
-__global__ __launch_bounds__(256) void stats_finalize_kernel(const float* __restrict__ stats, int n_tiles, int coutp, double* __restrict__ sums) {
-    const int c = blockIdx.x;
+struct StatParts { const void* p; int n; long cstride, tstride; int f64; };
+
+__device__ inline void block_channel_sums(const StatParts& P, int c, double* r, double& o1, double& o2) {
     double s1 = 0.0, s2 = 0.0;
-    for (int t = threadIdx.x; t < n_tiles; t += 256) {
-        const float2 v = *reinterpret_cast<const float2*>(stats + ((size_t)t * coutp + c) * 2);
-        s1 += v.x; s2 += v.y;
+    for (int t = threadIdx.x; t < P.n; t += 256) {
+        const size_t k = ((size_t)c * P.cstride + (size_t)t * P.tstride) * 2;
+        if (P.f64) { const double2 v = *reinterpret_cast<const double2*>(static_cast<const double*>(P.p) + k); s1 += v.x; s2 += v.y; }
+        else { const float2 v = *reinterpret_cast<const float2*>(static_cast<const float*>(P.p) + k); s1 += v.x; s2 += v.y; }
     }
     for (int off = 32; off > 0; off >>= 1) { s1 += __shfl_down(s1, off, 64); s2 += __shfl_down(s2, off, 64); }
-    __shared__ double r[8];
     if ((threadIdx.x & 63) == 0) { r[2 * (threadIdx.x >> 6)] = s1; r[2 * (threadIdx.x >> 6) + 1] = s2; }
     __syncthreads();
-    if (threadIdx.x == 0) { sums[2 * c] = r[0] + r[2] + r[4] + r[6]; sums[2 * c + 1] = r[1] + r[3] + r[5] + r[7]; }
+    o1 = r[0] + r[2] + r[4] + r[6]; o2 = r[1] + r[3] + r[5] + r[7];
+    __syncthreads();
+}
+
+__global__ __launch_bounds__(256) void stats_finalize_kernel(StatParts P, double* __restrict__ sums) {
+    const int c = blockIdx.x;
+    __shared__ double r[8];
+    double s1, s2;
+    block_channel_sums(P, c, r, s1, s2);
+    if (threadIdx.x == 0) { sums[2 * c] = s1; sums[2 * c + 1] = s2; }
+}
+
+__global__ __launch_bounds__(256) void stats_norm_finalize_kernel(StatParts P0, double* sums0, int c0, StatParts P1, double* sums1, int channels,
+                                                                  double spatial, int mode, int groups, double eps,
+                                                                  const float* __restrict__ weight, const float* __restrict__ bias,
+                                                                  float* __restrict__ a, float* __restrict__ b) {
+    __shared__ double r[8];
+    const int cpg = mode == 0 ? 1 : channels / groups;
+    const int first = blockIdx.x * cpg;
+    double s1 = 0.0, s2 = 0.0;
+    for (int k = first; k < first + cpg; ++k) {
+        const bool in0 = k < c0;
+        const StatParts& P = in0 ? P0 : P1;
+        double* sums = in0 ? sums0 : sums1;
+        const int kc = in0 ? k : k - c0;
+        double t1, t2;
+        if (P.n > 0) {
+            block_channel_sums(P, kc, r, t1, t2);
+            if (threadIdx.x == 0) { sums[2 * kc] = t1; sums[2 * kc + 1] = t2; }
+        } else {
+            t1 = sums[2 * kc]; t2 = sums[2 * kc + 1];
+        }
+        s1 += t1; s2 += t2;
+    }
+    const double cnt = mode == 0 ? spatial : spatial * cpg;
+    const double mean = s1 / cnt;
+    double var = s2 / cnt - mean * mean;
+    if (var < 0.0) var = 0.0;
+    const double rstd = 1.0 / sqrt(var + eps);
+    for (int k = first + threadIdx.x; k < first + cpg; k += 256) {
+        if (mode == 0) {
+            a[k] = (float)rstd;
+            b[k] = (float)(-mean * rstd);
+        } else {
+            const double w = weight ? (double)weight[k] : 1.0;
+            const double bb = bias ? (double)bias[k] : 0.0;
+            a[k] = (float)(rstd * w);
+            b[k] = (float)(bb - mean * rstd * w);
+        }
+    }
 }
 
 __global__ __launch_bounds__(256) void splitk_reduce_kernel(const float* __restrict__ partial, int slices, long n_elems, long osp,
@@ -627,6 +677,75 @@
     if (bias) v += bias[i / osp];
     if (residual) v += residual[i];
     out[i] = v;
+}
+
+constexpr int kReduceSeg = 4096;
+template <bool VEC>
+__global__ __launch_bounds__(256) void splitk_reduce_stats_kernel(const float* __restrict__ partial, int slices, long n_elems, long osp,
+                                                                  const float* __restrict__ bias, const float* residual, float* out,
+                                                                  double* __restrict__ stats, unsigned* out_amax) {
+    const int c = blockIdx.y;
+    const long seg0 = (long)blockIdx.x * kReduceSeg;
+    const size_t base = (size_t)c * osp;
+    const float bv = bias ? bias[c] : 0.0f;
+    double s1 = 0.0, s2 = 0.0;
+    float mx = 0.0f;
+    if (VEC) {
+#pragma unroll
+        for (int k = 0; k < kReduceSeg / 1024; ++k) {
+            const long j = seg0 + k * 1024 + (long)threadIdx.x * 4;
+            if (j < osp) {
+                const size_t i = base + j;
+                float4 v = *reinterpret_cast<const float4*>(partial + i);
+                for (int s = 1; s < slices; ++s) {
+                    const float4 q = *reinterpret_cast<const float4*>(partial + (size_t)s * n_elems + i);
+                    v.x += q.x; v.y += q.y; v.z += q.z; v.w += q.w;
+                }
+                if (bias) { v.x += bv; v.y += bv; v.z += bv; v.w += bv; }
+                if (residual) {
+                    const float4 q = *reinterpret_cast<const float4*>(residual + i);
+                    v.x += q.x; v.y += q.y; v.z += q.z; v.w += q.w;
+                }
+                *reinterpret_cast<float4*>(out + i) = v;
+                const double x = v.x, y = v.y, z = v.z, w = v.w;
+                s1 += (x + y) + (z + w);
+                s2 += (x * x + y * y) + (z * z + w * w);
+                mx = fmaxf(fmaxf(mx, fmaxf(fabsf(v.x), fabsf(v.y))), fmaxf(fabsf(v.z), fabsf(v.w)));
+            }
+        }
+    } else {
+#pragma unroll 4
+        for (int k = 0; k < kReduceSeg / 256; ++k) {
+            const long j = seg0 + k * 256 + threadIdx.x;
+            if (j < osp) {
+                const size_t i = base + j;
+                float v = partial[i];
+                for (int s = 1; s < slices; ++s) v += partial[(size_t)s * n_elems + i];
+                if (bias) v += bv;
+                if (residual) v += residual[i];
+                out[i] = v;
+                const double x = v;
+                s1 += x; s2 += x * x; mx = fmaxf(mx, fabsf(v));
+            }
+        }
+    }
+    for (int off = 32; off > 0; off >>= 1) {
+        s1 += __shfl_down(s1, off, 64);
+        s2 += __shfl_down(s2, off, 64);
+        mx = fmaxf(mx, __shfl_down(mx, off, 64));
+    }
+    __shared__ double r[8];
+    __shared__ float rmx[4];
+    const int lane = threadIdx.x & 63, wave = threadIdx.x >> 6;
+    if (lane == 0) { r[2 * wave] = s1; r[2 * wave + 1] = s2; rmx[wave] = mx; }
+    __syncthreads();
+    if (threadIdx.x == 0) {
+        double* dst = stats + ((size_t)c * gridDim.x + blockIdx.x) * 2;
+        dst[0] = r[0] + r[2] + r[4] + r[6];
+        dst[1] = r[1] + r[3] + r[5] + r[7];
+        const unsigned m = __float_as_uint(fmaxf(fmaxf(rmx[0], rmx[1]), fmaxf(rmx[2], rmx[3])));
+        if (out_amax && m > __hip_atomic_load(out_amax, __ATOMIC_RELAXED, __HIP_MEMORY_SCOPE_AGENT)) atomicMax(out_amax, m);
+    }
 }
 
 __global__ __launch_bounds__(256) void amax_kernel(const float* __restrict__ x, long n, unsigned* __restrict__ slot) {
@@ -812,6 +931,19 @@
     MB_out = MB; NB_out = NB;
 }
 
+static int reduce_segments(long osp) { return (int)((osp + kReduceSeg - 1) / kReduceSeg); }
+
+static StatParts conv16_stat_parts(const pixie_conv_desc* d, const void* stats) {
+    Conv16Args a{};
+    int MB = 0, NB = 0, slices = 1;
+    conv16_tiling(d, a, MB, NB, &slices);
+    if (slices > 1) {
+        const int n = reduce_segments((long)a.OD * a.OH * a.OW);
+        return StatParts{stats, n, n, 1, 1};
+    }
+    return StatParts{stats, a.n_tiles, 1, a.coutp, 0};
+}
+
 static size_t conv16_epi_bytes(int MB, int NB) { return ((size_t)4 * 32 * (NB * 32 + 4) + (size_t)4 * MB * 32 * 2) * sizeof(float); }
 static bool conv16_epi_lds(int MB, int NB, int slices) { return slices == 1 && conv16_epi_bytes(MB, NB) <= 80 * 1024; }
 
@@ -881,8 +1013,19 @@
         }
         if (rc) return rc;
         const long osp = (long)a.OD * a.OH * a.OW, n_elems = (long)a.cout * osp;
-        hipLaunchKernelGGL(splitk_reduce_kernel, dim3((unsigned)((n_elems + 255) / 256)), dim3(256), 0, st, a.partial, slices, n_elems, osp,
-                           a.bias, a.residual, a.out);
+        if (d->d_out_stats) {
+            const dim3 rgrid((unsigned)reduce_segments(osp), (unsigned)a.cout);
+            double* rstats = reinterpret_cast<double*>(d->d_out_stats);
+            PX_REQUIRE((reinterpret_cast<size_t>(rstats) & 7) == 0, "f16x3 conv: d_out_stats of a split-K launch must be 8-byte aligned");
+            const bool vec = osp % 4 == 0 && ((reinterpret_cast<size_t>(a.partial) | reinterpret_cast<size_t>(a.residual) | reinterpret_cast<size_t>(a.out)) & 15) == 0;
+            if (vec) hipLaunchKernelGGL(splitk_reduce_stats_kernel<true>, rgrid, dim3(256), 0, st, a.partial, slices, n_elems, osp, a.bias, a.residual,
+                                        a.out, rstats, d->d_out_amax);
+            else hipLaunchKernelGGL(splitk_reduce_stats_kernel<false>, rgrid, dim3(256), 0, st, a.partial, slices, n_elems, osp, a.bias, a.residual,
+                                    a.out, rstats, d->d_out_amax);
+        } else {
+            hipLaunchKernelGGL(splitk_reduce_kernel, dim3((unsigned)((n_elems + 255) / 256)), dim3(256), 0, st, a.partial, slices, n_elems, osp,
+                               a.bias, a.residual, a.out);
+        }
         PX_CHECK_HIP(hipGetLastError());
         return 0;
     }
@@ -951,7 +1094,8 @@
     Conv16Args a{};
     int MB = 0, NB = 0, slices = 1;
     conv16_tiling(d, a, MB, NB, &slices);
-    return slices > 1 ? 0 : (int64_t)a.n_tiles * a.coutp * 2;
+    if (slices > 1) return (int64_t)a.cout * reduce_segments((long)a.OD * a.OH * a.OW) * 2 * (int64_t)(sizeof(double) / sizeof(float));
+    return (int64_t)a.n_tiles * a.coutp * 2;
 }
 
 extern "C" int64_t pixie_conv_workspace_bytes(const pixie_conv_desc* d) {
@@ -1005,10 +1149,25 @@
 
 extern "C" int pixie_stats_finalize(const float* d_stats, const pixie_conv_desc* d, double* d_sums, void* stream) {
     PX_REQUIRE(d_stats && d && d_sums, "pixie_stats_finalize: null argument");
-    Conv16Args a{};
-    int MB = 0, NB = 0;
-    conv16_tiling(d, a, MB, NB);
-    hipLaunchKernelGGL(stats_finalize_kernel, dim3((unsigned)d->c_out), dim3(256), 0, as_stream(stream), d_stats, a.n_tiles, a.coutp, d_sums);
+    hipLaunchKernelGGL(stats_finalize_kernel, dim3((unsigned)d->c_out), dim3(256), 0, as_stream(stream), conv16_stat_parts(d, d_stats), d_sums);
+    PX_CHECK_HIP(hipGetLastError());
+    return 0;
+}
+
+extern "C" int pixie_stats_norm_finalize(const float* d_stats0, const pixie_conv_desc* desc0, double* d_sums0, const float* d_stats1,
+                                         const pixie_conv_desc* desc1, double* d_sums1, int c1, int64_t spatial, int mode, int groups,
+                                         double eps, const float* d_weight, const float* d_bias, float* d_a, float* d_b, void* stream) {
+    PX_REQUIRE(desc0 && d_sums0 && d_a && d_b && spatial > 0 && c1 >= 0, "pixie_stats_norm_finalize: bad arguments");
+    PX_REQUIRE(c1 == 0 || d_sums1, "pixie_stats_norm_finalize: a second part needs d_sums1");
+    PX_REQUIRE(!d_stats1 || desc1, "pixie_stats_norm_finalize: d_stats1 needs its descriptor");
+    const int c0 = desc0->c_out, channels = c0 + c1;
+    PX_REQUIRE(!d_stats1 || desc1->c_out == c1, "pixie_stats_norm_finalize: desc1 has %d output channels, c1 is %d", desc1 ? desc1->c_out : 0, c1);
+    PX_REQUIRE(mode == 0 || (mode == 1 && groups > 0 && channels % groups == 0), "pixie_stats_norm_finalize: bad mode/groups");
+    const StatParts none{nullptr, 0, 0, 0, 0};
+    const StatParts p0 = d_stats0 ? conv16_stat_parts(desc0, d_stats0) : none;
+    const StatParts p1 = d_stats1 ? conv16_stat_parts(desc1, d_stats1) : none;
+    hipLaunchKernelGGL(stats_norm_finalize_kernel, dim3((unsigned)(mode == 0 ? channels : groups)), dim3(256), 0, as_stream(stream), p0, d_sums0, c0,
+                       p1, d_sums1, channels, (double)spatial, mode, groups, eps, d_weight, d_bias, d_a, d_b);
     PX_CHECK_HIP(hipGetLastError());
     return 0;
 }
diff --git a/pixie_amd/csrc/unet_exec.hip b/pixie_amd/csrc/unet_exec.hip
--- a/pixie_amd/csrc/unet_exec.hip
+++ b/pixie_amd/csrc/unet_exec.hip
@@ -215,6 +215,8 @@
     int64_t sums_off = -1;
     bool has_sums = false;
     double* sums = nullptr;
+    int64_t partials_off = -1;
+    pixie_conv_desc pdesc;
     uint32_t* slot = nullptr;
     int64_t spatial() const { return (int64_t)d * h * w; }
     ~Tens();
@@ -241,6 +243,7 @@
     std::vector<uint32_t> h_bound_slots;
     std::map<std::tuple<int, int, int, bool>, Sized> sized;
     bool fuse_stats = true, split_k = true, fold_skip = true, subpixel = true;
+    bool split_stats = true;
     struct Replay { const float* feat; const float* proj0; float* out; void* ws; int d; uint64_t epoch; hipGraph_t graph; hipGraphExec_t exec; };
     bool use_graph = false;
     uint64_t epoch = 0;
@@ -339,7 +342,7 @@
     }
 
     void stats(const TP& t) {
-        if (t->has_sums) return;
+        if (t->has_sums || t->partials_off >= 0) return;
         t->has_sums = true;
         if (!dry && zsum_next + 2 * t->c > zsum_cap) fail("pixie_unet_forward: out of statistics space (internal sizing error)");
         t->sums = dry ? nullptr : zsums + zsum_next;
@@ -348,13 +351,30 @@
         if (!dry) ok(channel_stats_prezeroed(t->p, t->c, t->spatial(), t->sums, t->slot, as_stream(stream)), "pixie_channel_stats");
     }
     struct AB { std::shared_ptr<Scratch> mem; float* a; float* b; };
-    AB norm_finalize(const double* sums, int c, int64_t spatial, int mode, int groups, const float* w, const float* b) {
+    AB norm_finalize(const std::vector<TP>& parts, int64_t spatial, int mode, int groups, const float* w, const float* b) {
+        for (auto& t : parts) stats(t);
+        const Tens* t0 = parts[0].get();
+        const Tens* t1 = parts.size() > 1 ? parts[1].get() : nullptr;
+        const int c0 = t0->c, c1 = t1 ? t1->c : 0, c = c0 + c1;
         AB r;
         const int cpad = (c + 63) / 64 * 64;
         r.mem = std::make_shared<Scratch>(this, (int64_t)(cpad + c) * sizeof(float));
         r.a = r.mem->as<float>();
         r.b = r.a + cpad;
-        if (!dry) ok(pixie_norm_finalize(sums, c, spatial, mode, groups, 1e-5, w, b, r.a, r.b, stream), "pixie_norm_finalize");
+        const bool p0 = t0->partials_off >= 0, p1 = t1 && t1->partials_off >= 0;
+        if (p0 || p1) {
+            pixie_conv_desc d0 = t0->pdesc;
+            if (!p0) { std::memset(&d0, 0, sizeof d0); d0.c_out = c0; }
+            if (!dry) ok(pixie_stats_norm_finalize(p0 ? arena.ptr<float>(t0->partials_off) : nullptr, &d0, t0->sums,
+                                                   p1 ? arena.ptr<float>(t1->partials_off) : nullptr, p1 ? &t1->pdesc : nullptr, t1 ? t1->sums : nullptr,
+                                                   c1, spatial, mode, groups, 1e-5, w, b, r.a, r.b, stream), "pixie_stats_norm_finalize");
+            for (auto& t : parts)
+                if (t->partials_off >= 0) { arena.release(t->partials_off); t->partials_off = -1; t->has_sums = true; }
+        } else if (!t1) {
+            if (!dry) ok(pixie_norm_finalize(t0->sums, c, spatial, mode, groups, 1e-5, w, b, r.a, r.b, stream), "pixie_norm_finalize");
+        } else {
+            if (!dry) ok(norm_finalize_cat(t0->sums, c0, t1->sums, c1, spatial, mode, groups, 1e-5, w, b, r.a, r.b, as_stream(stream)), "pixie_norm_finalize");
+        }
         return r;
     }
 
@@ -436,7 +456,7 @@
         } else {
             desc.in_bound = o.bound;
         }
-        std::unique_ptr<Scratch> workspace, tile_stats;
+        std::unique_ptr<Scratch> workspace;
         if (dry) { desc.d_w16 = reinterpret_cast<const void*>(0x100); }
         if (net->split_k) {
             const int64_t wsb = pixie_conv_workspace_bytes(&desc);
@@ -446,9 +466,9 @@
         if (net->fuse_stats) {
             uint32_t* slot = new_slot();
             const int64_t nfl = pixie_conv_stats_floats(&desc);
-            if (nfl > 0) {
-                tile_stats.reset(new Scratch(this, nfl * (int64_t)sizeof(float)));
-                desc.d_out_stats = tile_stats->as<float>();
+            if (nfl > 0 && (!workspace || net->split_stats)) {
+                out->partials_off = arena.alloc(nfl * (int64_t)sizeof(float));
+                desc.d_out_stats = arena.ptr<float>(out->partials_off);
                 desc.d_out_amax = slot;
                 have_stats = true;
                 out->slot = slot;
@@ -458,33 +478,18 @@
         if (have_stats) {
             out->sums_off = arena.alloc((int64_t)cout * 2 * sizeof(double));
             out->sums = arena.ptr<double>(out->sums_off);
-            out->has_sums = true;
-            if (!dry) ok(pixie_stats_finalize(desc.d_out_stats, &desc, out->sums, stream), "pixie_stats_finalize");
+            out->pdesc = desc;
         }
         return out;
     }
 
-    AB norm_finalize_parts(const std::vector<TP>& parts, int64_t spatial) {
-        for (auto& t : parts) stats(t);
-        if (parts.size() == 1) return norm_finalize(parts[0]->sums, parts[0]->c, spatial, 0, 1, nullptr, nullptr);
-        const int c0 = parts[0]->c, c1 = parts[1]->c, c = c0 + c1;
-        AB r;
-        const int cpad = (c + 63) / 64 * 64;
-        r.mem = std::make_shared<Scratch>(this, (int64_t)(cpad + c) * sizeof(float));
-        r.a = r.mem->as<float>();
-        r.b = r.a + cpad;
-        if (!dry) ok(norm_finalize_cat(parts[0]->sums, c0, parts[1]->sums, c1, spatial, 0, 1, 1e-5, nullptr, nullptr, r.a, r.b, as_stream(stream)),
-                     "pixie_norm_finalize");
-        return r;
-    }
     TP res(const Blk& b, const std::vector<TP>& parts) {
         const std::string& p = b.prefix;
         const int64_t spatial = parts[0]->spatial();
-        AB pro = norm_finalize_parts(parts, spatial);
+        AB pro = norm_finalize(parts, spatial, 0, 1, nullptr, nullptr);
         ConvOpt o1; o1.pro = &pro; o1.affine_store = p + ".in_layers.0"; o1.act = ACT_LEAKY; o1.bound = norm_bound(p + ".in_layers.0", spatial);
         TP h = conv(parts, p + ".in_layers.2", b.cout, 3, o1);
-        stats(h);
-        AB pro2 = norm_finalize(h->sums, b.cout, spatial, 0, 1, nullptr, nullptr);
+        AB pro2 = norm_finalize({h}, spatial, 0, 1, nullptr, nullptr);
         TP skip = parts[0];
         ConvOpt o2; o2.pro = &pro2; o2.affine_store = p + ".out_layers.0"; o2.act = ACT_LEAKY; o2.bound = norm_bound(p + ".out_layers.0", spatial);
         if (b.cin != b.cout) {
@@ -503,8 +508,7 @@
         const std::string& p = b.prefix;
         const int c = x->c;
         const int64_t spatial = x->spatial();
-        stats(x);
-        AB pro = norm_finalize(x->sums, c, spatial, 1, 32, P(p + ".norm.weight"), P(p + ".norm.bias"));
+        AB pro = norm_finalize({x}, spatial, 1, 32, P(p + ".norm.weight"), P(p + ".norm.bias"));
         ConvOpt o; o.pro = &pro; o.bound = norm_bound(p + ".norm", spatial * (c / 32));
         TP qkv = conv({x}, p + ".qkv", 3 * c, 1, o);
         TP att = make(c, x->d, x->h, x->w);
@@ -538,23 +542,19 @@
             if (!hid) {
                 const int g = std::max(c.cond_dim / 2, 1);
                 x = conv({external(d_feat, c.feature_channels, D, H, W)}, q + "0", c.cond_dim, 1, ConvOpt{});
-                stats(x);
-                pro_in = norm_finalize(x->sums, c.cond_dim, spatial, 1, g, P(q + "1.weight"), P(q + "1.bias"));
+                pro_in = norm_finalize({x}, spatial, 1, g, P(q + "1.weight"), P(q + "1.bias"));
                 act_in = ACT_SILU;
                 bound_in = norm_bound(q + "1", spatial * (c.cond_dim / g));
             } else {
                 if (d_proj0) x = external(d_proj0, hid, D, H, W);
                 else x = conv({external(d_feat, c.feature_channels, D, H, W)}, q + "0", hid, 1, ConvOpt{});
-                stats(x);
-                AB pro = norm_finalize(x->sums, hid, spatial, 1, 32, P(q + "1.weight"), P(q + "1.bias"));
+                AB pro = norm_finalize({x}, spatial, 1, 32, P(q + "1.weight"), P(q + "1.bias"));
                 ConvOpt o; o.pro = &pro; o.act = ACT_SILU; o.bound = norm_bound(q + "1", spatial * (hid / 32));
                 x = conv({x}, q + "3", hid, 3, o);
-                stats(x);
-                AB pro2 = norm_finalize(x->sums, hid, spatial, 1, 32, P(q + "4.weight"), P(q + "4.bias"));
+                AB pro2 = norm_finalize({x}, spatial, 1, 32, P(q + "4.weight"), P(q + "4.bias"));
                 ConvOpt o2; o2.pro = &pro2; o2.act = ACT_SILU; o2.bound = norm_bound(q + "4", spatial * (hid / 32));
                 x = conv({x}, q + "6", c.cond_dim, 1, o2);
-                stats(x);
-                pro_in = norm_finalize(x->sums, c.cond_dim, spatial, 1, 32, P(q + "7.weight"), P(q + "7.bias"));
+                pro_in = norm_finalize({x}, spatial, 1, 32, P(q + "7.weight"), P(q + "7.bias"));
                 bound_in = norm_bound(q + "7", spatial * std::max(c.cond_dim / 32, 1));
             }
             pro_in_p = &pro_in;
@@ -586,8 +586,7 @@
             }
             h = parts[0];
         }
-        stats(h);
-        AB pro = norm_finalize(h->sums, h->c, h->spatial(), 0, 1, nullptr, nullptr);
+        AB pro = norm_finalize({h}, h->spatial(), 0, 1, nullptr, nullptr);
         ConvOpt oo; oo.pro = &pro; oo.affine_store = "unet.out.0"; oo.act = ACT_LEAKY; oo.bound = norm_bound("unet.out.0", h->spatial());
         oo.out_ptr = d_out;
         return conv({h}, "unet.out.2", c.out_channels, 3, oo);
@@ -598,6 +597,7 @@
     if (!ex) return;
     if (off >= 0) ex->arena.release(off);
     if (sums_off >= 0) ex->arena.release(sums_off);
+    if (partials_off >= 0) ex->arena.release(partials_off);
 }
 
 void refresh_bounds(pixie_unet* net, void* stream) {
@@ -689,6 +689,7 @@
         const char* fs = getenv("PIXIE_FUSE_STATS"); n->fuse_stats = !(fs && fs[0] == '0');
         const char* sk = getenv("PIXIE_CONV_SPLIT_K"); n->split_k = !(sk && sk[0] == '0');
         const char* fk = getenv("PIXIE_FOLD_SKIP"); n->fold_skip = !(fk && fk[0] == '0');
+        const char* ss = getenv("PIXIE_SPLIT_STATS"); n->split_stats = !(ss && ss[0] == '0');
         const char* sx = getenv("PIXIE_CONV_SUBPIXEL"); n->subpixel = !(sx && sx[0] == '0');
         *out = n.release();
         return 0;
diff --git a/pixie_amd/unet.py b/pixie_amd/unet.py
--- a/pixie_amd/unet.py
+++ b/pixie_amd/unet.py
@@ -31,7 +31,7 @@
 def fill_conv_desc(lib, alloc, parts: Sequence[torch.Tensor], packed_w, bias, cout: int, ksize: int, *, stride: int = 1,
                    upsample: bool = False, pro=None, affine=None, act: int = 0, residual=None, w16=None, in_amax=None,
                    in_bound: float = 0.0, out_amax=None, out_size=None, skip=None, subpixel: bool = False, split_k: bool = True,
-                   addr=_addr):
+                   split_stats: bool = False, addr=_addr):
     x0 = parts[0]
     x1 = parts[1] if len(parts) > 1 else None
     cin0, d, h, w = x0.shape
@@ -84,11 +84,17 @@
             desc.d_workspace = addr(workspace)
     if out_amax is not None and w16 is not None:
         nfl = lib.pixie_conv_stats_floats(C.byref(desc))
-        if nfl > 0:
+        if nfl > 0 and (workspace is None or split_stats):
             stats = alloc((nfl,), torch.float32)
             desc.d_out_stats = addr(stats)
             desc.d_out_amax = addr(out_amax)
     return desc, out, stats, workspace
+
+
+class PendingStats:
+
+    def __init__(self, stats: torch.Tensor, desc: ConvDesc, cout: int):
+        self.stats, self.desc, self.cout = stats, desc, cout
 
 
 class HipOps:
@@ -149,19 +155,22 @@
              residual: Optional[torch.Tensor] = None, w16: Optional[torch.Tensor] = None,
              in_amax: Optional[Sequence[torch.Tensor]] = None, in_bound: float = 0.0,
              out_amax: Optional[torch.Tensor] = None, out_size: Optional[Tuple[int, int, int]] = None,
-             skip: Optional[dict] = None, subpixel: bool = False):
+             skip: Optional[dict] = None, subpixel: bool = False, defer_stats: bool = False, split_stats: bool = True):
         desc, out, stats, _ = fill_conv_desc(
             self.lib, lambda shape, dtype: torch.empty(shape, device=self.device, dtype=dtype), parts, packed_w, bias, cout, ksize,
             stride=stride, upsample=upsample, pro=pro, affine=affine, act=act, residual=residual, w16=w16, in_amax=in_amax,
-            in_bound=in_bound, out_amax=out_amax, out_size=out_size, skip=skip, subpixel=subpixel, split_k=self.split_k)
+            in_bound=in_bound, out_amax=out_amax, out_size=out_size, skip=skip, subpixel=subpixel, split_k=self.split_k,
+            split_stats=defer_stats and split_stats)
         sums = None
         if self.record_variant:
             sl = C.c_int(1)
             self.last_variant = (int(_lib.load(diag=True).pixie_conv_kernel_variant(C.byref(desc), C.byref(sl))), int(sl.value))
         check(self.lib.pixie_conv3d_forward(C.byref(desc), self.stream), "pixie_conv3d_forward")
         if desc.d_out_stats:
-            sums = torch.empty((cout, 2), device=self.device, dtype=torch.float64)
-            check(self.lib.pixie_stats_finalize(_ptr(stats), C.byref(desc), _ptr(sums), self.stream), "pixie_stats_finalize")
+            if defer_stats:
+                sums = PendingStats(stats, desc, cout)
+            else:
+                sums = self.stats_finalize(PendingStats(stats, desc, cout))
         if out_amax is not None:
             return out, sums
         return out
@@ -199,6 +208,32 @@
         check(self.lib.pixie_norm_finalize(_ptr(sums), c, spatial, mode, groups, eps, _ptr(weight), _ptr(bias), _ptr(a), _ptr(b),
                                            self.stream), "pixie_norm_finalize")
         return a, b
+
+    def stats_finalize(self, pending: PendingStats) -> torch.Tensor:
+        sums = torch.empty((pending.cout, 2), device=self.device, dtype=torch.float64)
+        check(self.lib.pixie_stats_finalize(_ptr(pending.stats), C.byref(pending.desc), _ptr(sums), self.stream), "pixie_stats_finalize")
+        return sums
+
+    def stats_norm_finalize(self, parts: Sequence, spatial: int, mode: int, groups: int = 1, eps: float = 1e-5,
+                            weight: Optional[torch.Tensor] = None, bias: Optional[torch.Tensor] = None):
+        pend = [isinstance(p, PendingStats) for p in parts]
+        sums = [torch.empty((p.cout, 2), device=self.device, dtype=torch.float64) if is_p else p for p, is_p in zip(parts, pend)]
+        c0 = sums[0].shape[0]
+        c1 = sums[1].shape[0] if len(parts) > 1 else 0
+        if pend[0]:
+            desc0 = parts[0].desc
+        else:
+            desc0 = ConvDesc()
+            desc0.c_out = c0
+        two = len(parts) > 1
+        a = torch.empty(c0 + c1, device=self.device, dtype=torch.float32)
+        b = torch.empty(c0 + c1, device=self.device, dtype=torch.float32)
+        check(self.lib.pixie_stats_norm_finalize(
+            _ptr(parts[0].stats) if pend[0] else None, C.byref(desc0), _ptr(sums[0]),
+            _ptr(parts[1].stats) if two and pend[1] else None, C.byref(parts[1].desc) if two and pend[1] else None,
+            _ptr(sums[1]) if two else None, c1, spatial, mode, groups, eps, _ptr(weight), _ptr(bias), _ptr(a), _ptr(b), self.stream),
+            "pixie_stats_norm_finalize")
+        return a, b, sums
 
     def attention(self, qkv: torch.Tensor, channels: int, tokens: int) -> torch.Tensor:
         out = torch.empty((channels, tokens), device=self.device, dtype=torch.float32)
@@ -242,6 +277,7 @@
         self.fuse_stats = os.environ.get("PIXIE_FUSE_STATS", "1") != "0"
         self.fold_skip = os.environ.get("PIXIE_FOLD_SKIP", "1") != "0"
         self.subpixel = os.environ.get("PIXIE_CONV_SUBPIXEL", "1") != "0"
+        self.split_stats = os.environ.get("PIXIE_SPLIT_STATS", "1") != "0"
 
     @property
     def _f16x3(self) -> bool:
@@ -303,13 +339,32 @@
                 self._remember(cache, t, self.ops.channel_stats(t, slot), slot)
             else:
                 self._remember(cache, t, self.ops.channel_sums(t), None)
+        if isinstance(cache[k][0], PendingStats):
+            cache[k] = (self.ops.stats_finalize(cache[k][0]), cache[k][1])
         return cache[k]
+
+    def _norm(self, cache: dict, parts: List[torch.Tensor], spatial: int, mode: int, groups: int = 1, weight=None, bias=None):
+        ops = self.ops
+        for t in parts:
+            if id(t) not in cache:
+                self._stats(cache, t)
+        ents = [cache[id(t)][0] for t in parts]
+        if any(isinstance(e, PendingStats) for e in ents):
+            a, b, sums = ops.stats_norm_finalize(ents, spatial, mode, groups=groups, weight=weight, bias=bias)
+            for t, sm in zip(parts, sums):
+                cache[id(t)] = (sm, cache[id(t)][1])
+            return a, b
+        sums = torch.cat(ents, dim=0) if len(ents) > 1 else ents[0]
+        if mode == 0:
+            return ops.norm_finalize(sums, spatial, 0)
+        return ops.norm_finalize(sums, spatial, mode, groups=groups, weight=weight, bias=bias)
 
     def _sums(self, cache: dict, t: torch.Tensor) -> torch.Tensor:
         return self._stats(cache, t)[0]
 
     def _amax(self, cache: dict, t: torch.Tensor) -> torch.Tensor:
-        return self._stats(cache, t)[1]
+        k = id(t)
+        return cache[k][1] if k in cache else self._stats(cache, t)[1]
 
     def _conv(self, cache: dict, parts: List[torch.Tensor], wkey: str, cout: int, ksize: int, *, stride: int = 1,
               upsample: bool = False, pro=None, affine_key: Optional[str] = None, act: int = ACT_NONE,
@@ -332,6 +387,9 @@
             kw["subpixel"] = True
         if self.fuse_stats:
             slot = self._new_slot(cache, parts[0].device)
+            if hasattr(ops, "stats_norm_finalize"):
+                kw["defer_stats"] = True
+                kw["split_stats"] = self.split_stats
             out, sums = ops.conv(parts, None, self._b(wkey), cout, ksize, stride=stride, upsample=upsample, pro=pro, affine=affine,
                                  act=act, residual=residual, w16=self._w16(wkey, sub), out_amax=slot, **kw)
             if sums is not None:
@@ -343,11 +401,10 @@
     def _res(self, b: Block, parts: List[torch.Tensor], cache: dict) -> torch.Tensor:
         ops, p = self.ops, b.prefix
         spatial = parts[0][0].numel()
-        sums = torch.cat([self._sums(cache, t) for t in parts], dim=0) if len(parts) > 1 else self._sums(cache, parts[0])
-        pro = ops.norm_finalize(sums, spatial, 0)
+        pro = self._norm(cache, parts, spatial, 0)
         h = self._conv(cache, parts, p + ".in_layers.2", b.cout, 3, pro=pro, affine_key=p + ".in_layers.0", act=ACT_LEAKY,
                        bound=self._norm_bound(p + ".in_layers.0", spatial))
-        pro2 = ops.norm_finalize(self._sums(cache, h), spatial, 0)
+        pro2 = self._norm(cache, [h], spatial, 0)
         fold = None
         if b.cin != b.cout:
             if (self.fold_skip and self._f16x3 and ops.f16x3_ok([h], 1) and ops.f16x3_ok(parts, 1)
@@ -366,8 +423,7 @@
         ops, p = self.ops, b.prefix
         c = x.shape[0]
         spatial = x[0].numel()
-        pro = ops.norm_finalize(self._sums(cache, x), spatial, 1, groups=32, weight=self.p[p + ".norm.weight"],
-                                bias=self.p[p + ".norm.bias"])
+        pro = self._norm(cache, [x], spatial, 1, groups=32, weight=self.p[p + ".norm.weight"], bias=self.p[p + ".norm.bias"])
         qkv = self._conv(cache, [x], p + ".qkv", 3 * c, 1, pro=pro, bound=self._norm_bound(p + ".norm", spatial * (c // 32)))
         att = ops.attention(qkv.reshape(3 * c, spatial), c, spatial).reshape(x.shape)
         return self._conv(cache, [att], p + ".proj_out", c, 1, residual=x)
@@ -395,24 +451,23 @@
             if cfg.projector_hidden is None:
                 g = max(cfg.cond_dim // 2, 1)
                 x = self._conv(cache, [x], q + "0", cfg.cond_dim, 1)
-                pro_in = ops.norm_finalize(self._sums(cache, x), spatial, 1, groups=g,
-                                           weight=self.p[q + "1.weight"], bias=self.p[q + "1.bias"])
+                pro_in = self._norm(cache, [x], spatial, 1, groups=g, weight=self.p[q + "1.weight"], bias=self.p[q + "1.bias"])
                 act_in = ACT_SILU
                 bound_in = self._norm_bound(q + "1", spatial * (cfg.cond_dim // g))
             else:
                 hid = cfg.projector_hidden
                 x = proj0 if proj0 is not None else self._conv(cache, [x], q + "0", hid, 1)
-                pro = ops.norm_finalize(self._sums(cache, x), spatial, 1, groups=32, weight=self.p[q + "1.weight"], bias=self.p[q + "1.bias"])
+                pro = self._norm(cache, [x], spatial, 1, groups=32, weight=self.p[q + "1.weight"], bias=self.p[q + "1.bias"])
                 x = self._conv(cache, [x], q + "3", hid, 3, pro=pro, act=ACT_SILU, bound=self._norm_bound(q + "1", spatial * (hid // 32)))
-                pro = ops.norm_finalize(self._sums(cache, x), spatial, 1, groups=32, weight=self.p[q + "4.weight"], bias=self.p[q + "4.bias"])
+                pro = self._norm(cache, [x], spatial, 1, groups=32, weight=self.p[q + "4.weight"], bias=self.p[q + "4.bias"])
                 x = self._conv(cache, [x], q + "6", cfg.cond_dim, 1, pro=pro, act=ACT_SILU, bound=self._norm_bound(q + "4", spatial * (hid // 32)))
-                pro_in = ops.norm_finalize(self._sums(cache, x), spatial, 1, groups=32, weight=self.p[q + "7.weight"], bias=self.p[q + "7.bias"])
+                pro_in = self._norm(cache, [x], spatial, 1, groups=32, weight=self.p[q + "7.weight"], bias=self.p[q + "7.bias"])
                 bound_in = self._norm_bound(q + "7", spatial * max(cfg.cond_dim // 32, 1))
         first = self.plan.input_blocks[0][0]
         return self._conv(cache, [x], first.prefix, first.cout, 3, pro=pro_in, act=act_in, bound=bound_in)
 
     def _head(self, h: torch.Tensor, cache: dict) -> torch.Tensor:
-        pro = self.ops.norm_finalize(self._sums(cache, h), h[0].numel(), 0)
+        pro = self._norm(cache, [h], h[0].numel(), 0)
         return self._conv(cache, [h], "unet.out.2", self.cfg.out_channels, 3, pro=pro, affine_key="unet.out.0", act=ACT_LEAKY,
                           bound=self._norm_bound("unet.out.0", h[0].numel()))
 
```
